# DJjjjhao/FIRA-ICSE

Measured on AMD Instinct MI355X. Metric: training commits/sec (FIRA default config), higher is better.
Workload: dtype f32; 1 GPU; BASELINE configs[1]: FIRA training step (fwd+bwd+Adam, dropout 0.1/0.2), batch 32 commits/GPU, fp32, 650-node graphs (mean nnz 1066/graph), vocab 24650; global_batch=32, parallelism=dp1

## Files before the change

### fira_icse_amd/_lib.py

```python
from __future__ import annotations

import ctypes as C
import os

HERE = os.path.dirname(os.path.abspath(__file__))
LIB_PATH = os.environ.get("FIRA_HIP_LIB") or os.path.join(HERE, "libfira_hip.so")


class FiraError(RuntimeError):
    pass


class Dims(C.Structure):
    _fields_ = [("sou_len", C.c_int32), ("sub_len", C.c_int32), ("ast_len", C.c_int32), ("tar_len", C.c_int32),
                ("d_model", C.c_int32), ("n_head", C.c_int32), ("n_layer", C.c_int32), ("vocab", C.c_int32),
                ("ast_vocab", C.c_int32), ("d_ff", C.c_int32)]


class Batch(C.Structure):
    _fields_ = [("B", C.c_int32), ("nnz", C.c_int32), ("sou", C.c_void_p), ("tar", C.c_void_p), ("mark", C.c_void_p),
                ("ast_change", C.c_void_p), ("tar_label", C.c_void_p), ("sub_token", C.c_void_p),
                ("n_nodes", C.c_int32), ("node_rows", C.c_void_p), ("rowptr", C.c_void_p), ("col", C.c_void_p),
                ("val", C.c_void_p), ("n_code", C.c_int32), ("code_rows", C.c_void_p), ("code_mark", C.c_void_p),
                ("n_mem", C.c_int32), ("mem_rows", C.c_void_p), ("mem_dst", C.c_void_p), ("head_rows", C.c_void_p),
                ("n_head_rows", C.c_int32), ("n_emb_items", C.c_int32), ("emb_item_tok", C.c_void_p),
                ("emb_item_ptr", C.c_void_p), ("emb_rows", C.c_void_p), ("n_ast_items", C.c_int32),
                ("ast_rows", C.c_void_p), ("ast_ids", C.c_void_p), ("dec_off", C.c_void_p), ("n_dec_rows", C.c_int32),
                ("dec_off_host", C.c_void_p)]


class TrainOpts(C.Structure):
    _fields_ = [("dropout", C.c_float), ("gcn_dropout", C.c_float), ("seed", C.c_uint64), ("compact_head", C.c_int32),
                ("dtype", C.c_int32), ("compact_dec", C.c_int32), ("zero_grads", C.c_int32)]


class LrSchedule(C.Structure):
    _fields_ = [("kind", C.c_int32), ("base_lr", C.c_float), ("warmup_steps", C.c_int32), ("decay_steps", C.c_int32),
                ("min_lr", C.c_float)]


class AdamOpts(C.Structure):
    _fields_ = [("lr", C.c_float), ("beta1", C.c_float), ("beta2", C.c_float), ("eps", C.c_float), ("step", C.c_int32),
                ("m", C.c_void_p), ("v", C.c_void_p), ("sched", C.POINTER(LrSchedule))]


def sched_ptr(sched):
    return None if sched is None else C.pointer(sched)


class ClipState(C.Structure):
    _fields_ = [("sq", C.c_float * 4), ("norm", C.c_float), ("coef", C.c_float), ("zero_flag", C.c_int32),
                ("n_clipped", C.c_int32), ("n_nonfinite", C.c_int32), ("reserved", C.c_int32 * 7)]


class RedEntry(C.Structure):
    _fields_ = [("dst", C.c_void_p), ("src", C.c_void_p), ("width", C.c_int32), ("n_part", C.c_int32),
                ("stride", C.c_int32)]


_P, _I, _F, _L, _Z = C.c_void_p, C.c_int, C.c_float, C.c_int64, C.c_size_t
_U64, _U32 = C.c_uint64, C.c_uint32
_DP, _BP, _OP = C.POINTER(Dims), C.POINTER(Batch), C.POINTER(TrainOpts)

SIGNATURES = {
    "fira_last_error": (C.c_char_p, []),
    "fira_abi_version": (_I, []),
    "fira_param_count": (_I, [_DP]),
    "fira_param_info": (_I, [_DP, _I, C.c_char_p, C.POINTER(_L), C.POINTER(_L), C.POINTER(C.c_int32), C.POINTER(_L)]),
    "fira_param_total": (_L, [_DP]),
    "fira_workspace_bytes": (_Z, [_DP, _I, _I]),
    "fira_decode_workspace_bytes": (_Z, [_DP, _I, _I]),
    "fira_decode_workspace_bytes_ex": (_Z, [_DP, _I, _I, _I]),
    "fira_gemm_f32": (_I, [_P, _I, _I, _I, _I, _I, _P, _I, _P, _I, _P, _I, _P, _I, _I]),
    "fira_gemm_bf16": (_I, [_P, _I, _I, _I, _I, _I, _P, _I, _P, _I, _P, _I, _P, _I, _I]),
    "fira_weight_shadow": (_I, [_P, _I, _I, _P, _P, _P]),
    "fira_gemm_bf16_wb": (_I, [_P, _I, _I, _I, _P, _I, _P, _I, _P, _I, _P, _I, _I]),
    "fira_csr_spmm_f32": (_I, [_P, _I, _P, _P, _P, _P, _I, _P, _I, _I, _I]),
    "fira_csr_spmm": (_I, [_P, _I, _L, _P, _P, _P, _P, _I, _P, _I, _I, _I, _I]),
    "fira_gcn_layer_fwd": (_I, [_P, _I, _P, _P, _P, _P, _P, _P, _P, _P, _P, _P, _P, _P, _P, _F, _U64, _U32, _I]),
    "fira_gcn_layer_bwd": (_I, [_P, _I, _P, _P, _P, _P, _P, _P, _P, _I]),
    "fira_gcn_weight_planes": (_I, [_P, _I, _P, _P]),
    "fira_linear_x3": (_I, [_P, _I, _I, _P, _I, _P, _P, _P, _I, _I]),
    "fira_linear_dgrad_x3": (_I, [_P, _I, _I, _P, _I, _P, _P, _I, _I, _I]),
    "fira_dgrad_x3_splitk_planes_bytes": (_Z, [_I]),
    "fira_dgrad_x3_splitk": (_I, [_P, _I, _I, _P, _I, _P, _P, _P, _I, _I]),
    "fira_head_logits_x3_scratch_bytes": (_Z, [_I]),
    "fira_head_logits_x3": (_I, [_P, _I, _I, _P, _I, _P, _P, _P, _I, _P]),
    "fira_combination_block_fwd": (_I, [_P, _I, _P, _P, _P, _P, _P, _P, _P, _I, _P, _P, _P, _P, _P, _P, _P, _P, _P, _F, _U64, _U32, _U32, _I]),
    "fira_combination_block_bwd": (_I, [_P, _I, _P, _P, _P, _P, _P, _P, _P, _P, _P, _I, _P, _P, _P, _P, _P, _P, _I, _P, _F, _U64, _U32, _U32, _I]),
    "fira_combination_block_bwd_part_floats": (_I, []),
    "fira_embed_gather_fwd": (_I, [_P, _I, _I, _P, _P, _P, _P, _I, _I]),
    "fira_embed_gather_bwd": (_I, [_P, _I, _I, _P, _P, _P, _I, _I, _I]),
    "fira_combination_fwd": (_I, [_P, _I, _P, _P, _P, _P, _F, _U64, _U32]),
    "fira_combination_bwd": (_I, [_P, _I, _P, _P, _P, _P, _P, _P, _F, _U64, _U32]),
    "fira_add_layernorm_fwd": (_I, [_P, _I, _P, _P, _P, _P, _P, _P, _F, _U64, _U32]),
    "fira_linear_presum_f32": (_I, [_P, _I, _I, _P, _I, _P, _P, _P, _P, _F, _U64, _U32]),
    "fira_ln_linear_f32": (_I, [_P, _I, _I, _P, _I, _P, _P, _P, _I, _I, _P, _P, _P, _P]),
    "fira_ln_bwd_linear_f32": (_I, [_P, _I, _I, _P, _P, _P, _P, _P, _P, _P, _P, _P, _P, _P, _P, _F, _U64, _U32]),
    "fira_linear_layernorm_bf16_fwd": (_I, [_P, _I, _P, _I, _P, _I, _P, _P, _P, _P, _P, _P, _P, _F, _U64, _U32]),
    "fira_add_layernorm_bwd": (_I, [_P, _I, _P, _P, _P, _P, _P, _P, _P, _P, _F, _U64, _U32]),
    "fira_dropout_mask": (_I, [_P, _U64, _U32, _L, _F, _P]),
    "fira_colsum_f32": (_I, [_P, _I, _I, _P, _I, _P]),
    "fira_attention_fwd": (_I, [_P, _I, _I, _I, _I, _P, _I, _P, _I, _P, _I, _P, _I, _I, _P, _I]),
    "fira_attention_bwd": (_I, [_P, _I, _I, _I, _I, _P, _I, _P, _I, _P, _I, _P, _I, _I, _P, _I, _P, _I,
                                _P, _I, _P, _I, _P, _I]),
    "fira_attention_fwd_ex": (_I, [_P, _I, _I, _I, _I, _P, _I, _P, _I, _P, _I, _P, _I, _I, _P, _I, _P, _I, _I, _P]),
    "fira_attention_bwd_ex": (_I, [_P, _I, _I, _I, _I, _P, _I, _P, _I, _P, _I, _P, _I, _I, _P, _I, _P, _I,
                                   _P, _I, _P, _I, _P, _I, _P, _I, _I, _P]),
    "fira_decode_attention": (_I, [_P, _I, _I, _I, _P, _I, _P, _I, _P, _I, _P, _P, _I, _I, _I, _I, _P, _P, _I, _P, _P, _P]),
    "fira_copy_score_fwd": (_I, [_P, _I, _I, _I, _P, _P, _P, _P, _P]),
    "fira_copy_score_bwd": (_I, [_P, _I, _I, _I, _P, _P, _P, _P, _P, _P, _P, _P]),
    "fira_head_loss": (_I, [_P, _I, _I, _I, _I, _P, _P, _I, _P, _P, _P, _P, _P, _P, _P, _I]),
    "fira_copy_score_fwd_ex": (_I, [_P, _I, _I, _I, _P, _P, _P, _P, _P, _I, _P, _P, _I, _P]),
    "fira_copy_score_bwd_ex": (_I, [_P, _I, _I, _I, _P, _P, _P, _P, _P, _P, _P, _P, _P, _P, _P]),
    "fira_copy_score_bwd_blocks": (_I, [_I, _I]),
    "fira_copy_part_stride": (_I, []),
    "fira_head_loss_ex": (_I, [_P, _I, _I, _I, _I, _P, _P, _I, _P, _P, _P, _P, _P, _P, _P, _I, _P]),
    "fira_deferred_reduce_max": (_I, []),
    "fira_deferred_reduce": (_I, [_P, _I, C.POINTER(RedEntry)]),
    "fira_rows_move": (_I, [_P, _I, _I, _I, _P, _I, _P, _I, _P, _P]),
    "fira_rank2_rows": (_I, [_P, _I, _P, _P, _P]),
    "fira_colsum_weighted": (_I, [_P, _I, _I, _P, _I, _P, _P]),
    "fira_embed_rows_fwd": (_I, [_P, _I, _I, _P, _P, _P, _P, _P]),
    "fira_embed_rows_bwd": (_I, [_P, _I, _P, _P, _P, _P, _I]),
    "fira_embed_grouped_bwd": (_I, [_P, _I, _P, _P, _P, _P, _P]),
    "fira_embed_list_bwd_small": (_I, [_P, _I, _P, _P, _P, _P, _I]),
    "fira_embed_gather_bwd_small": (_I, [_P, _I, _I, _P, _P, _P, _I, _I, _I, _I]),
    "fira_adam_step": (_I, [_P, _L, _P, _P, _P, _P, _F, _F, _F, _F, _I, _P]),
    "fira_adam_step_mb": (_I, [_P, _L, _P, _P, _P, _P, _P, _F, _F, _F, _F, _I, _P, _P]),
    "fira_inv_count": (_I, [_P, _P, _P]),
    "fira_adam_step_count": (_I, [_P, _L, _P, _P, _P, _P, _F, _F, _F, _F, _I, _P]),
    "fira_pack_stats": (_I, [_P, _P, _P, _P]),
    "fira_accum_stats": (_I, [_P, _P, _P, _P, _P, _I]),
    "fira_train_accum_micro": (_I, [_P, _DP, _BP, _P, _P, _P, _Z, _OP, _P, _P, C.POINTER(AdamOpts), _P]),
    "fira_train_accum_last": (_I, [_P, _DP, _BP, _P, _P, _P, _Z, _OP, _P, _P, C.POINTER(AdamOpts), _P, _P, _P, _F, _P, _P]),
    "fira_debug_chain": (_I, [_P, _I, _I, _P]),
    "fira_train_fwd_bwd": (_I, [_P, _DP, _BP, _P, _P, _P, _Z, _OP, _P, _P, _P]),
    "fira_train_step": (_I, [_P, _DP, _BP, _P, _P, _P, _Z, _OP, _P, _P, C.POINTER(AdamOpts)]),
    "fira_gemm_wgrad_panel": (_I, [_P, _I, _I, _I, _I, _P, _I, _P, _I, _P, _I, _P, _P, _Z]),
    "fira_ffn_fwd": (_I, [_P, _I, _I] + [_P] * 11 + [_F, _U64, _U32, _I]),
    "fira_ffn_bwd": (_I, [_P, _I, _I] + [_P] * 17 + [_F, _U64, _U32, _I]),
    "fira_head_topk": (_I, [_P, _I, _I, _I, _P, _P, _P, _P, _I, _P, _P, _I]),
    "fira_train_step_rows": (_I, [_P, _DP, _BP, _P, _P, _P, _Z, _OP, _P, _P, C.POINTER(AdamOpts), _P]),
    "fira_adam_rows_sync": (_I, [_P, _DP, _P, C.POINTER(AdamOpts), _P]),
    "fira_adam_rows_catchup": (_I, [_P, _DP, _P, C.POINTER(AdamOpts), _P, _I, _P, _I]),
    "fira_adam_rows_step": (_I, [_P, _DP, _P, _P, C.POINTER(AdamOpts), _P, _P, _P, _I]),
    "fira_train_step_begin_rows": (_I, [_P, _DP, _BP, _P, _P, _P, _Z, _OP, _P, _P, _P, C.POINTER(AdamOpts), _P]),
    "fira_train_step_end_rows": (_I, [_P, _P, C.POINTER(AdamOpts), _P, _P, _P]),
    "fira_ema_update": (_I, [_P, _L, _P, _P, _F]),
    "fira_ema_update_rows": (_I, [_P, _DP, _P, _P, C.POINTER(AdamOpts), _P, _F]),
    "fira_grad_sqsum_scratch_bytes": (_Z, []),
    "fira_grad_sqsum": (_I, [_P, _L, _P, _P, _I, _P]),
    "fira_clip_finish": (_I, [_P, _P, _I, _P, _P, _F]),
    "fira_adam_step_clip": (_I, [_P, _L, _P, _P, _P, _P, _F, _F, _F, _F, _I, _P, _P, _P]),
    "fira_adam_rows_step_clip": (_I, [_P, _DP, _P, _P, C.POINTER(AdamOpts), _P, _P, _P, _I, _P]),
    "fira_train_step_clip": (_I, [_P, _DP, _BP, _P, _P, _P, _Z, _OP, _P, _P, C.POINTER(AdamOpts), _P, _F, _P, _P]),
    "fira_lr_at": (_F, [C.POINTER(LrSchedule), _I]),
    "fira_lr_schedule_check": (_I, [C.POINTER(LrSchedule)]),
    "fira_train_step_begin": (_I, [_P, _DP, _BP, _P, _P, _P, _Z, _OP, _P, _P, _P]),
    "fira_train_step_end": (_I, [_P, _P, C.POINTER(AdamOpts), _P, _P]),
    "fira_f32_to_bf16": (_I, [_P, _L, _P, _P]),
    "fira_bf16_to_f32": (_I, [_P, _L, _P, _P]),
    "fira_prof_enable": (None, [_I]),
    "fira_prof_report": (_I, [_I, C.POINTER(C.c_double), C.POINTER(C.c_double), C.POINTER(C.c_double), C.POINTER(_L)]),
    "fira_param_groups": (_I, [_DP, C.POINTER(_L), C.POINTER(_L)]),
    "fira_host_node_lists": (_I, [_I, _I, _I, _I, _I] + [_P] * 7 + [_I] + [_P] * 14),
    "fira_host_collate_csr": (_I, [_I, _I, _P, _L, _P, _P, _P, _P, _P, _P, _P]),
    "fira_forward_dev": (_I, [_P, _DP, _BP, _P, _P, _Z, _P, _P, _P, _I]),
    "fira_dev_bleu_stats": (_I, [_P, _I, _I, _I, _I, _I, _P, _P, _P, _P, _P, _P]),
    "fira_mbr_bleu_stats": (_I, [_P, _I, _I, _I, _P, _P, _P]),
    "fira_dev_rouge_l_stats": (_I, [_P, _I, _I, _I, _I, _I, _P, _P, _P, _P, _P]),
    "fira_mbr_rouge_l_stats": (_I, [_P, _I, _I, _I, _P, _P, _P]),
    "fira_dev_meteor_stats": (_I, [_P, _I, _I, _I, _I, _I, _P, _P, _P, _P, _P, _P]),
    "fira_mbr_meteor_stats": (_I, [_P, _I, _I, _I, _P, _P, _I, _P, _P]),
    "fira_constrain_dist": (_I, [_P, _DP, _I, _I, _P, _P, _P, _P, _I, _I, _P, _I, _P, _P, _P]),
    "fira_merge_dist": (_I, [_P, _DP, _I, _I, _P, _P, _P, _P, _P]),
    "fira_force_dist": (_I, [_P, _DP, _I, _I, _P, _P, _P, _P, _P, _P, _P, _P, _P]),
    "fira_penalise_dist": (_I, [_P, _DP, _I, _I, _P, _P, _P, _P, _P, _P, _P, _P, _P, _P, _P]),
    "fira_ban_phrases_dist": (_I, [_P, _DP, _I, _I] + [_P] * 10),
    "fira_template_dist": (_I, [_P, _DP, _I, _I] + [_P] * 11),
    "fira_wordset_dist": (_I, [_P, _DP, _I, _I] + [_P] * 13),
    "fira_mix_dist": (_I, [_P, _I, _I, _I, C.POINTER(_P), C.POINTER(_F), _P, _P, _P]),
    "fira_pool_memory": (_I, [_P, _DP, _I, _P, _P, _P]),
    "fira_nn_search_scratch_bytes": (_Z, [_I, _I]),
    "fira_nn_search": (_I, [_P, _P, _I, _P, _I, _P, _P, _P, _P, _Z]),
    "fira_mix_neighbour": (_I, [_P, _DP, _I, _I, _P, _P, _P, _P, _P]),
    "fira_knn_search_scratch_bytes": (_Z, [_I, _I, _I]),
    "fira_knn_search": (_I, [_P, _P, _I, _P, _P, _P, _P, _I, _I, _P, _P, _P, _Z]),
    "fira_mix_knn": (_I, [_P, _DP, _I, _P, _P, _P, _I, _I, _P, _P, _P, _P]),
    "fira_decode_begin": (_I, [_P, _DP, _BP, _P, _P, _Z, _I]),
    "fira_decode_begin_ex": (_I, [_P, _DP, _BP, _P, _P, _Z, _I, _I]),
    "fira_decode_step_ex": (_I, [_P, _DP, _P, _P, _Z, _I, _I, _I, _P, _P, _P, _P, _P, _I]),
    "fira_beam_prepare": (_I, [_P, _I, _I, _I, _I, _P, _P, _P, _P, _P, _P]),
    "fira_beam_select": (_I, [_P, _DP, _I, _I, _P, _P, _P, _P, _P, _P, _P, _P, _P, _P, _P, _P, _P]),
    "fira_beam_select_scored": (_I, [_P, _DP, _I, _I, _P, _P, _P, _P, _P, _P, _P, _P, _P, _P, _P, _P, _P, _P, _I, _F, _P]),
    "fira_beam_select_gumbel": (_I, [_P, _DP, _I, _I, _I, _F] + [_P] * 18),
    "fira_beam_select_required": (_I, [_P, _DP, _I, _I] + [_P] * 16),
    "fira_beam_select_phrases": (_I, [_P, _DP, _I, _I] + [_P] * 17),
    "fira_contrastive_select": (_I, [_P, _DP, _I, _I, _I, _F] + [_P] * 19),
    "fira_greedy_advance": (_I, [_P, _DP, _I, _I, _P, _P, _P, _P, _P, _P, _P, _P, _P, _P]),
    "fira_decode_step": (_I, [_P, _DP, _P, _P, _Z, _I, _I, _I, _P, _P, _P, _P, _P]),
    "fira_decode_step_sample": (_I, [_P, _DP, _P, _P, _Z, _I, _I, _I, _P, _P, _P, _F, _I, _F, _P, _P, _P, _I]),
    "fira_decode_step_sample_cut": (_I, [_P, _DP, _P, _P, _Z, _I, _I, _I, _P, _P, _P, _F, _I, _F, _F, _F, _F, _F, _P, _P, _P,
                                        _I]),
    "fira_sample_dist": (_I, [_P, _DP, _I, _I, _I, _P, _P, _P, _F, _I, _F, _F, _F, _F, _F, _P, _P]),
    "fira_decode_step_score": (_I, [_P, _DP, _P, _P, _Z, _I, _I, _I] + [_P] * 15 + [_I]),
    "fira_sample_advance": (_I, [_P, _DP, _I, _I, _I, _P, _P, _P, _P, _P, _P, _P, _P, _P, _P, _P]),
    "fira_decoder_forward": (_I, [_P, _DP, _P, _P, _Z, _I, _P, _P, _P, _P]),
    "fira_decode_memory": (_P, [_DP, _P, _I, _I]),
    "fira_decode_mem_valid": (_P, [_DP, _P, _I, _I]),
    "fira_decode_hidden": (_I, [_P, _DP, _P, _Z, _I, _I, _I, _P]),
}


def _ensure_built():
    if os.path.exists(LIB_PATH):
        return
    import fcntl
    from . import build as _build
    with open(os.path.join(HERE, ".build.lock"), "w") as lock:
        fcntl.flock(lock, fcntl.LOCK_EX)
        try:
            if not os.path.exists(LIB_PATH):
                _build.build()
        finally:
            fcntl.flock(lock, fcntl.LOCK_UN)


def load():
    try:
        _ensure_built()
    except Exception as e:
        raise ImportError(
            "fira_icse_amd: %s is missing and could not be built (%s). Build it with `python -m fira_icse_amd.build` "
            "(needs hipcc, gfx950). There is no CPU fallback." % (LIB_PATH, e))
    lib = C.CDLL(LIB_PATH)
    if lib.fira_abi_version() != 11:
        raise ImportError("libfira_hip.so ABI version mismatch")
    for name, (res, args) in SIGNATURES.items():
        fn = getattr(lib, name)
        fn.restype = res
        fn.argtypes = args
    return lib


_lib = None


def lib():
    global _lib
    if _lib is None:
        _lib = load()
    return _lib


_host_warned = False
_host_failed = False


def host_lib():
    global _host_warned, _host_failed
    if _host_failed:
        return None
    try:
        return lib()
    except (ImportError, OSError, AttributeError) as e:
        _host_failed = True
        if not _host_warned:
            _host_warned = True
            import warnings
            warnings.warn("fira_icse_amd: libfira_hip.so unavailable (%s); host collate falls back to numpy" % (e,))
        return None


def check(rc: int, what: str = ""):
    if rc != 0:
        msg = lib().fira_last_error()
        raise FiraError("%s failed: %s" % (what or "libfira_hip call", msg.decode() if msg else "unknown error"))


def ptr(t):
    return None if t is None else C.c_void_p(t.data_ptr())


def cur_stream():
    import torch
    return C.c_void_p(torch.cuda.current_stream().cuda_stream)


def make_dims(cfg) -> Dims:
    return Dims(cfg.sou_len, cfg.sub_token_len, cfg.ast_change_len, cfg.tar_len, cfg.embedding_dim, cfg.num_head,
                cfg.num_layers, cfg.vocab_size, cfg.ast_change_vocab_size, 4 * cfg.embedding_dim)
```

### fira_icse_amd/csrc/engine.h

```cpp
#pragma once
#include "common.h"
#include <string>
#include <vector>

namespace fira {

int gemm_f32(hipStream_t s, int tA, int tB, int M, int N, int K, const float* A, int lda, const float* B, int ldb,
             float* C, int ldc, const float* bias, int flags, int splitk);
int gemm_f32_ex(hipStream_t s, int tA, int tB, int M, int N, int K, const float* A, int lda, const float* B, int ldb,
                float* C, int ldc, const float* bias, int flags, int splitk, float* colsum,
                const int32_t* c_rows = nullptr, const float* relu_mask = nullptr);
int gemm_bf16_ex(hipStream_t s, int tA, int tB, int M, int N, int K, const float* A, int lda, const float* B, int ldb,
                 float* C, int ldc, const float* bias, int flags, int splitk, float* colsum,
                 const int32_t* c_rows = nullptr, const float* relu_mask = nullptr);
struct ShadowEntry { int64_t offset; int rows, cols, pitch_t; int64_t offset_t; };
constexpr int SHADOW_MAX = 64;
struct ShadowTable {
    int n = 0;
    int64_t wbt_elems = 0;
    int tile_start[SHADOW_MAX + 1] = {0};
    ShadowEntry e[SHADOW_MAX];
};
int weight_shadows(hipStream_t s, const ShadowTable& tab, const float* P, uint16_t* Wb, uint16_t* WbT);
int gemm_bf16_wb_ex(hipStream_t s, int M, int N, int K, const float* A, int lda, const uint16_t* Bb, int ldb, float* C,
                    int ldc, const float* bias, int flags, int splitk, const int32_t* c_rows = nullptr,
                    const float* relu_mask = nullptr);
bool gemm_bf16_takes(int M, int N, int K);
struct GroupProblem {
    const float* A;
    const float* B;
    float* C;
    float* colsum;
    int M, N, K, lda, ldb, ldc, tiles_m, tiles_n, splitk, k_chunk;
};
constexpr int GROUP_MAX = 40;
struct GroupTable {
    int n = 0, chunk = 0;
    int wg_start[GROUP_MAX + 1] = {0};
    GroupProblem p[GROUP_MAX];
    void cost(double& flop, double& bytes) const {
        flop = bytes = 0;
        for (int i = 0; i < n; ++i) {
            const double M = p[i].M, N = p[i].N, K = p[i].K;
            flop += 2.0 * M * N * K;
            bytes += 4.0 * (M * K + N * K + M * N);
        }
    }
};
int gemm_group_plan(GroupProblem& q, int max_split);
int gemm_group_launch(hipStream_t s, const GroupTable& t);
int gemm_bf16_group_plan(GroupProblem& q, int max_split);
int gemm_bf16_group_launch(hipStream_t s, GroupTable& t);
struct PanelProblem {
    const float *A, *B;
    float *C, *colsum;
    float* part;
    int M, N, K, lda, ldb, ldc;
    int tiles_m, tiles_n, slabs, k_slab;
};
constexpr int PANEL_MAX = 48;
struct PanelTable {
    int n = 0;
    int wg_start[PANEL_MAX + 1] = {0};
    PanelProblem p[PANEL_MAX];
};
bool gemm_wgrad_panel_takes(int M, int N, int K, const float* A, int lda, const float* B, int ldb, int ldc);
int gemm_wgrad_panel_launch(hipStream_t s, int np, PanelTable& t, float* scratch, size_t scratch_floats);
struct WgradQueue {
    GroupTable tiled;
    PanelTable panels;
    float* scratch = nullptr;
    size_t scratch_floats = 0;
    int dtype = 0;
    void reset(int dtype_, float* scratch_, size_t floats) {
        tiled.n = 0; panels.n = 0;
        dtype = dtype_; scratch = scratch_; scratch_floats = scratch_ ? floats : 0;
    }
    bool full() const { return tiled.n == GROUP_MAX || panels.n == PANEL_MAX; }
    int panel_pending() const { return panels.n; }
    int add_tiled(int M, int N, int K, const float* A, int lda, const float* B, int ldb, float* C, int ldc, float* colsum,
                  int max_split = 0) {
        if (M <= 0 || N <= 0 || K <= 0) return 0;
        FIRA_REQUIRE(tiled.n < GROUP_MAX, "wgrad queue: tiled group full (fork and flush first)");
        GroupProblem& q = tiled.p[tiled.n];
        q.A = A; q.B = B; q.C = C; q.colsum = colsum;
        q.M = M; q.N = N; q.K = K; q.lda = lda; q.ldb = ldb; q.ldc = ldc;
        q.tiles_m = cdiv(M, 64); q.tiles_n = cdiv(N, 64);
        if (int rc = dtype == 1 ? gemm_bf16_group_plan(q, max_split) : gemm_group_plan(q, max_split)) return rc;
        tiled.wg_start[tiled.n + 1] = tiled.wg_start[tiled.n] + q.tiles_m * q.tiles_n * q.splitk;
        ++tiled.n;
        return 0;
    }
    int add_panel(int M, int N, int K, const float* A, int lda, const float* B, int ldb, float* C, int ldc, float* colsum) {
        FIRA_REQUIRE(panels.n < PANEL_MAX, "wgrad queue: panel table full (fork and flush first)");
        PanelProblem& q = panels.p[panels.n++];
        q.A = A; q.B = B; q.C = C; q.colsum = colsum;
        q.M = M; q.N = N; q.K = K; q.lda = lda; q.ldb = ldb; q.ldc = ldc;
        q.tiles_m = cdiv(M, 256); q.tiles_n = N / 256;
        q.slabs = 1; q.k_slab = K; q.part = nullptr;
        return 0;
    }
    int flush(hipStream_t s) {
        int rc = 0;
        if (tiled.n > 0) rc = dtype == 1 ? gemm_bf16_group_launch(s, tiled) : gemm_group_launch(s, tiled);
        tiled.n = 0;
        return rc ? rc : flush_panels(s);
    }
    int flush_panels(hipStream_t s) {
        const int rc = gemm_wgrad_panel_launch(s, dtype == 1 ? 1 : 3, panels, scratch, scratch_floats);
        panels.n = 0;
        return rc;
    }
};
constexpr int GEMM_SIDE_PAD = 1 << 8;
struct EpiRes;
bool gemm_tile32_takes(int tB, int M, int N, int K, const float* A, int lda, const float* B, int ldb);
bool gemm_tile32_try(hipStream_t s, int tB, int M, int N, int K, const float* A, int lda, const float* B, int ldb,
                     float* C, int ldc, const float* bias, int flags, int* rc, const int32_t* c_rows,
                     const float* relu_mask, const int32_t* a_rows, const EpiRes* er);
bool gemm_tile32_ln_try(hipStream_t s, int M, int N, const float* S, int lds, const float* W, const float* bias, float* Y,
                        int ldy, int flags, const float* gamma, const float* beta, float* x_out, float* stats_out, int* rc);
int gemm_tile32_lnb_blocks(int M);
bool gemm_tile32_lnb_try(hipStream_t s, int M, int N, const float* dy, const float* W, int ldw, float* dX, int lddx,
                         const float* relu_mask, const float* sum, const float* stats, const float* gamma, float* ds,
                         float* dx_drop, float* part, float dropout, uint64_t seed, uint32_t site, int* rc,
                         uint32_t idx0 = 0);
bool gemm_small_try(hipStream_t s, int tA, int tB, int M, int N, int K, const float* A, int lda, const float* B, int ldb,
                    float* C, int ldc, const float* bias, int flags, int* rc, const int32_t* c_rows = nullptr,
                    const float* relu_mask = nullptr);
int csr_spmm(hipStream_t s, int n_rows, const int32_t* rowptr, const int32_t* col, const float* val, const float* X,
             int ldx, float* Y, int ldy, int graph_rows, int variant);
int csr_spmm_ex(hipStream_t s, int n_rows, const int32_t* rowptr, const int32_t* col, const float* val, const float* X,
                int ldx, float* Y, int ldy, int graph_rows, int variant, int accum, float* rowsum);
int gcn_fused_fwd(hipStream_t s, int n_rows, const int32_t* rowptr, const int32_t* col, const float* val, const float* X,
                  const float* Wk, const float* bias, const float* r1_col, const float* gamma, const float* beta, float* sum,
                  float* y, float* stats, float* rowsum_out, const int32_t* slot2, float* y2, float dropout, uint64_t seed,
                  uint32_t site, int bf16, const uint16_t* Wx = nullptr);
int gcn_fused_bwd(hipStream_t s, int n_rows, const int32_t* rowptr, const int32_t* col, const float* val, const float* dY,
                  const float* Wk, float* u_out, float* acc_out, int bf16, const uint16_t* Wx = nullptr);
int gcn_split_planes(hipStream_t s, int n, const float* const* src, uint16_t* const* dst);
size_t head_logits_x3_scratch_elems(int R);
int head_logits_x3(hipStream_t s, int R, int V, const float* x, int ldx, const float* W, const float* bias, float* out, int ldo,
                   uint16_t* xplanes);
int transpose256(hipStream_t s, int nl, const float* W, float* Wt);
int linear_x3(hipStream_t s, int M, const float* X, int ldx, const uint16_t* Wx, int nb, const float* bias, float* out, int ldo,
              bool one_plane);
int split_planes_t(hipStream_t s, const float* W, int V, uint16_t* planes, bool one_plane);
int dgrad_x3_splitk(hipStream_t s, int M, int K, const float* A, int lda, const uint16_t* Wx, float* out, int ldo, bool one_plane);
int linear_x3_kacc(hipStream_t s, int M, const float* A, int lda, const uint16_t* Wx, int nkb, float* out, int ldo, bool accum,
                   bool one_plane);
int comb_fused_fwd(hipStream_t s, int n_rows, const float* Xc, const float* WqT, const float* WkT, const float* WoT,
                   const float* bqk, const float* bo, const float* vtab, int ldv, const int32_t* mark, float* qk, float* c,
                   const float* gamma, const float* beta, float* sum, float* y, const int32_t* y_rows, float* stats,
                   float dropout, uint64_t seed, uint32_t site_gate, uint32_t site_out, int bf16, const uint16_t* Wx = nullptr);
int comb_fused_bwd_parts();
int comb_fused_bwd(hipStream_t s, int n_rows, float* dG, const int32_t* rows, const float* sum, const float* stats,
                   const float* gamma, const float* Wo, const float* Wqk, const float* qk, const float* vtab, int ldv,
                   const int32_t* mark, float* dYc, float* dqk, float* part_ln, float* part_v, float dropout, uint64_t seed,
                   uint32_t site_gate, uint32_t site_out, int bf16, const uint16_t* WTx = nullptr);
struct TransposeTable { int n = 0; const float* src[24]; float* dst[24]; };
int transpose256_table(hipStream_t s, const TransposeTable& tab);
int embed_gather_fwd(hipStream_t s, int B, int L, const int32_t* idx, const float* table, const float* pos, float* out,
                     int out_bstride, int out_off);
int embed_grouped_bwd(hipStream_t s, int n_items, const int32_t* item_tok, const int32_t* item_ptr, const int32_t* rows,
                      float* dtable, const float* dnode);
int embed_list_bwd_small(hipStream_t s, int n, const int32_t* rows, const int32_t* ids, float* dtable, const float* dnode,
                         int table_rows);
int embed_gather_bwd(hipStream_t s, int B, int L, const int32_t* idx, float* dtable, const float* dout,
                     int out_bstride, int out_off, int padding_idx);
int embed_gather_bwd_small(hipStream_t s, int B, int L, const int32_t* idx, float* dtable, const float* dout,
                           int out_bstride, int out_off, int padding_idx, int table_rows);
int combination_fwd(hipStream_t s, int M, const float* qk, const float* vtab, int ldv, const int32_t* mark, float* out,
                    float dropout, uint64_t seed, uint32_t site);
int combination_bwd(hipStream_t s, int M, const float* qk, const float* vtab, int ldv, const int32_t* mark,
                    const float* dout, float* dqk, float* dvtab, int lddv, float dropout, uint64_t seed, uint32_t site,
                    float* part = nullptr);
int combination_bwd_blocks(int M);
struct RedEntry { float* dst; const float* src; int width, n_part, stride; };
constexpr int RED_MAX = 96;
struct RedTable {
    int n = 0;
    int wg_start[RED_MAX + 1] = {0};
    RedEntry e[RED_MAX];
};
int deferred_reduce(hipStream_t s, RedTable& tab);
int add_layernorm_fwd(hipStream_t s, int M, float* x, const float* res, const float* gamma, const float* beta,
                      float* y, float* stats, float dropout, uint64_t seed, uint32_t site, const int32_t* y_rows, const float* r1_row = nullptr,
                      const float* r1_col = nullptr,
                      const int32_t* slot2 = nullptr, float* y2 = nullptr,
                      uint32_t idx0 = 0);
bool gemm_bf16_k256_try(hipStream_t s, int M, int N, int K, const float* A, int lda, const uint16_t* Bb, int ldb, float* C,
                        int ldc, const float* bias, int flags, const int32_t* c_rows, const float* relu_mask, int* rc);
bool linear_ln_bf16_try(hipStream_t s, int M, int K, const float* X, int ldx, const uint16_t* Wb, int ldb, const float* bias,
                        const float* res, const float* gamma, const float* beta, float* sum, float* y, float* stats,
                        float dropout, uint64_t seed, uint32_t site, const int32_t* y_rows, const float* r1_row,
                        const float* r1_col, int* rc, bool force = false);
int add_layernorm_bwd(hipStream_t s, int M, const float* dy, const float* sum, const float* stats, const float* gamma,
                      float* ds, float* dx_drop, float* dgamma, float* dbeta, float dropout, uint64_t seed,
                      uint32_t site, const int32_t* rows = nullptr,
                      float* part = nullptr,
                      const float* row_w = nullptr, uint32_t idx0 = 0);
int add_layernorm_bwd_blocks(int M);
int gcn_bias_unfold(hipStream_t s, const float* W2, const float* b1, const float* dc, float* dW2, float* db1);
struct UnfoldEntry { const float *W2, *b1, *dc; float *dW2, *db1; };
struct UnfoldTable { int n = 0; UnfoldEntry e[16]; };
int gcn_bias_unfold_all(hipStream_t s, const UnfoldTable& tab);
int gcn_fold_weights(hipStream_t s, int n_layers, const float* const* W2, const float* const* W1, const float* const* b1,
                     float* W21, float* W21t, float* c21);
int gcn_unfold_products(hipStream_t s, int n_layers, const float* const* dW21, const float* const* W1, const float* const* W2,
                        float* const* dW1, float* const* dW2);
int colsum(hipStream_t s, int M, int N, const float* X, int ldx, float* out, const float* row_weight = nullptr);
int rank2_rows(hipStream_t s, int M, const float* g, const float* w, float* out);
int prep(hipStream_t s, int B, int L, int S, int T, const int32_t* sou, const int32_t* sub, const int32_t* tar,
         int32_t* mem_valid, int32_t* tar_valid, float* pos_code, float* pos_tar, int R, const int32_t* rows,
         int32_t* compact_row, int32_t* iota, float* loss_sum = nullptr, int32_t* n_tok = nullptr,
         int Nc = 0, const int32_t* code_rows = nullptr, int Cc = 0, int32_t* code_slot = nullptr,
         const int32_t* mem_rows = nullptr, int Mc = 0, int32_t* mem_slot = nullptr,
         const int32_t* dec_off = nullptr, int32_t* row_bt = nullptr, int32_t* rows_c = nullptr,
         const int32_t* mem_dst = nullptr, int32_t* mem_off = nullptr, int32_t* mem_valid_c = nullptr);
struct AdamRowsView;
int embed_rows_fwd(hipStream_t s, int R, int T, const int32_t* row_bt, const int32_t* idx, const float* table,
                   const float* pos, float* out, const AdamRowsView* vw = nullptr);
int embed_rows_bwd(hipStream_t s, int R, const int32_t* row_bt, const int32_t* idx, float* dtable, const float* dout,
                   int padding_idx);
int node_features(hipStream_t s, int Nc, const int32_t* node_rows, int N, int L, int S, const int32_t* sou,
                  const int32_t* sub, const int32_t* ast, const float* emb, const float* ast_emb, const float* pos_code,
                  float* X, const int32_t* slot2 = nullptr, float* X2 = nullptr,
                  const AdamRowsView* vw = nullptr);
int rows_move(hipStream_t s, int mode, int R, int W, float* out, const float* in, const int32_t* src, const int32_t* dst);
int rows_move_ld(hipStream_t s, int mode, int R, int W, float* out, int ld_out, const float* in, int ld_in,
                 const int32_t* src, const int32_t* dst);
int rows_gather_idx(hipStream_t s, int R, float* compact, const float* src, const int32_t* rows);
int rows_scatter_add_idx(hipStream_t s, int R, const float* compact, float* dst, const int32_t* rows);
int fill_pos_tables(hipStream_t s, int L, float* pos_code, int T, float* pos_tar);
int tar_mask(hipStream_t s, int n, const int32_t* tar, int32_t* valid);
int permute_cache(hipStream_t s, int nl, int BR, int T, int len, const int32_t* parent, const float* ksrc,
                  const float* vsrc, float* kdst, float* vdst, const int32_t* hist_src, int32_t* hist_dst);
int mark_history(hipStream_t s, int BR, int T, int step, const int32_t* tokens, int32_t* hist);
int decode_embed(hipStream_t s, int BR, int T, int step, const int32_t* tokens, const float* table, const float* pos_row,
                 float* x, int32_t* hist);

int attention_fwd(hipStream_t s, int B, int H, int Tq, int Tk, const float* Q, int ldq, const float* K, int ldk,
                  const float* V, int ldv, const int32_t* key_valid, int causal, int q_pos0, float* O, int ldo,
                  const int32_t* q_off = nullptr, int self_kv = 0,
                  int bf16 = 0,
                  const int32_t* k_off = nullptr);
int attention_fwd_ex(hipStream_t s, int B, int H, int Tq, int Tk, const float* Q, int ldq, const float* K, int ldk,
                     const float* V, int ldv, const int32_t* key_valid, int causal, int q_pos0, float* O, int ldo,
                     int kb, int kvb, int qpk, const int32_t* q_off = nullptr, int self_kv = 0, int bf16 = 0,
                     const int32_t* k_off = nullptr);
int decode_attention(hipStream_t s, int BR, int H, int Tk, const float* Q, int ldq, const float* K, int ldk,
                     const float* V, int ldv, const int32_t* key_valid, float* O, int ldo, int kb, int kvb, int qpk,
                     const float* Knew = nullptr, const float* Vnew = nullptr, int ldn = 0, float* Kc_out = nullptr,
                     float* Vc_out = nullptr, const int32_t* k_off = nullptr);
int decode_self_block(hipStream_t s, int BR, int Tk, int T, const float* qkv, float* Kc, float* Vc, const int32_t* hist,
                      const float* WoT, const float* bo, const float* xres, const float* gamma, const float* beta,
                      const float* WqT, const float* bq, float* xa, float* qc);
int decode_attention_kv16(hipStream_t s, int BR, int H, int Tk, const float* Q, int ldq, const uint16_t* K, int ldk,
                          const uint16_t* V, int ldv, const int32_t* key_valid, float* O, int ldo, int kb, int kvb, int qpk,
                          const int32_t* k_off = nullptr);
int rows_to_bf16(hipStream_t s, int64_t n, const float* in, uint16_t* out);
int rows_from_bf16(hipStream_t s, int64_t n, const uint16_t* in, float* out);
int attention_bwd(hipStream_t s, int B, int H, int Tq, int Tk, const float* Q, int ldq, const float* K, int ldk,
                  const float* V, int ldv, const int32_t* key_valid, int causal, int q_pos0, const float* O, int ldo,
                  const float* dO, int lddo, float* dQ, int lddq, float* dK, int lddk, float* dV, int lddv,
                  const int32_t* q_off = nullptr, int self_kv = 0, int bf16 = 0, const int32_t* k_off = nullptr);
int copy_score_fwd(hipStream_t s, int B, int T, int S, const float* src, const float* tgt, const float* w,
                   const float* bias, float* score);
int copy_score_fwd_ex(hipStream_t s, int B, int T, int S, const float* src, const float* tgt, const float* w,
                      const float* bias, float* score, int qpk, const int32_t* mem_valid,
                      const int32_t* tar_label = nullptr, int V = 0,
                      const int32_t* t_off = nullptr);
int copy_score_bwd_ex(hipStream_t s, int B, int T, int S, const float* src, const float* tgt, const float* w,
                      const float* dscore, float* dsrc, float* dtgt, float* dw, float* dbias, const int32_t* mem_valid,
                      float* part = nullptr, const int32_t* t_off = nullptr);
int copy_score_bwd_blocks(int B, int S);
constexpr int COPY_PART_STRIDE = 264;
int decode_dist(hipStream_t s, int R, int V, int S, const float* logits, int ldl, const float* score,
                const int32_t* mem_valid, int qpk, const float* gate_logits, float* dist, int32_t* best_id,
                float* best_p, const float* x = nullptr, const float* wp = nullptr, const float* bp = nullptr);
int inv_count(hipStream_t s, const int32_t* n_tok, float* out);
int accum_stats(hipStream_t s, const float* loss_sum, const int32_t* n_tok, float* stats, int32_t* n_tok_total, int first);
struct SampleCuts {
    float min_p = 0.f, epsilon = 0.f, eta = 0.f, typical_p = 1.f;
    bool on() const { return min_p > 0.f || epsilon > 0.f || eta > 0.f || typical_p < 1.f; }
};
int require_sampler_args(const char* who, int W, float temperature, int top_k, float top_p, const SampleCuts* cut);
int sample_dist(hipStream_t s, int R, int n_sample, int V, int S, const float* logits, int ldl, const float* score,
                const int32_t* mem_valid, const float* x, const float* wp, const float* bp, int T, int step,
                const int32_t* key, const uint64_t* seed_dev, float temperature, int top_k, float top_p, float* dist,
                int32_t* best_id, float* best_p, const SampleCuts* cut = nullptr);
int score_dist(hipStream_t s, int R, int n_cand, int V, int L, int S, const float* logits, int ldl, const float* score,
               const int32_t* mem_valid, const float* x, const float* wp, const float* bp, const int32_t* target,
               const int32_t* label, const int32_t* sou, const int32_t* sub, float* dist, float* p_word, float* p_entry,
               int32_t* entry, float* copy_share, float* p_label, int32_t* top_id, float* logp_word, float* logp_entry,
               float* logp_label);
int row_topk(hipStream_t s, int R, int V, int k, const float* logits, int ldl, int32_t* ids, float* vals);
int copy_score_bwd(hipStream_t s, int B, int T, int S, const float* src, const float* tgt, const float* w,
                   const float* dscore, float* dsrc, float* dtgt, float* dw, float* dbias);
int head_loss(hipStream_t s, int BT, int T, int V, int S, const int32_t* compact_row, float* logits, int ldl,
              float* score, const int32_t* mem_valid, float* gate_logits, const int32_t* tar_label, float* loss_sum,
              int32_t* n_tok, int32_t* argmax_out, int want_grad,
              const int32_t* row_bt = nullptr);
int adam_step(hipStream_t s, int64_t n, float* p, const float* g, float* m, float* v, float lr, float beta1,
              float beta2, float eps, int step, const float* scale_ptr, int scale_is_count = 0);
int adam_step_mb(hipStream_t s, int64_t n, float* p, const float* g0, const float* g1, float* m, float* v, float lr,
                 float beta1, float beta2, float eps, int step, const int32_t* n0, const int32_t* n1);
constexpr int ADAM_ROWS_K = 32;
struct AdamRowsHist { float bc1[ADAM_ROWS_K], bc2s[ADAM_ROWS_K], lr[ADAM_ROWS_K]; };
struct AdamLr {
    float lr = 0.f;
    bool scheduled = false;
    fira_lr_schedule sched{};
    float at(int step) const { return scheduled ? fira_lr_at(&sched, step) : lr; }
};
inline AdamLr adam_lr(const fira_adam_opts& ad) {
    AdamLr r;
    r.lr = ad.lr;
    if (ad.sched) { r.scheduled = true; r.sched = *ad.sched; }
    return r;
}
struct AdamRowsTables { float *p, *m, *v; int64_t off[2]; int rows[2]; int32_t* last; };
struct AdamRowsView {
    const float *m = nullptr, *v = nullptr;
    const int32_t* last = nullptr;
    int to = 0;
    float beta1 = 0.f, beta2 = 0.f, eps = 0.f, gz = 0.f;
    AdamRowsHist h;
};
AdamRowsView adam_rows_view(const AdamRowsTables& tb, int table, const AdamLr& lr, float beta1, float beta2, float eps, int to);
struct AdamRowsLists { int n_lists; int end[4]; int table[4]; const int32_t* ids[4]; };
int adam_rows_step(hipStream_t s, const AdamRowsTables& tb, const float* g, const AdamLr& lr, float beta1, float beta2, float eps,
                   int step, const int32_t* n0, const float* count, int tables = 3);
int adam_rows_catchup(hipStream_t s, const AdamRowsTables& tb, const AdamRowsLists* ls, const AdamLr& lr, float beta1, float beta2,
                      float eps, int to);
AdamRowsHist adam_rows_hist(const AdamLr& lr, float beta1, float beta2, int end);
struct ClipClose {
    const int32_t* n_tok;
    const float* count;
    float max_norm;
    int n_slots;
};
size_t grad_sqsum_scratch_bytes();
int grad_sqsum(hipStream_t s, int64_t n, const float* g, fira_clip_state* st, int slot, void* scratch, const ClipClose* fin);
int clip_finish(hipStream_t s, fira_clip_state* st, const ClipClose& fin);
int adam_step_clip(hipStream_t s, int64_t n, float* p, const float* g, float* m, float* v, float lr, float beta1, float beta2,
                   float eps, int step, const int32_t* n0, const float* count, const fira_clip_state* st);
int adam_rows_step_clip(hipStream_t s, const AdamRowsTables& tb, const float* g, const AdamLr& lr, float beta1, float beta2, float eps,
                        int step, const int32_t* n0, const float* count, int tables, const fira_clip_state* st);

struct ParamInfo {
    std::string name;
    int64_t offset = -1, numel = 0;
    int ndim = 0;
    int64_t shape[2] = {0, 0};
};

struct EncLayer {
    int64_t wqk, bqk, w2, b2, wo, bo, ln1g, ln1b, fc1w, fc1b, fc2w, fc2b, ln2g, ln2b;
};
struct DecLayer {
    int64_t wqkv, bqkv, wo_s, bo_s, lns_g, lns_b, wq_c, bq_c, wkv_c, bkv_c, wo_c, bo_c, lnc_g, lnc_b, w1, b1, w2, b2,
        lnf_g, lnf_b;
};
struct Layout {
    fira_dims d;
    std::vector<ParamInfo> infos;
    int64_t total = 0;
    int64_t split = 0, live = 0;
    int64_t emb, ast_emb, mark_emb, w2_all, b2_all, dec_emb, wkv_all, bkv_all, wout, bout, ws, wt, wres, bres, wp, bp;
    std::vector<EncLayer> enc;
    std::vector<DecLayer> dec;
};
const Layout* get_layout(const fira_dims* d);

}
```

### fira_icse_amd/csrc/gemm_small.hip

```cpp
#include "engine.h"
#include "epilogue.h"
#include <stdlib.h>

namespace fira {

typedef float f32x16 __attribute__((ext_vector_type(16)));
typedef float f32x4 __attribute__((ext_vector_type(4)));

template <bool B_KCONTIG>
__global__ __launch_bounds__(256) void gemm_small_kernel(int M, int N, int K, const float* __restrict__ A, int lda,
                                                         const float* __restrict__ B, int ldb, float* __restrict__ C,
                                                         int ldc, const float* __restrict__ bias, int flags,
                                                         const int32_t* __restrict__ c_rows,
                                                         const float* __restrict__ relu_mask) {
    __shared__ float red[4][1024];
    const int lane = threadIdx.x & 63, wave = threadIdx.x >> 6;
    const int l31 = lane & 31, kh = lane >> 5;
    const int m0 = blockIdx.y * 32, n0 = blockIdx.x * 32;
    const float* pa = A + (size_t)min(m0 + l31, M - 1) * lda + kh * 16;
    const float* pb = B_KCONTIG ? B + (size_t)min(n0 + l31, N - 1) * ldb + kh * 16
                                : B + (size_t)(kh * 16) * ldb + min(n0 + l31, N - 1);
    f32x16 acc;
#pragma unroll
    for (int r = 0; r < 16; ++r) acc[r] = 0.f;
    const int nchunk = K / 32;
    for (int c = wave; c < nchunk; c += 8) {
        float a[2][16], b[2][16];
#pragma unroll
        for (int u = 0; u < 2; ++u) {
            const int cc = c + 4 * u;
            if (cc < nchunk) {
                const float4* qa = reinterpret_cast<const float4*>(pa + cc * 32);
#pragma unroll
                for (int q = 0; q < 4; ++q) {
                    const float4 v = qa[q];
                    a[u][4 * q] = v.x; a[u][4 * q + 1] = v.y; a[u][4 * q + 2] = v.z; a[u][4 * q + 3] = v.w;
                }
                if (B_KCONTIG) {
                    const float4* qb = reinterpret_cast<const float4*>(pb + cc * 32);
#pragma unroll
                    for (int q = 0; q < 4; ++q) {
                        const float4 v = qb[q];
                        b[u][4 * q] = v.x; b[u][4 * q + 1] = v.y; b[u][4 * q + 2] = v.z; b[u][4 * q + 3] = v.w;
                    }
                } else {
                    const float* qb = pb + (size_t)cc * 32 * ldb;
#pragma unroll
                    for (int s = 0; s < 16; ++s) b[u][s] = qb[(size_t)s * ldb];
                }
            } else {
#pragma unroll
                for (int s = 0; s < 16; ++s) { a[u][s] = 0.f; b[u][s] = 0.f; }
            }
        }
#pragma unroll
        for (int u = 0; u < 2; ++u)
#pragma unroll
            for (int s = 0; s < 16; ++s) acc = __builtin_amdgcn_mfma_f32_32x32x2f32(a[u][s], b[u][s], acc, 0, 0, 0);
    }
#pragma unroll
    for (int r = 0; r < 16; ++r) red[wave][r * 64 + lane] = acc[r];
    __syncthreads();
    {
        const int ln = threadIdx.x & 63, rq = threadIdx.x >> 6;
        float vals[4];
        int rows[4];
#pragma unroll
        for (int i = 0; i < 4; ++i) {
            const int idx = threadIdx.x + 256 * i, r = rq + 4 * i;
            vals[i] = (red[0][idx] + red[1][idx]) + (red[2][idx] + red[3][idx]);
            rows[i] = m0 + (r & 3) + 8 * (r >> 2) + 4 * (ln >> 5);
        }
        epilogue_col<4>(vals, rows, n0 + (ln & 31), M, N, C, ldc, bias, flags & FIRA_GEMM_RELU, flags & FIRA_GEMM_ACCUM, false,
                        c_rows, relu_mask);
    }
}

__device__ __forceinline__ int swz8(int row) { return (row >> 1) & 7; }

struct ChunkRegs { f32x4 a0, a1, a2, a3, b0, b1, b2, b3; };

template <bool B_KCONTIG>
__device__ __forceinline__ void tile32_fetch(ChunkRegs& R, const float* pa0, const float* pa1, const float* pa2,
                                             const float* pa3, const float* pb0, const float* pb1, const float* pb2,
                                             const float* pb3, int kc, int ldb) {
    const size_t ob = B_KCONTIG ? (size_t)kc : (size_t)kc * ldb;
    R.a0 = *reinterpret_cast<const f32x4*>(pa0 + kc);
    R.a1 = *reinterpret_cast<const f32x4*>(pa1 + kc);
    R.a2 = *reinterpret_cast<const f32x4*>(pa2 + kc);
    R.a3 = *reinterpret_cast<const f32x4*>(pa3 + kc);
    R.b0 = *reinterpret_cast<const f32x4*>(pb0 + ob);
    R.b1 = *reinterpret_cast<const f32x4*>(pb1 + ob);
    R.b2 = *reinterpret_cast<const f32x4*>(pb2 + ob);
    R.b3 = *reinterpret_cast<const f32x4*>(pb3 + ob);
}

#define FIRA_MFMA4(va, vb)                                                    \
    acc = __builtin_amdgcn_mfma_f32_32x32x2f32(va.x, vb.x, acc, 0, 0, 0);     \
    acc = __builtin_amdgcn_mfma_f32_32x32x2f32(va.y, vb.y, acc, 0, 0, 0);     \
    acc = __builtin_amdgcn_mfma_f32_32x32x2f32(va.z, vb.z, acc, 0, 0, 0);     \
    acc = __builtin_amdgcn_mfma_f32_32x32x2f32(va.w, vb.w, acc, 0, 0, 0);

__device__ __forceinline__ void tile32_stage(const ChunkRegs& R, char* slot, int wr_off) {
    __builtin_amdgcn_wave_barrier();
    *reinterpret_cast<f32x4*>(slot + wr_off) = R.a0;
    *reinterpret_cast<f32x4*>(slot + wr_off + 1024) = R.a1;
    *reinterpret_cast<f32x4*>(slot + wr_off + 2048) = R.a2;
    *reinterpret_cast<f32x4*>(slot + wr_off + 3072) = R.a3;
    *reinterpret_cast<f32x4*>(slot + 4096 + wr_off) = R.b0;
    *reinterpret_cast<f32x4*>(slot + 4096 + wr_off + 1024) = R.b1;
    *reinterpret_cast<f32x4*>(slot + 4096 + wr_off + 2048) = R.b2;
    *reinterpret_cast<f32x4*>(slot + 4096 + wr_off + 3072) = R.b3;
    __builtin_amdgcn_fence(__ATOMIC_RELEASE, "wavefront");
    __builtin_amdgcn_wave_barrier();
    __builtin_amdgcn_fence(__ATOMIC_ACQUIRE, "wavefront");
}
template <bool B_KCONTIG>
__device__ __forceinline__ f32x16 tile32_compute(const char* slot, int fa0, int fa1, int fa2, int fa3, int fb, f32x16 acc) {
    const f32x4 va0 = *reinterpret_cast<const f32x4*>(slot + fa0);
    const f32x4 va1 = *reinterpret_cast<const f32x4*>(slot + fa1);
    const f32x4 va2 = *reinterpret_cast<const f32x4*>(slot + fa2);
    const f32x4 va3 = *reinterpret_cast<const f32x4*>(slot + fa3);
    if (B_KCONTIG) {
        const f32x4 vb0 = *reinterpret_cast<const f32x4*>(slot + 4096 + fa0);
        const f32x4 vb1 = *reinterpret_cast<const f32x4*>(slot + 4096 + fa1);
        const f32x4 vb2 = *reinterpret_cast<const f32x4*>(slot + 4096 + fa2);
        const f32x4 vb3 = *reinterpret_cast<const f32x4*>(slot + 4096 + fa3);
        FIRA_MFMA4(va0, vb0) FIRA_MFMA4(va1, vb1) FIRA_MFMA4(va2, vb2) FIRA_MFMA4(va3, vb3)
    } else {
        const char* pb = slot + 4096 + fb;
        f32x4 vb0, vb1, vb2, vb3;
        vb0.x = *reinterpret_cast<const float*>(pb);        vb0.y = *reinterpret_cast<const float*>(pb + 128);
        vb0.z = *reinterpret_cast<const float*>(pb + 256);  vb0.w = *reinterpret_cast<const float*>(pb + 384);
        vb1.x = *reinterpret_cast<const float*>(pb + 512);  vb1.y = *reinterpret_cast<const float*>(pb + 640);
        vb1.z = *reinterpret_cast<const float*>(pb + 768);  vb1.w = *reinterpret_cast<const float*>(pb + 896);
        vb2.x = *reinterpret_cast<const float*>(pb + 1024); vb2.y = *reinterpret_cast<const float*>(pb + 1152);
        vb2.z = *reinterpret_cast<const float*>(pb + 1280); vb2.w = *reinterpret_cast<const float*>(pb + 1408);
        vb3.x = *reinterpret_cast<const float*>(pb + 1536); vb3.y = *reinterpret_cast<const float*>(pb + 1664);
        vb3.z = *reinterpret_cast<const float*>(pb + 1792); vb3.w = *reinterpret_cast<const float*>(pb + 1920);
        FIRA_MFMA4(va0, vb0) FIRA_MFMA4(va1, vb1) FIRA_MFMA4(va2, vb2) FIRA_MFMA4(va3, vb3)
    }
    return acc;
}

struct LnA {
    const float* gamma = nullptr;
    const float* beta = nullptr;
    float* x_out = nullptr;
    float* stats_out = nullptr;
};

struct LnB {
    const float* sum = nullptr;
    const float* stats = nullptr;
    const float* gamma = nullptr;
    float* ds = nullptr;
    float* dx = nullptr;
    float* part = nullptr;
    float p = 0.f, inv_keep = 1.f;
    uint64_t seed = 0;
    uint32_t site = 0;
    uint32_t idx0 = 0;
};

template <bool B_KCONTIG, int NCH, bool LN_A = false, bool LN_B = false, int NW = 4>
__global__ __launch_bounds__(NW * 64) void gemm_tile32_kernel(int M, int N, const float* __restrict__ A, int lda,
                                                          const float* __restrict__ B, int ldb, float* __restrict__ C,
                                                          int ldc, const float* __restrict__ bias, int flags,
                                                          const int32_t* __restrict__ c_rows,
                                                          const float* __restrict__ relu_mask,
                                                          const int32_t* __restrict__ a_rows, int tiles_n, const EpiRes er,
                                                          const LnA ln, const LnB lb) {
    static_assert(NW == 4 || (!LN_A && !LN_B), "the LayerNorm prologues are written for four waves");
    extern __shared__ __attribute__((aligned(16))) char tile32_dyn[];
    __shared__ __attribute__((aligned(16))) char smem4[NW == 4 ? 4 * 8192 : 16];
    char* const smem = NW == 4 ? smem4 : tile32_dyn;
    __shared__ float ln_red[2][4][32];
    const int lane = threadIdx.x & 63;
    const int wave = __builtin_amdgcn_readfirstlane(threadIdx.x >> 6);
    int t;
    {
        const int b = blockIdx.x, nwg = gridDim.x, q = nwg >> 3, r = nwg & 7, x = b & 7;
        t = (x < r ? x * (q + 1) : r * (q + 1) + (x - r) * q) + (b >> 3);
    }
    const int m0 = (t / tiles_n) * 32, n0 = (t % tiles_n) * 32;
    char* slot = smem + wave * 8192;
    const int lr = lane >> 3, ls = lane & 7;
    const int sw_even = lr >> 1, sw_odd = 4 + (lr >> 1);
    int ra0 = min(m0 + lr, M - 1), ra1 = min(m0 + 8 + lr, M - 1), ra2 = min(m0 + 16 + lr, M - 1), ra3 = min(m0 + 24 + lr, M - 1);
    if (a_rows) { ra0 = a_rows[ra0]; ra1 = a_rows[ra1]; ra2 = a_rows[ra2]; ra3 = a_rows[ra3]; }
    const float* pa0 = A + (size_t)ra0 * lda + ((ls ^ sw_even) << 2);
    const float* pa1 = A + (size_t)ra1 * lda + ((ls ^ sw_odd) << 2);
    const float* pa2 = A + (size_t)ra2 * lda + ((ls ^ sw_even) << 2);
    const float* pa3 = A + (size_t)ra3 * lda + ((ls ^ sw_odd) << 2);
    const float *pb0, *pb1, *pb2, *pb3;
    if (B_KCONTIG) {
        pb0 = B + (size_t)min(n0 + lr, N - 1) * ldb + ((ls ^ sw_even) << 2);
        pb1 = B + (size_t)min(n0 + 8 + lr, N - 1) * ldb + ((ls ^ sw_odd) << 2);
        pb2 = B + (size_t)min(n0 + 16 + lr, N - 1) * ldb + ((ls ^ sw_even) << 2);
        pb3 = B + (size_t)min(n0 + 24 + lr, N - 1) * ldb + ((ls ^ sw_odd) << 2);
    } else {
        pb0 = B + (size_t)lr * ldb + n0 + (ls << 2);
        pb1 = pb0 + (size_t)8 * ldb;
        pb2 = pb0 + (size_t)16 * ldb;
        pb3 = pb0 + (size_t)24 * ldb;
    }
    const int i31 = lane & 31, kh = lane >> 5;
    const int wr_off = lr * 128 + ls * 16;
    const int sw_i = swz8(i31);
    const int fa0 = i31 * 128 + (((kh * 4 + 0) ^ sw_i) << 4), fa1 = i31 * 128 + (((kh * 4 + 1) ^ sw_i) << 4);
    const int fa2 = i31 * 128 + (((kh * 4 + 2) ^ sw_i) << 4), fa3 = i31 * 128 + (((kh * 4 + 3) ^ sw_i) << 4);
    const int fb = kh * 16 * 128 + i31 * 4;
    f32x16 acc;
#pragma unroll
    for (int r = 0; r < 16; ++r) acc[r] = 0.f;
    ChunkRegs R0, R1;
    tile32_fetch<B_KCONTIG>(R0, pa0, pa1, pa2, pa3, pb0, pb1, pb2, pb3, wave << 5, ldb);
    if (NCH > 1) tile32_fetch<B_KCONTIG>(R1, pa0, pa1, pa2, pa3, pb0, pb1, pb2, pb3, (wave + NW) << 5, ldb);
    if (LN_A) {
        static_assert(!LN_A || NCH == 2, "the LayerNorm prologue needs the whole row in the two chunks of the four waves");
        auto hsum = [](const f32x4 v) { return (v.x + v.y) + (v.z + v.w); };
        const int ce = (ls ^ sw_even) << 2, co = (ls ^ sw_odd) << 2;
        const int k0 = wave << 5, k1 = (wave + 4) << 5;
        const f32x4 g0e = *reinterpret_cast<const f32x4*>(ln.gamma + k0 + ce), g0o = *reinterpret_cast<const f32x4*>(ln.gamma + k0 + co);
        const f32x4 g1e = *reinterpret_cast<const f32x4*>(ln.gamma + k1 + ce), g1o = *reinterpret_cast<const f32x4*>(ln.gamma + k1 + co);
        const f32x4 b0e = *reinterpret_cast<const f32x4*>(ln.beta + k0 + ce), b0o = *reinterpret_cast<const f32x4*>(ln.beta + k0 + co);
        const f32x4 b1e = *reinterpret_cast<const f32x4*>(ln.beta + k1 + ce), b1o = *reinterpret_cast<const f32x4*>(ln.beta + k1 + co);
        asm volatile("" ::: "memory");
        float mean[4], rstd[4];
        {
            const float p0 = sum8(hsum(R0.a0) + hsum(R1.a0)), p1 = sum8(hsum(R0.a1) + hsum(R1.a1));
            const float p2 = sum8(hsum(R0.a2) + hsum(R1.a2)), p3 = sum8(hsum(R0.a3) + hsum(R1.a3));
            if (ls == 0) { ln_red[0][wave][lr] = p0; ln_red[0][wave][8 + lr] = p1; ln_red[0][wave][16 + lr] = p2; ln_red[0][wave][24 + lr] = p3; }
            __syncthreads();
#pragma unroll
            for (int j = 0; j < 4; ++j)
                mean[j] = ((ln_red[0][0][8 * j + lr] + ln_red[0][1][8 * j + lr]) + (ln_red[0][2][8 * j + lr] + ln_red[0][3][8 * j + lr])) *
                          (1.0f / FIRA_D);
        }
        {
            auto sq = [](const f32x4 v, float m) { const f32x4 d = v - m; return (d.x * d.x + d.y * d.y) + (d.z * d.z + d.w * d.w); };
            const float p0 = sum8(sq(R0.a0, mean[0]) + sq(R1.a0, mean[0])), p1 = sum8(sq(R0.a1, mean[1]) + sq(R1.a1, mean[1]));
            const float p2 = sum8(sq(R0.a2, mean[2]) + sq(R1.a2, mean[2])), p3 = sum8(sq(R0.a3, mean[3]) + sq(R1.a3, mean[3]));
            if (ls == 0) { ln_red[1][wave][lr] = p0; ln_red[1][wave][8 + lr] = p1; ln_red[1][wave][16 + lr] = p2; ln_red[1][wave][24 + lr] = p3; }
            __syncthreads();
#pragma unroll
            for (int j = 0; j < 4; ++j) {
                const float var = ((ln_red[1][0][8 * j + lr] + ln_red[1][1][8 * j + lr]) + (ln_red[1][2][8 * j + lr] + ln_red[1][3][8 * j + lr])) *
                                  (1.0f / FIRA_D);
                rstd[j] = 1.0f / sqrtf(var + 1e-5f);
            }
        }
        R0.a0 = (R0.a0 - mean[0]) * rstd[0] * g0e + b0e; R1.a0 = (R1.a0 - mean[0]) * rstd[0] * g1e + b1e;
        R0.a1 = (R0.a1 - mean[1]) * rstd[1] * g0o + b0o; R1.a1 = (R1.a1 - mean[1]) * rstd[1] * g1o + b1o;
        R0.a2 = (R0.a2 - mean[2]) * rstd[2] * g0e + b0e; R1.a2 = (R1.a2 - mean[2]) * rstd[2] * g1e + b1e;
        R0.a3 = (R0.a3 - mean[3]) * rstd[3] * g0o + b0o; R1.a3 = (R1.a3 - mean[3]) * rstd[3] * g1o + b1o;
        if (n0 == 0) {
            const int r0 = m0 + lr, r1 = m0 + 8 + lr, r2 = m0 + 16 + lr, r3 = m0 + 24 + lr;
            float* xo = ln.x_out;
            if (r0 < M) { *reinterpret_cast<f32x4*>(xo + (size_t)r0 * FIRA_D + k0 + ce) = R0.a0; *reinterpret_cast<f32x4*>(xo + (size_t)r0 * FIRA_D + k1 + ce) = R1.a0; }
            if (r1 < M) { *reinterpret_cast<f32x4*>(xo + (size_t)r1 * FIRA_D + k0 + co) = R0.a1; *reinterpret_cast<f32x4*>(xo + (size_t)r1 * FIRA_D + k1 + co) = R1.a1; }
            if (r2 < M) { *reinterpret_cast<f32x4*>(xo + (size_t)r2 * FIRA_D + k0 + ce) = R0.a2; *reinterpret_cast<f32x4*>(xo + (size_t)r2 * FIRA_D + k1 + ce) = R1.a2; }
            if (r3 < M) { *reinterpret_cast<f32x4*>(xo + (size_t)r3 * FIRA_D + k0 + co) = R0.a3; *reinterpret_cast<f32x4*>(xo + (size_t)r3 * FIRA_D + k1 + co) = R1.a3; }
            if (ln.stats_out && wave == 0 && ls == 0) {
                if (r0 < M) { ln.stats_out[2 * r0] = mean[0]; ln.stats_out[2 * r0 + 1] = rstd[0]; }
                if (r1 < M) { ln.stats_out[2 * r1] = mean[1]; ln.stats_out[2 * r1 + 1] = rstd[1]; }
                if (r2 < M) { ln.stats_out[2 * r2] = mean[2]; ln.stats_out[2 * r2 + 1] = rstd[2]; }
                if (r3 < M) { ln.stats_out[2 * r3] = mean[3]; ln.stats_out[2 * r3 + 1] = rstd[3]; }
            }
        }
    }
    if constexpr (LN_B) {
        static_assert(!LN_B || (NCH == 2 && !LN_A), "the LayerNorm-backward prologue needs the whole row in the two chunks of the four waves");
        auto hsum = [](const f32x4 v) { return (v.x + v.y) + (v.z + v.w); };
        const int ce = (ls ^ sw_even) << 2, co = (ls ^ sw_odd) << 2;
        const int k0 = wave << 5, k1 = (wave + 4) << 5;
        const float* ps0 = lb.sum + (size_t)ra0 * FIRA_D; const float* ps1 = lb.sum + (size_t)ra1 * FIRA_D;
        const float* ps2 = lb.sum + (size_t)ra2 * FIRA_D; const float* ps3 = lb.sum + (size_t)ra3 * FIRA_D;
        f32x4 s00 = *reinterpret_cast<const f32x4*>(ps0 + k0 + ce), s10 = *reinterpret_cast<const f32x4*>(ps0 + k1 + ce);
        f32x4 s01 = *reinterpret_cast<const f32x4*>(ps1 + k0 + co), s11 = *reinterpret_cast<const f32x4*>(ps1 + k1 + co);
        f32x4 s02 = *reinterpret_cast<const f32x4*>(ps2 + k0 + ce), s12 = *reinterpret_cast<const f32x4*>(ps2 + k1 + ce);
        f32x4 s03 = *reinterpret_cast<const f32x4*>(ps3 + k0 + co), s13 = *reinterpret_cast<const f32x4*>(ps3 + k1 + co);
        const float mean0 = lb.stats[2 * ra0], rstd0 = lb.stats[2 * ra0 + 1], mean1 = lb.stats[2 * ra1], rstd1 = lb.stats[2 * ra1 + 1];
        const float mean2 = lb.stats[2 * ra2], rstd2 = lb.stats[2 * ra2 + 1], mean3 = lb.stats[2 * ra3], rstd3 = lb.stats[2 * ra3 + 1];
        const f32x4 g0e = *reinterpret_cast<const f32x4*>(lb.gamma + k0 + ce), g0o = *reinterpret_cast<const f32x4*>(lb.gamma + k0 + co);
        const f32x4 g1e = *reinterpret_cast<const f32x4*>(lb.gamma + k1 + ce), g1o = *reinterpret_cast<const f32x4*>(lb.gamma + k1 + co);
        s00 = (s00 - mean0) * rstd0; s10 = (s10 - mean0) * rstd0; s01 = (s01 - mean1) * rstd1; s11 = (s11 - mean1) * rstd1;
        s02 = (s02 - mean2) * rstd2; s12 = (s12 - mean2) * rstd2; s03 = (s03 - mean3) * rstd3; s13 = (s13 - mean3) * rstd3;
        const f32x4 h00 = R0.a0 * g0e, h10 = R1.a0 * g1e, h01 = R0.a1 * g0o, h11 = R1.a1 * g1o;
        const f32x4 h02 = R0.a2 * g0e, h12 = R1.a2 * g1e, h03 = R0.a3 * g0o, h13 = R1.a3 * g1o;
        {
            const float p0 = sum8(hsum(h00) + hsum(h10)), p1 = sum8(hsum(h01) + hsum(h11));
            const float p2 = sum8(hsum(h02) + hsum(h12)), p3 = sum8(hsum(h03) + hsum(h13));
            const float q0 = sum8(hsum(h00 * s00) + hsum(h10 * s10)), q1 = sum8(hsum(h01 * s01) + hsum(h11 * s11));
            const float q2 = sum8(hsum(h02 * s02) + hsum(h12 * s12)), q3 = sum8(hsum(h03 * s03) + hsum(h13 * s13));
            if (ls == 0) {
                ln_red[0][wave][lr] = p0; ln_red[0][wave][8 + lr] = p1; ln_red[0][wave][16 + lr] = p2; ln_red[0][wave][24 + lr] = p3;
                ln_red[1][wave][lr] = q0; ln_red[1][wave][8 + lr] = q1; ln_red[1][wave][16 + lr] = q2; ln_red[1][wave][24 + lr] = q3;
            }
        }
        if (lb.part && n0 == 0) {
            const bool v0 = m0 + lr < M, v1 = m0 + 8 + lr < M, v2 = m0 + 16 + lr < M, v3 = m0 + 24 + lr < M;
            const f32x4 z = {0.f, 0.f, 0.f, 0.f};
            const f32x4 d00 = v0 ? R0.a0 : z, d10 = v0 ? R1.a0 : z, d01 = v1 ? R0.a1 : z, d11 = v1 ? R1.a1 : z;
            const f32x4 d02 = v2 ? R0.a2 : z, d12 = v2 ? R1.a2 : z, d03 = v3 ? R0.a3 : z, d13 = v3 ? R1.a3 : z;
            float* sc = reinterpret_cast<float*>(slot);
            float colsum[2];
#pragma unroll
            for (int pass = 0; pass < 2; ++pass) {
                __builtin_amdgcn_wave_barrier();
                *reinterpret_cast<f32x4*>(sc + (lr) * 64 + ce) = pass ? d00 : d00 * s00;
                *reinterpret_cast<f32x4*>(sc + (lr) * 64 + 32 + ce) = pass ? d10 : d10 * s10;
                *reinterpret_cast<f32x4*>(sc + (8 + lr) * 64 + co) = pass ? d01 : d01 * s01;
                *reinterpret_cast<f32x4*>(sc + (8 + lr) * 64 + 32 + co) = pass ? d11 : d11 * s11;
                *reinterpret_cast<f32x4*>(sc + (16 + lr) * 64 + ce) = pass ? d02 : d02 * s02;
                *reinterpret_cast<f32x4*>(sc + (16 + lr) * 64 + 32 + ce) = pass ? d12 : d12 * s12;
                *reinterpret_cast<f32x4*>(sc + (24 + lr) * 64 + co) = pass ? d03 : d03 * s03;
                *reinterpret_cast<f32x4*>(sc + (24 + lr) * 64 + 32 + co) = pass ? d13 : d13 * s13;
                __builtin_amdgcn_fence(__ATOMIC_RELEASE, "wavefront");
                __builtin_amdgcn_wave_barrier();
                __builtin_amdgcn_fence(__ATOMIC_ACQUIRE, "wavefront");
                float a0 = 0.f, a1 = 0.f;
#pragma unroll
                for (int r = 0; r < 32; r += 2) { a0 += sc[r * 64 + lane]; a1 += sc[(r + 1) * 64 + lane]; }
                colsum[pass] = a0 + a1;
            }
            const int col = ((wave + 4 * (lane >> 5)) << 5) + (lane & 31);
            float* pp = lb.part + (size_t)(m0 >> 5) * (2 * FIRA_D);
            pp[col] = colsum[0];
            pp[FIRA_D + col] = colsum[1];
        }
        __syncthreads();
        float m1[4], m2[4];
#pragma unroll
        for (int j = 0; j < 4; ++j) {
            m1[j] = ((ln_red[0][0][8 * j + lr] + ln_red[0][1][8 * j + lr]) + (ln_red[0][2][8 * j + lr] + ln_red[0][3][8 * j + lr])) * (1.0f / FIRA_D);
            m2[j] = ((ln_red[1][0][8 * j + lr] + ln_red[1][1][8 * j + lr]) + (ln_red[1][2][8 * j + lr] + ln_red[1][3][8 * j + lr])) * (1.0f / FIRA_D);
        }
        const f32x4 e00 = (h00 - m1[0] - s00 * m2[0]) * rstd0, e10 = (h10 - m1[0] - s10 * m2[0]) * rstd0;
        const f32x4 e01 = (h01 - m1[1] - s01 * m2[1]) * rstd1, e11 = (h11 - m1[1] - s11 * m2[1]) * rstd1;
        const f32x4 e02 = (h02 - m1[2] - s02 * m2[2]) * rstd2, e12 = (h12 - m1[2] - s12 * m2[2]) * rstd2;
        const f32x4 e03 = (h03 - m1[3] - s03 * m2[3]) * rstd3, e13 = (h13 - m1[3] - s13 * m2[3]) * rstd3;
        auto drop = [&](const f32x4 v, int row, int col) {
            if (lb.p <= 0.f) return v;
            const uint32_t e0 = lb.idx0 + (uint32_t)row * FIRA_D + (uint32_t)col;
            return f32x4{v.x * dropout_scale(lb.seed, lb.site, e0, lb.p, lb.inv_keep), v.y * dropout_scale(lb.seed, lb.site, e0 + 1, lb.p, lb.inv_keep),
                         v.z * dropout_scale(lb.seed, lb.site, e0 + 2, lb.p, lb.inv_keep), v.w * dropout_scale(lb.seed, lb.site, e0 + 3, lb.p, lb.inv_keep)};
        };
        const int r0 = m0 + lr, r1 = m0 + 8 + lr, r2 = m0 + 16 + lr, r3 = m0 + 24 + lr;
        R0.a0 = drop(e00, r0, k0 + ce); R1.a0 = drop(e10, r0, k1 + ce); R0.a1 = drop(e01, r1, k0 + co); R1.a1 = drop(e11, r1, k1 + co);
        R0.a2 = drop(e02, r2, k0 + ce); R1.a2 = drop(e12, r2, k1 + ce); R0.a3 = drop(e03, r3, k0 + co); R1.a3 = drop(e13, r3, k1 + co);
        if (n0 == 0) {
            float* o1 = lb.ds;
            float* o2 = lb.dx;
            if (r0 < M) { *reinterpret_cast<f32x4*>(o1 + (size_t)r0 * FIRA_D + k0 + ce) = e00; *reinterpret_cast<f32x4*>(o1 + (size_t)r0 * FIRA_D + k1 + ce) = e10;
                          *reinterpret_cast<f32x4*>(o2 + (size_t)r0 * FIRA_D + k0 + ce) = R0.a0; *reinterpret_cast<f32x4*>(o2 + (size_t)r0 * FIRA_D + k1 + ce) = R1.a0; }
            if (r1 < M) { *reinterpret_cast<f32x4*>(o1 + (size_t)r1 * FIRA_D + k0 + co) = e01; *reinterpret_cast<f32x4*>(o1 + (size_t)r1 * FIRA_D + k1 + co) = e11;
                          *reinterpret_cast<f32x4*>(o2 + (size_t)r1 * FIRA_D + k0 + co) = R0.a1; *reinterpret_cast<f32x4*>(o2 + (size_t)r1 * FIRA_D + k1 + co) = R1.a1; }
            if (r2 < M) { *reinterpret_cast<f32x4*>(o1 + (size_t)r2 * FIRA_D + k0 + ce) = e02; *reinterpret_cast<f32x4*>(o1 + (size_t)r2 * FIRA_D + k1 + ce) = e12;
                          *reinterpret_cast<f32x4*>(o2 + (size_t)r2 * FIRA_D + k0 + ce) = R0.a2; *reinterpret_cast<f32x4*>(o2 + (size_t)r2 * FIRA_D + k1 + ce) = R1.a2; }
            if (r3 < M) { *reinterpret_cast<f32x4*>(o1 + (size_t)r3 * FIRA_D + k0 + co) = e03; *reinterpret_cast<f32x4*>(o1 + (size_t)r3 * FIRA_D + k1 + co) = e13;
                          *reinterpret_cast<f32x4*>(o2 + (size_t)r3 * FIRA_D + k0 + co) = R0.a3; *reinterpret_cast<f32x4*>(o2 + (size_t)r3 * FIRA_D + k1 + co) = R1.a3; }
        }
    }
#pragma unroll
    for (int ci = 0; ci < NCH; ++ci) {
        if ((ci & 1) == 0) {
            tile32_stage(R0, slot, wr_off);
            if (ci + 2 < NCH) tile32_fetch<B_KCONTIG>(R0, pa0, pa1, pa2, pa3, pb0, pb1, pb2, pb3, (wave + NW * (ci + 2)) << 5, ldb);
        } else {
            tile32_stage(R1, slot, wr_off);
            if (ci + 2 < NCH) tile32_fetch<B_KCONTIG>(R1, pa0, pa1, pa2, pa3, pb0, pb1, pb2, pb3, (wave + NW * (ci + 2)) << 5, ldb);
        }
        acc = tile32_compute<B_KCONTIG>(slot, fa0, fa1, fa2, fa3, fb, acc);
    }
    __builtin_amdgcn_wave_barrier();
    float* red = reinterpret_cast<float*>(slot);
#pragma unroll
    for (int r = 0; r < 16; ++r) red[r * 64 + lane] = acc[r];
    __syncthreads();
    {
        constexpr int NV = (16 + NW - 1) / NW;
        const int lnn = threadIdx.x & 63;
        float vals[NV];
        int rows[NV];
        const float* p0 = reinterpret_cast<const float*>(smem);
#pragma unroll
        for (int i = 0; i < NV; ++i) {
            const int idx = threadIdx.x + NW * 64 * i, r = idx >> 6;
            const bool in = (16 % NW == 0) || idx < 1024;
            const int ix = in ? idx : threadIdx.x;
            if constexpr (NW == 4) {
                vals[i] = (p0[ix] + p0[2048 + ix]) + (p0[4096 + ix] + p0[6144 + ix]);
            } else {
                float v = 0.f;
#pragma unroll
                for (int w = 0; w < NW; w += 4)
                    v += (p0[w * 2048 + ix] + p0[(w + 1) * 2048 + ix]) + (p0[(w + 2) * 2048 + ix] + p0[(w + 3) * 2048 + ix]);
                vals[i] = v;
            }
            rows[i] = in ? m0 + (r & 3) + 8 * (r >> 2) + 4 * (lnn >> 5) : M;
        }
        epilogue_col<NV>(vals, rows, n0 + (lnn & 31), M, N, C, ldc, bias, flags & FIRA_GEMM_RELU, flags & FIRA_GEMM_ACCUM, false,
                         c_rows, relu_mask, er);
    }
}

template <bool B_KCONTIG, int NCH>
static void tile32_launch(hipStream_t s, dim3 grid, int M, int N, const float* A, int lda, const float* B, int ldb, float* C,
                          int ldc, const float* bias, int flags, const int32_t* c_rows, const float* relu_mask,
                          const int32_t* a_rows, int tiles_n, const EpiRes& er) {
    hipLaunchKernelGGL((gemm_tile32_kernel<B_KCONTIG, NCH, false, false>), grid, dim3(256), 0, s, M, N, A, lda, B, ldb, C, ldc, bias,
                       flags, c_rows, relu_mask, a_rows, tiles_n, er, LnA(), LnB());
}

static int tile32_waves(int K, int n_wg) {
    const int chunks = K / 32;
    if (chunks == 32 && n_wg <= 256) return 16;
    if (chunks == 24 && n_wg <= 256) return 12;
    if ((chunks == 16 || chunks == 32) && n_wg <= 512) return 8;
    return 4;
}
template <bool B_KCONTIG, int NCH, int NW>
static int tile32_launch_wide_t(hipStream_t s, dim3 grid, int M, int N, const float* A, int lda, const float* B, int ldb, float* C,
                                int ldc, const float* bias, int flags, const int32_t* c_rows, const float* relu_mask,
                                const int32_t* a_rows, int tiles_n, const EpiRes& er) {
    constexpr auto kern = gemm_tile32_kernel<B_KCONTIG, NCH, false, false, NW>;
    if (int rc = raise_dynamic_lds<kern>(NW * 8192, "gemm_tile32")) return rc;
    hipLaunchKernelGGL(kern, grid, dim3(NW * 64), NW * 8192, s, M, N, A, lda, B, ldb, C, ldc, bias, flags, c_rows, relu_mask, a_rows,
                       tiles_n, er, LnA(), LnB());
    hipError_t e = hipGetLastError();
    return e != hipSuccess ? set_err("gemm_tile32 (%d waves): %s", NW, hipGetErrorString(e)) : 0;
}
static int tile32_launch_wide(hipStream_t s, int nw, int K, int tB, dim3 grid, int M, int N, const float* A, int lda, const float* B,
                              int ldb, float* C, int ldc, const float* bias, int flags, const int32_t* c_rows,
                              const float* relu_mask, const int32_t* a_rows, int tiles_n, const EpiRes& er) {
#define FIRA_T32W(NCH, NW)                                                                                             \
    return tB ? tile32_launch_wide_t<true, NCH, NW>(s, grid, M, N, A, lda, B, ldb, C, ldc, bias, flags, c_rows, relu_mask, a_rows, tiles_n, er) \
              : tile32_launch_wide_t<false, NCH, NW>(s, grid, M, N, A, lda, B, ldb, C, ldc, bias, flags, c_rows, relu_mask, a_rows, tiles_n, er);
    const int per_wave = K / 32 / nw;
    if (nw == 16 && per_wave == 2) { FIRA_T32W(2, 16) }
    if (nw == 12 && per_wave == 2) { FIRA_T32W(2, 12) }
    if (nw == 8 && per_wave == 2) { FIRA_T32W(2, 8) }
    if (nw == 8 && per_wave == 4) { FIRA_T32W(4, 8) }
    return set_err("gemm_tile32: unsupported shape K = %d on %d waves", K, nw);
#undef FIRA_T32W
}

bool gemm_tile32_takes(int tB, int M, int N, int K, const float* A, int lda, const float* B, int ldb) {
    if (M <= 0 || N <= 0) return false;
    if (K % 128 != 0 || lda % 4 != 0 || ((uintptr_t)A % 16) != 0 || ldb % 4 != 0 || ((uintptr_t)B % 16) != 0) return false;
    const int nch = K / 128;
    if (nch != 1 && nch != 2 && nch != 3 && nch != 4 && nch != 6 && nch != 8) return false;
    if (!tB && N % 32 != 0) return false;
    return true;
}

bool gemm_tile32_try(hipStream_t s, int tB, int M, int N, int K, const float* A, int lda, const float* B, int ldb,
                     float* C, int ldc, const float* bias, int flags, int* rc, const int32_t* c_rows,
                     const float* relu_mask, const int32_t* a_rows, const EpiRes* er_in) {
    if (!gemm_tile32_takes(tB, M, N, K, A, lda, B, ldb)) return false;
    const EpiRes er = er_in ? *er_in : EpiRes();
    const int nch = K / 128;
    const int tiles_n = cdiv(N, 32);
    const dim3 grid(cdiv(M, 32) * tiles_n);
    {
        const int nw = tile32_waves(K, (int)grid.x);
        if (nw > 4) {
            *rc = tile32_launch_wide(s, nw, K, tB, grid, M, N, A, lda, B, ldb, C, ldc, bias, flags, c_rows, relu_mask, a_rows, tiles_n, er);
            return true;
        }
    }
#define FIRA_T32(NCH)                                                                                                  \
    case NCH:                                                                                                          \
        if (tB) tile32_launch<true, NCH>(s, grid, M, N, A, lda, B, ldb, C, ldc, bias, flags, c_rows, relu_mask, a_rows, tiles_n, er); \
        else tile32_launch<false, NCH>(s, grid, M, N, A, lda, B, ldb, C, ldc, bias, flags, c_rows, relu_mask, a_rows, tiles_n, er); \
        break;
    switch (nch) { FIRA_T32(1) FIRA_T32(2) FIRA_T32(3) FIRA_T32(4) FIRA_T32(6) FIRA_T32(8) }
#undef FIRA_T32
    hipError_t e = hipGetLastError();
    *rc = e != hipSuccess ? set_err("gemm_tile32: %s", hipGetErrorString(e)) : 0;
    return true;
}

bool gemm_tile32_ln_try(hipStream_t s, int M, int N, const float* S, int lds, const float* W, const float* bias, float* Y,
                        int ldy, int flags, const float* gamma, const float* beta, float* x_out, float* stats_out, int* rc) {
    if (!gemm_tile32_takes(1, M, N, FIRA_D, S, lds, W, FIRA_D)) return false;
    if (((uintptr_t)gamma % 16) || ((uintptr_t)beta % 16) || ((uintptr_t)x_out % 16)) return false;
    ProfScope prof(s, PROF_GEMM, 2.0 * M * N * (double)FIRA_D, 4.0 * ((double)M * FIRA_D + (double)N * FIRA_D + (double)M * N));
    const int tiles_n = cdiv(N, 32);
    LnA ln;
    ln.gamma = gamma; ln.beta = beta; ln.x_out = x_out; ln.stats_out = stats_out;
    hipLaunchKernelGGL((gemm_tile32_kernel<true, 2, true, false>), dim3(cdiv(M, 32) * tiles_n), dim3(256), 0, s, M, N, S, lds, W, FIRA_D,
                       Y, ldy, bias, flags & 3, (const int32_t*)nullptr, (const float*)nullptr, (const int32_t*)nullptr, tiles_n,
                       EpiRes(), ln, LnB());
    hipError_t e = hipGetLastError();
    *rc = e != hipSuccess ? set_err("gemm_tile32_ln: %s", hipGetErrorString(e)) : 0;
    return true;
}

int gemm_tile32_lnb_blocks(int M) { return cdiv(M, 32); }
bool gemm_tile32_lnb_try(hipStream_t s, int M, int N, const float* dy, const float* W, int ldw, float* dX, int lddx,
                         const float* relu_mask, const float* sum, const float* stats, const float* gamma, float* ds,
                         float* dx_drop, float* part, float dropout, uint64_t seed, uint32_t site, int* rc, uint32_t idx0) {
    if (!gemm_tile32_takes(0, M, N, FIRA_D, dy, FIRA_D, W, ldw)) return false;
    if (((uintptr_t)sum % 16) || ((uintptr_t)gamma % 16) || ((uintptr_t)ds % 16) || ((uintptr_t)dx_drop % 16) || ds == dy) return false;
    ProfScope prof(s, PROF_GEMM, 2.0 * M * N * (double)FIRA_D, 4.0 * ((double)M * FIRA_D + (double)N * FIRA_D + (double)M * N));
    const int tiles_n = cdiv(N, 32);
    LnB lb;
    lb.sum = sum; lb.stats = stats; lb.gamma = gamma; lb.ds = ds; lb.dx = dx_drop; lb.part = part;
    lb.p = dropout; lb.inv_keep = dropout > 0.f ? 1.0f / (1.0f - dropout) : 1.0f; lb.seed = seed; lb.site = site; lb.idx0 = idx0;
    hipLaunchKernelGGL((gemm_tile32_kernel<false, 2, false, true>), dim3(cdiv(M, 32) * tiles_n), dim3(256), 0, s, M, N, dy, FIRA_D, W, ldw,
                       dX, lddx, (const float*)nullptr, 0, (const int32_t*)nullptr, relu_mask, (const int32_t*)nullptr, tiles_n,
                       EpiRes(), LnA(), lb);
    hipError_t e = hipGetLastError();
    *rc = e != hipSuccess ? set_err("gemm_tile32_lnb: %s", hipGetErrorString(e)) : 0;
    return true;
}

struct UnfoldGemm { const float *A, *B; float* C; int a_rs, a_ks, b_rs, b_ks, mode; };
struct UnfoldGemmTable { int n = 0; UnfoldGemm e[32]; };
__global__ __launch_bounds__(256) void unfold_gemm_kernel(const UnfoldGemmTable tab) {
    __shared__ float red[4][1024];
    const UnfoldGemm& q = tab.e[blockIdx.y];
    const int lane = threadIdx.x & 63, wave = threadIdx.x >> 6;
    const int l31 = lane & 31, kh = lane >> 5;
    if (q.mode == 2) {
        if (blockIdx.x >= 8) return;
        const f32x4 x = *reinterpret_cast<const f32x4*>(q.B + lane * 4);
        f32x4 a[8];
#pragma unroll
        for (int r = 0; r < 8; ++r)
            a[r] = *reinterpret_cast<const f32x4*>(q.A + (size_t)(blockIdx.x * 32 + wave * 8 + r) * q.a_rs + lane * 4);
#pragma unroll
        for (int r = 0; r < 8; ++r) {
            const float d = wave_sum((a[r].x * x.x + a[r].y * x.y) + (a[r].z * x.z + a[r].w * x.w));
            if (lane == 0) q.C[blockIdx.x * 32 + wave * 8 + r] = d;
        }
        return;
    }
    const int m0 = (blockIdx.x >> 3) * 32, n0 = (blockIdx.x & 7) * 32;
    const float* pa = q.A + (size_t)(m0 + l31) * q.a_rs;
    const float* pb = q.B + (size_t)(n0 + l31) * q.b_rs;
    f32x16 acc;
#pragma unroll
    for (int r = 0; r < 16; ++r) acc[r] = 0.f;
    float a[2][16], b[2][16];
#pragma unroll
    for (int u = 0; u < 2; ++u) {
        const int k0 = (wave + 4 * u) * 32 + kh * 16;
        if (q.a_ks == 1) {
#pragma unroll
            for (int v = 0; v < 4; ++v) {
                const f32x4 x = *reinterpret_cast<const f32x4*>(pa + k0 + 4 * v);
                a[u][4 * v] = x.x; a[u][4 * v + 1] = x.y; a[u][4 * v + 2] = x.z; a[u][4 * v + 3] = x.w;
            }
        } else {
#pragma unroll
            for (int t = 0; t < 16; ++t) a[u][t] = pa[(size_t)(k0 + t) * q.a_ks];
        }
        if (q.b_ks == 1) {
#pragma unroll
            for (int v = 0; v < 4; ++v) {
                const f32x4 x = *reinterpret_cast<const f32x4*>(pb + k0 + 4 * v);
                b[u][4 * v] = x.x; b[u][4 * v + 1] = x.y; b[u][4 * v + 2] = x.z; b[u][4 * v + 3] = x.w;
            }
        } else {
#pragma unroll
            for (int t = 0; t < 16; ++t) b[u][t] = pb[(size_t)(k0 + t) * q.b_ks];
        }
    }
#pragma unroll
    for (int u = 0; u < 2; ++u)
#pragma unroll
        for (int t = 0; t < 16; ++t) acc = __builtin_amdgcn_mfma_f32_32x32x2f32(a[u][t], b[u][t], acc, 0, 0, 0);
#pragma unroll
    for (int r = 0; r < 16; ++r) red[wave][r * 64 + lane] = acc[r];
    __syncthreads();
#pragma unroll
    for (int i = 0; i < 4; ++i) {
        const int idx = threadIdx.x + 256 * i;
        const int r = idx >> 6, ln = idx & 63;
        const int row = m0 + (r & 3) + 8 * (r >> 2) + 4 * (ln >> 5), col = n0 + (ln & 31);
        float* pc = q.C + (size_t)row * FIRA_D + col;
        const float v = (red[0][idx] + red[1][idx]) + (red[2][idx] + red[3][idx]);
        if (q.mode == 0) *pc += v;
        else *pc = v;
    }
}
int gcn_unfold_products(hipStream_t s, int n_layers, const float* const* dW21, const float* const* W1, const float* const* W2,
                        float* const* dW1, float* const* dW2) {
    if (n_layers <= 0) return 0;
    if (n_layers > 16) return set_err("gcn_unfold_products: %d layers", n_layers);
    UnfoldGemmTable tab;
    for (int l = 0; l < n_layers; ++l) {
        tab.e[tab.n++] = UnfoldGemm{dW21[l], W1[l], dW2[l], FIRA_D, 1, FIRA_D, 1, 0};
        tab.e[tab.n++] = UnfoldGemm{W2[l], dW21[l], dW1[l], 1, FIRA_D, 1, FIRA_D, 0};
    }
    ProfScope prof(s, PROF_GEMM, 2.0 * tab.n * FIRA_D * (double)FIRA_D * FIRA_D, 4.0 * tab.n * 3.0 * FIRA_D * FIRA_D);
    hipLaunchKernelGGL(unfold_gemm_kernel, dim3(64, tab.n), dim3(256), 0, s, tab);
    hipError_t e = hipGetLastError();
    return e != hipSuccess ? set_err("gcn_unfold_products: %s", hipGetErrorString(e)) : 0;
}

int gcn_fold_weights(hipStream_t s, int n_layers, const float* const* W2, const float* const* W1, const float* const* b1,
                     float* W21, float* W21t, float* c21) {
    if (n_layers <= 0) return 0;
    if (n_layers > 10) return set_err("gcn_fold_weights: %d layers", n_layers);
    UnfoldGemmTable tab;
    for (int l = 0; l < n_layers; ++l) {
        float* w = W21 + (size_t)l * FIRA_D * FIRA_D;
        tab.e[tab.n++] = UnfoldGemm{W2[l], W1[l], w, FIRA_D, 1, 1, FIRA_D, 1};
        if (W21t)
            tab.e[tab.n++] = UnfoldGemm{W1[l], W2[l], W21t + (size_t)l * FIRA_D * FIRA_D, 1, FIRA_D, FIRA_D, 1, 1};
        tab.e[tab.n++] = UnfoldGemm{W2[l], b1[l], c21 + (size_t)l * FIRA_D, FIRA_D, 1, 0, 0, 2};
    }
    ProfScope prof(s, PROF_GEMM, 2.0 * n_layers * (W21t ? 2 : 1) * FIRA_D * (double)FIRA_D * FIRA_D, 4.0 * tab.n * 3.0 * FIRA_D * FIRA_D);
    hipLaunchKernelGGL(unfold_gemm_kernel, dim3(64, tab.n), dim3(256), 0, s, tab);
    hipError_t e = hipGetLastError();
    return e != hipSuccess ? set_err("gcn_fold_weights: %s", hipGetErrorString(e)) : 0;
}

bool gemm_small_try(hipStream_t s, int tA, int tB, int M, int N, int K, const float* A, int lda, const float* B, int ldb,
                    float* C, int ldc, const float* bias, int flags, int* rc, const int32_t* c_rows,
                    const float* relu_mask) {
    *rc = 0;
    constexpr long max_tiles = 1024;
    const long tiles = (long)cdiv(M, 32) * cdiv(N, 32);
    if (tA || (M > 64 && tiles > max_tiles) || K % 32 != 0 || K < 64 || lda % 4 != 0 || ((uintptr_t)A % 16) != 0) return false;
    if (tB && (ldb % 4 != 0 || ((uintptr_t)B % 16) != 0)) return false;
    if (gemm_tile32_try(s, tB, M, N, K, A, lda, B, ldb, C, ldc, bias, flags, rc, c_rows, relu_mask, nullptr, nullptr))
        return true;
    dim3 grid(cdiv(N, 32), cdiv(M, 32));
    if (tB) hipLaunchKernelGGL(gemm_small_kernel<true>, grid, dim3(256), 0, s, M, N, K, A, lda, B, ldb, C, ldc, bias, flags, c_rows, relu_mask);
    else hipLaunchKernelGGL(gemm_small_kernel<false>, grid, dim3(256), 0, s, M, N, K, A, lda, B, ldb, C, ldc, bias, flags, c_rows, relu_mask);
    hipError_t e = hipGetLastError();
    if (e != hipSuccess) *rc = set_err("gemm_small: %s", hipGetErrorString(e));
    return true;
}

}

extern "C" {
int fira_linear_presum_f32(void* stream, int M, int K, const float* X, int ldx, const float* W, const float* bias,
                           const float* res, float* sum, float dropout, uint64_t seed, uint32_t stream_id) {
    FIRA_REQUIRE(X && W && res && sum && M > 0, "fira_linear_presum_f32: bad argument");
    FIRA_REQUIRE(dropout >= 0.f && dropout < 1.f, "fira_linear_presum_f32: dropout must be in [0,1)");
    fira::EpiRes er;
    er.res = res; er.ldr = FIRA_D; er.p = dropout; er.inv_keep = dropout > 0.f ? 1.0f / (1.0f - dropout) : 1.0f;
    er.seed = seed; er.site = stream_id;
    int rc = 0;
    if (!fira::gemm_tile32_try((hipStream_t)stream, 1, M, FIRA_D, K, X, ldx, W, K, sum, FIRA_D, bias, 0, &rc, nullptr, nullptr,
                               nullptr, &er))
        return fira::set_err("fira_linear_presum_f32: shape %d x 256 x %d / alignment not taken by the tile kernel", M, K);
    return rc;
}
int fira_ln_bwd_linear_f32(void* stream, int M, int N, const float* dy, const float* Wt, float* dX, const float* relu_mask,
                           const float* sum, const float* stats, const float* gamma, float* ds, float* dx_drop, float* dgamma,
                           float* dbeta, float* part, float dropout, uint64_t seed, uint32_t site) {
    FIRA_REQUIRE(dy && Wt && dX && sum && stats && gamma && ds && dx_drop && dgamma && dbeta && part && M > 0 && N > 0,
                 "fira_ln_bwd_linear_f32: bad argument");
    FIRA_REQUIRE(ds != dy, "fira_ln_bwd_linear_f32: ds must not alias dy");
    FIRA_REQUIRE(dropout >= 0.f && dropout < 1.f, "fira_ln_bwd_linear_f32: dropout must be in [0,1)");
    int rc = 0;
    if (!fira::gemm_tile32_lnb_try((hipStream_t)stream, M, N, dy, Wt, N, dX, N, relu_mask, sum, stats, gamma, ds, dx_drop, part,
                                   dropout, seed, site, &rc))
        return fira::set_err("fira_ln_bwd_linear_f32: shape %d x %d / alignment not taken by the tile kernel", M, N);
    if (rc) return rc;
    fira::RedTable tab;
    const int nb = fira::gemm_tile32_lnb_blocks(M);
    tab.e[0] = fira::RedEntry{dgamma, part, FIRA_D, nb, 2 * FIRA_D};
    tab.e[1] = fira::RedEntry{dbeta, part + FIRA_D, FIRA_D, nb, 2 * FIRA_D};
    tab.n = 2;
    return fira::deferred_reduce((hipStream_t)stream, tab);
}
int fira_ln_linear_f32(void* stream, int M, int N, const float* S, int lds, const float* W, const float* bias, float* Y,
                       int ldy, int relu, const float* gamma, const float* beta, float* x_out, float* stats_out) {
    FIRA_REQUIRE(S && W && Y && gamma && beta && x_out && M > 0 && N > 0, "fira_ln_linear_f32: bad argument");
    int rc = 0;
    if (!fira::gemm_tile32_ln_try((hipStream_t)stream, M, N, S, lds, W, bias, Y, ldy, relu ? FIRA_GEMM_RELU : 0, gamma, beta, x_out,
                                  stats_out, &rc))
        return fira::set_err("fira_ln_linear_f32: shape %d x %d / alignment not taken by the tile kernel", M, N);
    return rc;
}
}
```

### fira_icse_amd/ops.py

```python
from __future__ import annotations

import dataclasses

import torch

from . import _lib
from ._lib import check, cur_stream, ptr


def _f32(t):
    assert t.is_cuda and t.dtype == torch.float32 and t.is_contiguous(), "expected a contiguous fp32 CUDA tensor"
    return t


def _i32(t):
    assert t.is_cuda and t.dtype == torch.int32 and t.is_contiguous(), "expected a contiguous int32 CUDA tensor"
    return t


def gemm(A, B, *, transA=False, transB=True, bias=None, relu=False, out=None, accumulate=False, splitk=1,
         tile=0, dtype="f32"):
    for t in (A, B):
        assert t.is_cuda and t.dtype == torch.float32 and t.dim() == 2 and t.stride(1) == 1
    M, K = (A.shape[1], A.shape[0]) if transA else A.shape
    N = B.shape[0] if transB else B.shape[1]
    assert (B.shape[1] if transB else B.shape[0]) == K
    if out is None:
        out = torch.zeros((M, N), dtype=torch.float32, device=A.device) if accumulate else \
            torch.empty((M, N), dtype=torch.float32, device=A.device)
    flags = (1 if relu else 0) | (2 if accumulate else 0) | (tile << 4)
    fn = _lib.lib().fira_gemm_bf16 if dtype == "bf16" else _lib.lib().fira_gemm_f32
    check(fn(cur_stream(), int(transA), int(transB), M, N, K, ptr(A), A.stride(0), ptr(B), B.stride(0), ptr(out),
             out.stride(0), ptr(bias), flags, splitk), "fira_gemm_%s" % dtype)
    return out


def weight_shadow(W):
    rows, cols = W.shape
    wb = torch.empty((rows, cols), dtype=torch.int16, device=W.device)
    wbt = torch.empty((cols, rows), dtype=torch.int16, device=W.device)
    check(_lib.lib().fira_weight_shadow(cur_stream(), rows, cols, ptr(_f32(W)), ptr(wb), ptr(wbt)), "fira_weight_shadow")
    return wb, wbt


def gemm_wb(A, Bb, *, bias=None, relu=False, out=None, accumulate=False, splitk=1):
    M, K = A.shape
    N = Bb.shape[0]
    assert Bb.shape[1] == K and Bb.dtype == torch.int16 and Bb.stride(1) == 1
    if out is None:
        out = (torch.zeros if accumulate else torch.empty)((M, N), dtype=torch.float32, device=A.device)
    flags = (1 if relu else 0) | (2 if accumulate else 0)
    check(_lib.lib().fira_gemm_bf16_wb(cur_stream(), M, N, K, ptr(A), A.stride(0), ptr(Bb), Bb.stride(0), ptr(out),
                                       out.stride(0), ptr(bias), flags, splitk), "fira_gemm_bf16_wb")
    return out


def csr_spmm(rowptr, col, val, X, graph_rows=0, variant=0, out=None, dtype=0, auto=False):
    for t in (X,) + ((out,) if out is not None else ()):
        assert t.is_cuda and t.dtype == torch.float32 and t.dim() == 2 and t.stride(1) == 1
    Y = torch.empty_like(X, memory_format=torch.contiguous_format) if out is None else out
    assert Y.shape == X.shape
    if auto or variant >= 3:
        check(_lib.lib().fira_csr_spmm(cur_stream(), X.shape[0], int(col.numel()), ptr(_i32(rowptr)), ptr(_i32(col)),
                                       ptr(_f32(val)), ptr(X), X.stride(0), ptr(Y), Y.stride(0), graph_rows, variant, dtype),
              "fira_csr_spmm")
        return Y
    check(_lib.lib().fira_csr_spmm_f32(cur_stream(), X.shape[0], ptr(_i32(rowptr)), ptr(_i32(col)), ptr(_f32(val)),
                                       ptr(X), X.stride(0), ptr(Y), Y.stride(0), graph_rows, variant),
          "fira_csr_spmm_f32")
    return Y


def embed_gather(idx, table, pos=None, out=None, out_bstride=None, out_off=0):
    B, L = idx.shape
    if out is None:
        out = torch.empty((B, L, 256), dtype=torch.float32, device=table.device)
        out_bstride = L
    check(_lib.lib().fira_embed_gather_fwd(cur_stream(), B, L, ptr(_i32(idx)), ptr(_f32(table)), ptr(pos), ptr(out),
                                           out_bstride, out_off), "fira_embed_gather_fwd")
    return out


def embed_scatter_add(idx, dtable, dout, out_bstride, out_off, padding_idx):
    B, L = idx.shape
    check(_lib.lib().fira_embed_gather_bwd(cur_stream(), B, L, ptr(_i32(idx)), ptr(_f32(dtable)), ptr(_f32(dout)),
                                           out_bstride, out_off, padding_idx), "fira_embed_gather_bwd")
    return dtable


def combination_fwd(qk, vtab, mark, dropout=0.0, seed=0, site=0):
    M = qk.shape[0]
    out = torch.empty((M, 256), dtype=torch.float32, device=qk.device)
    check(_lib.lib().fira_combination_fwd(cur_stream(), M, ptr(_f32(qk)), ptr(_f32(vtab)), ptr(_i32(mark)), ptr(out),
                                          dropout, seed, site), "fira_combination_fwd")
    return out


def combination_bwd(qk, vtab, mark, dout, dropout=0.0, seed=0, site=0):
    M = qk.shape[0]
    dqk = torch.empty_like(qk)
    dvtab = torch.zeros_like(vtab)
    check(_lib.lib().fira_combination_bwd(cur_stream(), M, ptr(_f32(qk)), ptr(_f32(vtab)), ptr(_i32(mark)),
                                          ptr(_f32(dout)), ptr(dqk), ptr(dvtab), dropout, seed, site),
          "fira_combination_bwd")
    return dqk, dvtab


def add_layernorm_fwd(x, res, gamma, beta, dropout=0.0, seed=0, site=0):
    M = x.shape[0]
    y = torch.empty_like(x)
    stats = torch.empty((M, 2), dtype=torch.float32, device=x.device)
    check(_lib.lib().fira_add_layernorm_fwd(cur_stream(), M, ptr(_f32(x)), ptr(res), ptr(_f32(gamma)), ptr(_f32(beta)),
                                            ptr(y), ptr(stats), dropout, seed, site), "fira_add_layernorm_fwd")
    return y, x, stats


def linear_presum(x, w, bias, res, dropout=0.0, seed=0, site=0):
    M, K = x.shape
    assert w.shape == (256, K) and x.stride(1) == 1
    s = torch.empty((M, 256), dtype=torch.float32, device=x.device)
    check(_lib.lib().fira_linear_presum_f32(cur_stream(), M, K, ptr(x), x.stride(0), ptr(_f32(w)), ptr(bias), ptr(_f32(res)),
                                            ptr(s), dropout, seed, site), "fira_linear_presum_f32")
    return s


def ln_linear(s, w, bias, gamma, beta, relu=False):
    M = s.shape[0]
    N = w.shape[0]
    assert w.shape[1] == 256 and s.shape[1] == 256 and s.stride(1) == 1
    y = torch.empty((M, N), dtype=torch.float32, device=s.device)
    x = torch.empty((M, 256), dtype=torch.float32, device=s.device)
    stats = torch.empty((M, 2), dtype=torch.float32, device=s.device)
    check(_lib.lib().fira_ln_linear_f32(cur_stream(), M, N, ptr(s), s.stride(0), ptr(_f32(w)), ptr(bias), ptr(y), N, int(relu),
                                        ptr(_f32(gamma)), ptr(_f32(beta)), ptr(x), ptr(stats)), "fira_ln_linear_f32")
    return y, x, stats


def linear_layernorm_bf16_fwd(x, wb, bias, res, gamma, beta, dropout=0.0, seed=0, site=0):
    M, K = x.shape
    assert K == 256 and wb.shape == (256, 256) and wb.dtype == torch.int16 and x.stride(1) == 1
    y = torch.empty((M, 256), dtype=torch.float32, device=x.device)
    s = torch.empty_like(y)
    stats = torch.empty((M, 2), dtype=torch.float32, device=x.device)
    check(_lib.lib().fira_linear_layernorm_bf16_fwd(cur_stream(), M, ptr(x), x.stride(0), ptr(wb), wb.stride(0), ptr(bias),
                                                    ptr(res), ptr(_f32(gamma)), ptr(_f32(beta)), ptr(s), ptr(y), ptr(stats),
                                                    dropout, seed, site), "fira_linear_layernorm_bf16_fwd")
    return y, s, stats


def add_layernorm_bwd(dy, s, stats, gamma, dropout=0.0, seed=0, site=0, want_dx_drop=False):
    M = dy.shape[0]
    ds = torch.empty_like(dy)
    dxd = torch.empty_like(dy) if want_dx_drop else None
    dg = torch.zeros(256, dtype=torch.float32, device=dy.device)
    db = torch.zeros(256, dtype=torch.float32, device=dy.device)
    check(_lib.lib().fira_add_layernorm_bwd(cur_stream(), M, ptr(_f32(dy)), ptr(_f32(s)), ptr(_f32(stats)),
                                            ptr(_f32(gamma)), ptr(ds), ptr(dxd), ptr(dg), ptr(db), dropout, seed, site),
          "fira_add_layernorm_bwd")
    return ds, dxd, dg, db


def ln_bwd_linear(dy, Wt, summ, stats, gamma, relu_mask=None, dropout=0.0, seed=0, site=0):
    M, N = dy.shape[0], Wt.shape[1]
    dX = torch.empty((M, N), dtype=torch.float32, device=dy.device)
    ds, dxd = torch.empty_like(dy), torch.empty_like(dy)
    dg = torch.zeros(256, dtype=torch.float32, device=dy.device)
    db = torch.zeros(256, dtype=torch.float32, device=dy.device)
    part = torch.empty(((M + 31) // 32) * 512, dtype=torch.float32, device=dy.device)
    check(_lib.lib().fira_ln_bwd_linear_f32(cur_stream(), M, N, ptr(_f32(dy)), ptr(_f32(Wt)), ptr(dX),
                                            ptr(None if relu_mask is None else _f32(relu_mask)), ptr(_f32(summ)),
                                            ptr(_f32(stats)), ptr(_f32(gamma)), ptr(ds), ptr(dxd), ptr(dg), ptr(db), ptr(part),
                                            dropout, seed, site), "fira_ln_bwd_linear_f32")
    return dX, ds, dxd, dg, db


def dropout_mask(seed, site, n, p, device="cuda"):
    out = torch.empty(n, dtype=torch.float32, device=device)
    check(_lib.lib().fira_dropout_mask(cur_stream(), seed, site, n, p, ptr(out)), "fira_dropout_mask")
    return out


def colsum(X):
    out = torch.zeros(X.shape[1], dtype=torch.float32, device=X.device)
    check(_lib.lib().fira_colsum_f32(cur_stream(), X.shape[0], X.shape[1], ptr(_f32(X)), X.stride(0), ptr(out)),
          "fira_colsum_f32")
    return out


def gcn_weight_planes(B):
    B = _f32(B).contiguous()
    n = B.numel() // (256 * 256)
    planes = torch.empty(n * 3 * 256 * 256, dtype=torch.int16, device=B.device)
    check(_lib.lib().fira_gcn_weight_planes(cur_stream(), n, ptr(B), ptr(planes)), "fira_gcn_weight_planes")
    return planes


def linear_x3(x, W, bias=None, dtype=2, ldo=None):
    x = _f32(x)
    M, N = x.shape[0], W.shape[0]
    planes = gcn_weight_planes(W)
    ldo = N if ldo is None else ldo
    out = torch.zeros((M, ldo), dtype=torch.float32, device=x.device)
    check(_lib.lib().fira_linear_x3(cur_stream(), M, N, ptr(x), x.stride(0), ptr(planes), ptr(None if bias is None else _f32(bias)),
                                    ptr(out), ldo, dtype), "fira_linear_x3")
    return out[:, :N]


def linear_dgrad_x3(dy, W, dx=None, dtype=2):
    assert dy.is_cuda and dy.dtype == torch.float32 and dy.stride(1) == 1
    M, K = dy.shape
    Wt = _f32(W).view(K // 256, 256, 256).transpose(1, 2).contiguous()
    planes = gcn_weight_planes(Wt)
    acc = dx is not None
    if dx is None:
        dx = torch.empty((M, 256), dtype=torch.float32, device=dy.device)
    check(_lib.lib().fira_linear_dgrad_x3(cur_stream(), M, K, ptr(dy), dy.stride(0), ptr(planes), ptr(dx), dx.stride(0), 1 if acc else 0,
                                          dtype), "fira_linear_dgrad_x3")
    return dx


def dgrad_x3_splitk(dy, W, dx, dtype=2):
    assert dy.is_cuda and dy.dtype == torch.float32 and dy.stride(1) == 1
    M, K = dy.shape
    ws = torch.empty(_lib.lib().fira_dgrad_x3_splitk_planes_bytes(K), dtype=torch.uint8, device=dy.device)
    check(_lib.lib().fira_dgrad_x3_splitk(cur_stream(), M, K, ptr(dy), dy.stride(0), ptr(_f32(W)), ptr(ws), ptr(dx), dx.stride(0),
                                          dtype), "fira_dgrad_x3_splitk")
    return dx


def gcn_layer_fwd(rowptr, col, val, X, W21t, bias, c21, gamma, beta, dropout=0.0, seed=0, site=0, dtype=0, want_rowsum=True):
    n = X.shape[0]
    if dtype >= 2:
        W21t = gcn_weight_planes(_f32(W21t).t().contiguous())
    else:
        W21t = _f32(W21t)
    summ, y = torch.empty_like(X), torch.empty_like(X)
    stats = torch.empty((n, 2), dtype=torch.float32, device=X.device)
    rs = torch.empty(n, dtype=torch.float32, device=X.device) if want_rowsum else None
    check(_lib.lib().fira_gcn_layer_fwd(cur_stream(), n, ptr(_i32(rowptr)), ptr(_i32(col)), ptr(_f32(val)), ptr(_f32(X)),
                                        ptr(W21t), ptr(_f32(bias)), ptr(_f32(c21)), ptr(_f32(gamma)), ptr(_f32(beta)),
                                        ptr(summ), ptr(y), ptr(stats), ptr(rs), dropout, seed, site, dtype),
          "fira_gcn_layer_fwd")
    return summ, y, stats, rs


def combination_block_fwd(Xc, Wqk, bqk, Wo, bo, vtab, mark, gamma, beta, dropout=0.0, seed=0, site_gate=0, site_out=0, y=None,
                          y_rows=None, dtype=0):
    n = Xc.shape[0]
    dev = Xc.device
    assert vtab.is_cuda and vtab.dtype == torch.float32 and vtab.stride(1) == 1 and vtab.shape[0] == 4, "vtab: fp32 rows"
    if dtype >= 2:
        WqT = WkT = WoT = gcn_weight_planes(torch.cat([_f32(Wqk), _f32(Wo)], 0))
    else:
        WqT, WkT, WoT = (_f32(Wqk[:256]).t().contiguous(), _f32(Wqk[256:]).t().contiguous(), _f32(Wo).t().contiguous())
    qk = torch.empty((n, 512), dtype=torch.float32, device=dev)
    c, summ = torch.empty_like(Xc), torch.empty_like(Xc)
    if y is None:
        y = torch.empty_like(Xc)
    stats = torch.empty((n, 2), dtype=torch.float32, device=dev)
    yr = None if y_rows is None else _i32(y_rows)
    check(_lib.lib().fira_combination_block_fwd(cur_stream(), n, ptr(_f32(Xc)), ptr(WqT), ptr(WkT), ptr(WoT), ptr(_f32(bqk)),
                                                ptr(_f32(bo)), ptr(vtab), vtab.stride(0), ptr(_i32(mark)), ptr(qk), ptr(c),
                                                ptr(_f32(gamma)), ptr(_f32(beta)), ptr(summ), ptr(y), ptr(yr), ptr(stats),
                                                dropout, seed, site_gate, site_out, dtype), "fira_combination_block_fwd")
    return qk, c, summ, y, stats


def combination_block_bwd(dG, rows, summ, stats, gamma, Wo, Wqk, qk, vtab, mark, dropout=0.0, seed=0, site_gate=0, site_out=0,
                          dtype=0):
    n = summ.shape[0]
    dev = summ.device
    assert vtab.is_cuda and vtab.dtype == torch.float32 and vtab.stride(1) == 1 and vtab.shape[0] == 4, "vtab: fp32 rows"
    dYc = torch.empty((n, 256), dtype=torch.float32, device=dev)
    dqk = torch.empty((n, 512), dtype=torch.float32, device=dev)
    dgamma, dbeta = torch.zeros(256, device=dev), torch.zeros(256, device=dev)
    dvtab = torch.zeros((4, 256), device=dev)
    part = torch.empty(_lib.lib().fira_combination_block_bwd_part_floats(), dtype=torch.float32, device=dev)
    if dtype >= 2:
        Wo = gcn_weight_planes(torch.stack([_f32(Wqk[:256]).t(), _f32(Wqk[256:]).t(), _f32(Wo).t()]).contiguous())
    else:
        Wo = _f32(Wo)
    check(_lib.lib().fira_combination_block_bwd(cur_stream(), n, ptr(_f32(dG)), ptr(_i32(rows)), ptr(_f32(summ)), ptr(_f32(stats)),
                                                ptr(_f32(gamma)), ptr(Wo), ptr(_f32(Wqk)), ptr(_f32(qk)), ptr(vtab),
                                                vtab.stride(0), ptr(_i32(mark)), ptr(dYc), ptr(dqk), ptr(dgamma), ptr(dbeta),
                                                ptr(dvtab), 256, ptr(part), dropout, seed, site_gate, site_out, dtype),
          "fira_combination_block_bwd")
    return dYc, dqk, dgamma, dbeta, dvtab


def gcn_layer_bwd(rowptr, col, val, dY, W21, dX, dtype=0):
    V = torch.empty_like(dY)
    W = gcn_weight_planes(_f32(W21).t().contiguous()) if dtype >= 2 else _f32(W21)
    check(_lib.lib().fira_gcn_layer_bwd(cur_stream(), dY.shape[0], ptr(_i32(rowptr)), ptr(_i32(col)), ptr(_f32(val)),
                                        ptr(_f32(dY)), ptr(W), ptr(V), ptr(_f32(dX)), dtype), "fira_gcn_layer_bwd")
    return V


def attention_ragged_fwd(q, k, v, key_valid, q_off, Tq, Tk, causal=False, self_kv=False, dtype=0, heads=8, k_off=None):
    B = q_off.numel() - 1
    o = torch.zeros_like(q)
    ko = None if k_off is None else _i32(k_off)
    check(_lib.lib().fira_attention_fwd_ex(cur_stream(), B, heads, Tq, Tk, ptr(q), q.stride(0), ptr(k), k.stride(0), ptr(v),
                                           v.stride(0), ptr(_i32(key_valid)), int(causal), 0, ptr(o), 256, ptr(_i32(q_off)),
                                           int(self_kv), dtype, ptr(ko)), "fira_attention_fwd_ex")
    return o


def attention_ragged_bwd(q, k, v, key_valid, o, do, q_off, Tq, Tk, causal=False, self_kv=False, dtype=0, heads=8, k_off=None,
                         fill=0.0):
    B = q_off.numel() - 1
    dq, dk, dv = torch.full_like(q, fill), torch.full_like(k, fill), torch.full_like(v, fill)
    ko = None if k_off is None else _i32(k_off)
    check(_lib.lib().fira_attention_bwd_ex(cur_stream(), B, heads, Tq, Tk, ptr(q), q.stride(0), ptr(k), k.stride(0), ptr(v),
                                           v.stride(0), ptr(_i32(key_valid)), int(causal), 0, ptr(_f32(o)), 256,
                                           ptr(_f32(do)), 256, ptr(dq), dq.stride(0), ptr(dk), dk.stride(0), ptr(dv),
                                           dv.stride(0), ptr(_i32(q_off)), int(self_kv), dtype, ptr(ko)),
          "fira_attention_bwd_ex")
    return dq, dk, dv


def attention_fwd(q, k, v, key_valid, causal=False, q_pos0=0, heads=8):
    B, Tq, _ = q.shape
    Tk = k.shape[1]
    o = torch.empty((B, Tq, 256), dtype=torch.float32, device=q.device)
    check(_lib.lib().fira_attention_fwd(cur_stream(), B, heads, Tq, Tk, ptr(q), q.stride(1), ptr(k), k.stride(1),
                                        ptr(v), v.stride(1), ptr(_i32(key_valid)), int(causal), q_pos0, ptr(o), 256),
          "fira_attention_fwd")
    return o


def decode_attention(q, k, v, key_valid, tk=None, qpk=1, heads=8, knew=None, vnew=None, k_off=None):
    BR = q.shape[0]
    if k_off is not None:
        kb = kvb = tk
        ldk, ldv = k.stride(0), v.stride(0)
    else:
        kb, kvb = k.shape[1], key_valid.shape[1]
        ldk, ldv = k.stride(1), v.stride(1)
    tk = kb if tk is None else tk
    o = torch.empty((BR, 256), dtype=torch.float32, device=q.device)
    ko = None if k_off is None else _i32(k_off)
    check(_lib.lib().fira_decode_attention(cur_stream(), BR, heads, tk, ptr(q), q.stride(0), ptr(k), ldk, ptr(v),
                                           ldv, ptr(_i32(key_valid)), ptr(o), 256, kb, kvb, qpk, ptr(knew),
                                           ptr(vnew), knew.stride(0) if knew is not None else 0,
                                           ptr(k) if knew is not None else None, ptr(v) if knew is not None else None,
                                           ptr(ko)),
          "fira_decode_attention")
    return o


def attention_bwd(q, k, v, key_valid, o, do, causal=False, q_pos0=0, heads=8):
    B, Tq, _ = q.shape
    Tk = k.shape[1]
    dq = torch.empty((B, Tq, 256), dtype=torch.float32, device=q.device)
    dk = torch.empty((B, Tk, 256), dtype=torch.float32, device=q.device)
    dv = torch.empty((B, Tk, 256), dtype=torch.float32, device=q.device)
    check(_lib.lib().fira_attention_bwd(cur_stream(), B, heads, Tq, Tk, ptr(q), q.stride(1), ptr(k), k.stride(1),
                                        ptr(v), v.stride(1), ptr(_i32(key_valid)), int(causal), q_pos0, ptr(_f32(o)),
                                        256, ptr(_f32(do)), 256, ptr(dq), 256, ptr(dk), 256, ptr(dv), 256),
          "fira_attention_bwd")
    return dq, dk, dv


def copy_score_fwd(src, tgt, w, bias):
    B, S, _ = src.shape
    T = tgt.shape[1]
    score = torch.empty((B, T, S), dtype=torch.float32, device=src.device)
    check(_lib.lib().fira_copy_score_fwd(cur_stream(), B, T, S, ptr(_f32(src)), ptr(_f32(tgt)), ptr(_f32(w)),
                                         ptr(_f32(bias)), ptr(score)), "fira_copy_score_fwd")
    return score


def copy_score_bwd(src, tgt, w, dscore):
    B, S, _ = src.shape
    T = tgt.shape[1]
    dsrc = torch.empty_like(src)
    dtgt = torch.zeros_like(tgt)
    dw = torch.zeros(256, dtype=torch.float32, device=src.device)
    db = torch.zeros(1, dtype=torch.float32, device=src.device)
    check(_lib.lib().fira_copy_score_bwd(cur_stream(), B, T, S, ptr(_f32(src)), ptr(_f32(tgt)), ptr(_f32(w)),
                                         ptr(_f32(dscore)), ptr(dsrc), ptr(dtgt), ptr(dw), ptr(db)),
          "fira_copy_score_bwd")
    return dsrc, dtgt, dw, db


def head_loss(logits, score, mem_valid, gate_logits, tar_label, V, compact_row=None, want_grad=True, argmax=False):
    B, T = tar_label.shape
    S = score.shape[-1]
    loss = torch.zeros(1, dtype=torch.float32, device=logits.device)
    ntok = torch.zeros(1, dtype=torch.int32, device=logits.device)
    ids = torch.empty((B, T), dtype=torch.int32, device=logits.device) if argmax else None
    check(_lib.lib().fira_head_loss(cur_stream(), B * T, T, V, S, ptr(compact_row), ptr(_f32(logits)),
                                    logits.stride(0), ptr(_f32(score)), ptr(_i32(mem_valid)), ptr(_f32(gate_logits)),
                                    ptr(_i32(tar_label)), ptr(loss), ptr(ntok), ptr(ids), int(want_grad)),
          "fira_head_loss")
    return loss, ntok, ids


def copy_score_fwd_ex(src, tgt, w, bias, score, T, qpk=1, mem_valid=None, tar_label=None, V=0, t_off=None):
    S = src.shape[1]
    B = src.shape[0] * qpk
    opt = lambda t: None if t is None else _i32(t)
    check(_lib.lib().fira_copy_score_fwd_ex(cur_stream(), B, T, S, ptr(_f32(src)), ptr(_f32(tgt)), ptr(_f32(w)),
                                            ptr(_f32(bias)), ptr(_f32(score)), qpk, ptr(opt(mem_valid)), ptr(opt(tar_label)),
                                            V, ptr(opt(t_off))), "fira_copy_score_fwd_ex")
    return score


def copy_score_bwd_blocks(B, S):
    n = _lib.lib().fira_copy_score_bwd_blocks(B, S)
    if n < 0:
        check(n, "fira_copy_score_bwd_blocks")
    return n


def copy_part_stride():
    return _lib.lib().fira_copy_part_stride()


def copy_score_bwd_ex(src, tgt, w, dscore, dsrc, dtgt, dw, dbias, T, mem_valid=None, part=None, t_off=None):
    B, S = src.shape[0], src.shape[1]
    opt = lambda t: None if t is None else _i32(t)
    optf = lambda t: None if t is None else _f32(t)
    check(_lib.lib().fira_copy_score_bwd_ex(cur_stream(), B, T, S, ptr(_f32(src)), ptr(_f32(tgt)), ptr(_f32(w)),
                                            ptr(_f32(dscore)), ptr(_f32(dsrc)), ptr(_f32(dtgt)), ptr(optf(dw)),
                                            ptr(optf(dbias)), ptr(opt(mem_valid)), ptr(optf(part)), ptr(opt(t_off))),
          "fira_copy_score_bwd_ex")


def head_loss_ex(logits, score, mem_valid, gate_logits, tar_label, V, compact_row=None, row_bt=None, want_grad=True,
                 argmax=False):
    B, T = tar_label.shape
    R, S = score.shape
    loss = torch.zeros(1, dtype=torch.float32, device=logits.device)
    ntok = torch.zeros(1, dtype=torch.int32, device=logits.device)
    ids = torch.empty(R, dtype=torch.int32, device=logits.device) if argmax else None
    opt = lambda t: None if t is None else _i32(t)
    check(_lib.lib().fira_head_loss_ex(cur_stream(), R, T, V, S, ptr(opt(compact_row)), ptr(_f32(logits)), logits.stride(0),
                                       ptr(_f32(score)), ptr(_i32(mem_valid)), ptr(_f32(gate_logits)), ptr(_i32(tar_label)),
                                       ptr(loss), ptr(ntok), ptr(ids), int(want_grad), ptr(opt(row_bt))),
          "fira_head_loss_ex")
    return loss, ntok, ids


def deferred_reduce_max():
    return _lib.lib().fira_deferred_reduce_max()


def deferred_reduce(entries):
    arr = (_lib.RedEntry * max(len(entries), 1))()
    for i, (dst, src, width, n_part, stride) in enumerate(entries):
        assert dst.is_cuda and src.is_cuda and dst.dtype == src.dtype == torch.float32
        arr[i] = _lib.RedEntry(dst.data_ptr(), src.data_ptr(), width, n_part, stride)
    check(_lib.lib().fira_deferred_reduce(cur_stream(), len(entries), arr), "fira_deferred_reduce")


def rows_move(mode, R, W, out, ld_out, inp, ld_in, src=None, dst=None):
    opt = lambda t: None if t is None else _i32(t)
    assert out.is_cuda and inp.is_cuda and out.dtype == inp.dtype == torch.float32
    check(_lib.lib().fira_rows_move(cur_stream(), mode, R, W, ptr(out), ld_out, ptr(inp), ld_in, ptr(opt(src)),
                                    ptr(opt(dst))), "fira_rows_move")


def rank2_rows(g, w):
    out = torch.empty((g.shape[0], 256), dtype=torch.float32, device=g.device)
    check(_lib.lib().fira_rank2_rows(cur_stream(), g.shape[0], ptr(_f32(g)), ptr(_f32(w)), ptr(out)), "fira_rank2_rows")
    return out


def colsum_weighted(X, N, out, row_weight=None):
    check(_lib.lib().fira_colsum_weighted(cur_stream(), X.shape[0], N, ptr(_f32(X)), X.stride(0), ptr(_f32(out)),
                                          ptr(None if row_weight is None else _f32(row_weight))), "fira_colsum_weighted")
    return out


def embed_rows_fwd(row_bt, idx, table, pos):
    R, T = row_bt.numel(), idx.shape[1]
    out = torch.empty((R, 256), dtype=torch.float32, device=table.device)
    check(_lib.lib().fira_embed_rows_fwd(cur_stream(), R, T, ptr(_i32(row_bt)), ptr(_i32(idx)), ptr(_f32(table)),
                                         ptr(_f32(pos)), ptr(out)), "fira_embed_rows_fwd")
    return out


def embed_rows_bwd(row_bt, idx, dtable, dout, padding_idx=0):
    check(_lib.lib().fira_embed_rows_bwd(cur_stream(), row_bt.numel(), ptr(_i32(row_bt)), ptr(_i32(idx)), ptr(_f32(dtable)),
                                         ptr(_f32(dout)), padding_idx), "fira_embed_rows_bwd")
    return dtable


def embed_grouped_bwd(item_tok, item_ptr, rows, dtable, dnode):
    check(_lib.lib().fira_embed_grouped_bwd(cur_stream(), item_tok.numel(), ptr(_i32(item_tok)), ptr(_i32(item_ptr)),
                                            ptr(_i32(rows)), ptr(_f32(dtable)), ptr(_f32(dnode))), "fira_embed_grouped_bwd")
    return dtable


def embed_list_bwd_small(rows, ids, dtable, dnode):
    check(_lib.lib().fira_embed_list_bwd_small(cur_stream(), rows.numel(), ptr(_i32(rows)), ptr(_i32(ids)), ptr(_f32(dtable)),
                                               ptr(_f32(dnode)), dtable.shape[0]), "fira_embed_list_bwd_small")
    return dtable


def embed_scatter_add_small(idx, dtable, dout, out_bstride, out_off, padding_idx):
    B, L = idx.shape
    check(_lib.lib().fira_embed_gather_bwd_small(cur_stream(), B, L, ptr(_i32(idx)), ptr(_f32(dtable)), ptr(_f32(dout)),
                                                 out_bstride, out_off, padding_idx, dtable.shape[0]),
          "fira_embed_gather_bwd_small")
    return dtable


def adam_step(p, g, m, v, lr, step, beta1=0.9, beta2=0.999, eps=1e-8, inv_scale=None):
    check(_lib.lib().fira_adam_step(cur_stream(), p.numel(), ptr(_f32(p)), ptr(_f32(g)), ptr(_f32(m)), ptr(_f32(v)),
                                    lr, beta1, beta2, eps, step, ptr(inv_scale)), "fira_adam_step")


def adam_step_count(p, g, m, v, lr, step, count, beta1=0.9, beta2=0.999, eps=1e-8):
    check(_lib.lib().fira_adam_step_count(cur_stream(), p.numel(), ptr(_f32(p)), ptr(_f32(g)), ptr(_f32(m)), ptr(_f32(v)),
                                          lr, beta1, beta2, eps, step, ptr(_f32(count))), "fira_adam_step_count")


def pack_stats(loss_sum, n_tok, out2):
    check(_lib.lib().fira_pack_stats(cur_stream(), ptr(_f32(loss_sum)), ptr(_i32(n_tok)), ptr(_f32(out2))), "fira_pack_stats")
    return out2


ACCUM_MAX = 64


def accum_check(k):
    if k is None:
        return 1
    if isinstance(k, bool) or not isinstance(k, int) or not 1 <= k <= ACCUM_MAX:
        raise ValueError("accum steps %r: must be an integer in [1, %d]" % (k, ACCUM_MAX))
    return int(k)


def accum_split(lo: int, hi: int, k: int):
    k = accum_check(k)
    n = max(hi - lo, 0)
    size = -(-n // k)
    return [(min(lo + i * size, hi), min(lo + (i + 1) * size, hi)) for i in range(k)]


def accum_stats(loss_sum, n_tok, stats, n_tok_total, first: bool):
    check(_lib.lib().fira_accum_stats(cur_stream(), ptr(_f32(loss_sum)), ptr(_i32(n_tok)), ptr(_f32(stats)),
                                      ptr(_i32(n_tok_total)), 1 if first else 0), "fira_accum_stats")
    return stats


def adam_step_mb(p, g0, g1, m, v, lr, step, n_tok0, n_tok1=None, beta1=0.9, beta2=0.999, eps=1e-8):
    check(_lib.lib().fira_adam_step_mb(cur_stream(), p.numel(), ptr(_f32(p)), ptr(_f32(g0)), ptr(g1), ptr(_f32(m)),
                                       ptr(_f32(v)), lr, beta1, beta2, eps, step, ptr(_i32(n_tok0)), ptr(n_tok1)),
          "fira_adam_step_mb")


def ema_check(decay, every):
    try:
        ok = 0.0 < float(decay) < 1.0
    except (TypeError, ValueError):
        ok = False
    if not ok:
        raise ValueError("ema decay %r: must be a number in (0, 1)" % (decay,))
    if isinstance(every, bool) or not isinstance(every, int) or every < 1:
        raise ValueError("ema cadence %r: must be an integer >= 1" % (every,))
    return float(decay), int(every)


def ema_weight(decay: float, every: int = 1) -> float:
    import numpy as np
    decay, every = ema_check(decay, every)
    return float(np.float32(1.0 - decay ** every))


def ema_update(ema, p, w: float):
    assert ema.numel() == p.numel(), "ema and p differ in length"
    check(_lib.lib().fira_ema_update(cur_stream(), ema.numel(), ptr(_f32(ema)), ptr(_f32(p)), float(w)), "fira_ema_update")
    return ema


LR_KINDS = ("constant", "inv_sqrt", "cosine", "linear")


@dataclasses.dataclass(frozen=True)
class LrSchedule:
    kind: str = "constant"
    base_lr: float = 1e-4
    warmup_steps: int = 0
    decay_steps: int = 0
    min_lr: float = 0.0

    @staticmethod
    def make(obj) -> "LrSchedule":
        if isinstance(obj, LrSchedule):
            s = obj
        else:
            d = dict(obj)
            unknown = set(d) - {f.name for f in dataclasses.fields(LrSchedule)}
            if unknown:
                raise ValueError("lr_schedule: unknown field(s) %s" % sorted(unknown))
            s = LrSchedule(**d)
        kind = s.kind
        if isinstance(kind, int) and not isinstance(kind, bool) and 0 <= kind < len(LR_KINDS):
            kind = LR_KINDS[kind]
        kind = str(kind).replace("-", "_")
        if kind not in LR_KINDS:
            raise ValueError("lr_schedule: kind %r is not one of %s" % (s.kind, ", ".join(LR_KINDS)))
        s = LrSchedule(kind, float(s.base_lr), int(s.warmup_steps), int(s.decay_steps), float(s.min_lr))
        lr_schedule_check(s)
        return s

    def struct(self) -> "_lib.LrSchedule":
        return _lib.LrSchedule(LR_KINDS.index(self.kind), self.base_lr, self.warmup_steps, self.decay_steps, self.min_lr)

    def as_dict(self) -> dict:
        return dataclasses.asdict(self)


def _sched_struct(sched):
    return sched if isinstance(sched, _lib.LrSchedule) else sched.struct()


def lr_at(sched, step: int) -> float:
    import ctypes as C
    return float(_lib.lib().fira_lr_at(C.byref(_sched_struct(sched)), int(step)))


def lr_schedule_check(sched):
    import ctypes as C
    lib = _lib.lib()
    if lib.fira_lr_schedule_check(C.byref(_sched_struct(sched))) != 0:
        raise ValueError(lib.fira_last_error().decode())


def clip_state(device="cuda"):
    state = torch.zeros(16, dtype=torch.int32, device=device)
    scratch = torch.zeros(_lib.lib().fira_grad_sqsum_scratch_bytes() // 8, dtype=torch.float64, device=device)
    return state, scratch


def read_clip_state(state):
    st = _lib.ClipState.from_buffer_copy(state.cpu().numpy().tobytes())
    return {"sq": list(st.sq), "norm": st.norm, "coef": st.coef, "zero_flag": st.zero_flag, "n_clipped": st.n_clipped,
            "n_nonfinite": st.n_nonfinite}


def grad_sqsum_depth(n: int) -> int:
    n4 = n // 4
    slice4 = -(-(-(-n4 // 1024)) // 1024) * 1024
    return slice4 // 1024 + 12


def grad_sqsum(g, state, slot, scratch):
    assert g.dtype == torch.float32 and g.is_contiguous()
    check(_lib.lib().fira_grad_sqsum(cur_stream(), g.numel(), ptr(g), ptr(state), slot, ptr(scratch)), "fira_grad_sqsum")


def clip_finish(state, n_slots, max_norm, n_tok=None, count=None):
    check(_lib.lib().fira_clip_finish(cur_stream(), ptr(state), n_slots, ptr(n_tok), ptr(count), max_norm), "fira_clip_finish")


def adam_step_clip(p, g, m, v, lr, step, state, n_tok=None, count=None, beta1=0.9, beta2=0.999, eps=1e-8):
    check(_lib.lib().fira_adam_step_clip(cur_stream(), p.numel(), ptr(_f32(p)), ptr(_f32(g)), ptr(_f32(m)), ptr(_f32(v)), lr,
                                         beta1, beta2, eps, step, ptr(n_tok), ptr(count), ptr(state)), "fira_adam_step_clip")


def inv_count(n_tok, out):
    check(_lib.lib().fira_inv_count(cur_stream(), ptr(_i32(n_tok)), ptr(_f32(out))), "fira_inv_count")
    return out


def f32_to_bf16(src, dst):
    n = src.numel()
    assert dst.numel() == n and dst.dtype == torch.bfloat16 and src.dtype == torch.float32 and n % 4 == 0
    check(_lib.lib().fira_f32_to_bf16(cur_stream(), n, ptr(src), ptr(dst)), "fira_f32_to_bf16")
    return dst


def bf16_to_f32(src, dst):
    n = src.numel()
    assert dst.numel() == n and src.dtype == torch.bfloat16 and dst.dtype == torch.float32 and n % 4 == 0
    check(_lib.lib().fira_bf16_to_f32(cur_stream(), n, ptr(src), ptr(dst)), "fira_bf16_to_f32")
    return dst


def ffn_fwd(x, w1, b1, w2, b2, gamma, beta, dropout=0.0, seed=0, site=0, dtype=0):
    M, F = x.shape[0], w1.shape[0]
    h = torch.empty((M, F), dtype=torch.float32, device=x.device)
    summ, y = torch.empty_like(x), torch.empty_like(x)
    stats = torch.empty((M, 2), dtype=torch.float32, device=x.device)
    check(_lib.lib().fira_ffn_fwd(cur_stream(), M, F, ptr(_f32(x)), ptr(_f32(w1)), ptr(_f32(b1)), ptr(_f32(w2)), ptr(_f32(b2)),
                                  ptr(_f32(gamma)), ptr(_f32(beta)), ptr(h), ptr(summ), ptr(y), ptr(stats), dropout, seed, site,
                                  dtype), "fira_ffn_fwd")
    return h, summ, y, stats


def ffn_bwd(dy, x, h, summ, stats, w1, w2, gamma, dropout=0.0, seed=0, site=0, dtype=0):
    M, F = x.shape[0], w1.shape[0]
    dev = x.device
    z = lambda *s: torch.zeros(s, dtype=torch.float32, device=dev)
    dx, dyf, dh = torch.empty_like(x), torch.empty_like(x), torch.empty((M, F), dtype=torch.float32, device=dev)
    dw1, db1, dw2, db2, dg, db = z(F, 256), z(F), z(256, F), z(256), z(256), z(256)
    check(_lib.lib().fira_ffn_bwd(cur_stream(), M, F, ptr(_f32(dy)), ptr(_f32(x)), ptr(_f32(h)), ptr(_f32(summ)), ptr(_f32(stats)),
                                  ptr(_f32(w1)), ptr(_f32(w2)), ptr(_f32(gamma)), ptr(dx), ptr(dyf), ptr(dh), ptr(dw1), ptr(db1),
                                  ptr(dw2), ptr(db2), ptr(dg), ptr(db), dropout, seed, site, dtype), "fira_ffn_bwd")
    return dx, dw1, db1, dw2, db2, dg, db


def head_topk(x, wout, bout, k, dtype=0):
    R, V = x.shape[0], wout.shape[0]
    ldl = (V + 63) // 64 * 64
    logits = torch.empty((R, ldl), dtype=torch.float32, device=x.device)
    ids = torch.empty((R, k), dtype=torch.int32, device=x.device)
    vals = torch.empty((R, k), dtype=torch.float32, device=x.device)
    check(_lib.lib().fira_head_topk(cur_stream(), R, V, k, ptr(_f32(x)), ptr(_f32(wout)), ptr(_f32(bout)), ptr(logits), ldl,
                                    ptr(ids), ptr(vals), dtype), "fira_head_topk")
    return ids, vals, logits[:, :V]


def head_logits_x3(x, wout, bout):
    R, V = x.shape[0], wout.shape[0]
    ldl = (V + 63) // 64 * 64
    logits = torch.empty((R, ldl), dtype=torch.float32, device=x.device)
    scratch = torch.empty(_lib.lib().fira_head_logits_x3_scratch_bytes(R), dtype=torch.uint8, device=x.device)
    x = _f32(x)
    check(_lib.lib().fira_head_logits_x3(cur_stream(), R, V, ptr(x), x.stride(0), ptr(_f32(wout)), ptr(_f32(bout)), ptr(logits), ldl,
                                         ptr(scratch)), "fira_head_logits_x3")
    return logits[:, :V]


_panel_scratch = {}


def gemm_wgrad_panel(A, B, out, colsum=None, dtype=0, split=True):
    K, M, N = A.shape[0], out.shape[0], out.shape[1]
    assert B.shape[0] == K and B.shape[1] == N and A.stride(1) == 1 and B.stride(1) == 1 and out.stride(1) == 1
    scratch = None
    if split:
        scratch = _panel_scratch.get(A.device)
        if scratch is None:
            scratch = _panel_scratch[A.device] = torch.empty(256 * 65536, dtype=torch.float32, device=A.device)
    check(_lib.lib().fira_gemm_wgrad_panel(cur_stream(), dtype, M, N, K, ptr(A), A.stride(0), ptr(B), B.stride(0), ptr(out),
                                           out.stride(0), ptr(colsum), ptr(scratch), scratch.numel() if split else 0),
          "fira_gemm_wgrad_panel")
    return out


def dev_bleu_stats(ids, sou, sub_token, tar, V, hyp=None, stats=None):
    B, T = ids.shape
    L, S = sou.shape[1], sub_token.shape[1]
    assert sou.shape[0] == B and sub_token.shape[0] == B and tuple(tar.shape) == (B, T)
    if hyp is None:
        hyp = torch.empty((B, T), dtype=torch.int32, device=ids.device)
    if stats is None:
        stats = torch.empty((B, 12), dtype=torch.int32, device=ids.device)
    assert tuple(hyp.shape) == (B, T) and tuple(stats.shape) == (B, 12)
    check(_lib.lib().fira_dev_bleu_stats(cur_stream(), B, T, int(V), L, S, ptr(_i32(ids)), ptr(_i32(sou)), ptr(_i32(sub_token)),
                                         ptr(_i32(tar)), ptr(_i32(hyp)), ptr(_i32(stats))), "fira_dev_bleu_stats")
    return hyp, stats


def mbr_bleu_stats(tokens, length, stats=None):
    B, n, T = tokens.shape
    assert tuple(length.shape) == (B, n)
    if stats is None:
        stats = torch.empty((B, n, n, 12), dtype=torch.int32, device=tokens.device)
    assert tuple(stats.shape) == (B, n, n, 12)
    check(_lib.lib().fira_mbr_bleu_stats(cur_stream(), B, n, T, ptr(_i32(tokens)), ptr(_i32(length)), ptr(_i32(stats))),
          "fira_mbr_bleu_stats")
    return stats


def dev_rouge_l_stats(ids, sou, sub_token, tar, V, stats=None):
    B, T = ids.shape
    L, S = sou.shape[1], sub_token.shape[1]
    assert sou.shape[0] == B and sub_token.shape[0] == B and tuple(tar.shape) == (B, T)
    if stats is None:
        stats = torch.empty((B, 4), dtype=torch.int32, device=ids.device)
    assert tuple(stats.shape) == (B, 4)
    check(_lib.lib().fira_dev_rouge_l_stats(cur_stream(), B, T, int(V), L, S, ptr(_i32(ids)), ptr(_i32(sou)), ptr(_i32(sub_token)),
                                            ptr(_i32(tar)), ptr(_i32(stats))), "fira_dev_rouge_l_stats")
    return stats


def mbr_rouge_l_stats(tokens, length, stats=None):
    B, n, T = tokens.shape
    assert tuple(length.shape) == (B, n)
    if stats is None:
        stats = torch.empty((B, n, n, 4), dtype=torch.int32, device=tokens.device)
    assert tuple(stats.shape) == (B, n, n, 4)
    check(_lib.lib().fira_mbr_rouge_l_stats(cur_stream(), B, n, T, ptr(_i32(tokens)), ptr(_i32(length)), ptr(_i32(stats))),
          "fira_mbr_rouge_l_stats")
    return stats


def dev_meteor_stats(ids, sou, sub_token, tar, V, classes=None, stats=None):
    B, T = ids.shape
    L, S = sou.shape[1], sub_token.shape[1]
    assert sou.shape[0] == B and sub_token.shape[0] == B and tuple(tar.shape) == (B, T)
    assert classes is None or tuple(classes.shape) == (int(V),)
    if stats is None:
        stats = torch.empty((B, 4), dtype=torch.int32, device=ids.device)
    assert tuple(stats.shape) == (B, 4)
    check(_lib.lib().fira_dev_meteor_stats(cur_stream(), B, T, int(V), L, S, ptr(_i32(ids)), ptr(_i32(sou)), ptr(_i32(sub_token)),
                                           ptr(_i32(tar)), None if classes is None else ptr(_i32(classes)), ptr(_i32(stats))),
          "fira_dev_meteor_stats")
    return stats


def mbr_meteor_stats(tokens, length, classes=None, stats=None):
    B, n, T = tokens.shape
    assert tuple(length.shape) == (B, n)
    assert classes is None or classes.dim() == 1
    if stats is None:
        stats = torch.empty((B, n, n, 4), dtype=torch.int32, device=tokens.device)
    assert tuple(stats.shape) == (B, n, n, 4)
    check(_lib.lib().fira_mbr_meteor_stats(cur_stream(), B, n, T, ptr(_i32(tokens)), ptr(_i32(length)),
                                           0 if classes is None else classes.shape[0],
                                           None if classes is None else ptr(_i32(classes)), ptr(_i32(stats))),
          "fira_mbr_meteor_stats")
    return stats


def pool_memory(dims, mem, mem_valid, out=None):
    B = mem.shape[0]
    assert mem.dim() == 3 and tuple(mem_valid.shape) == tuple(mem.shape[:2]) and mem.shape[2] == 256
    assert mem.shape[1] == dims.sou_len + dims.sub_len
    if out is None:
        out = torch.empty((B, 256), dtype=torch.float32, device=mem.device)
    assert tuple(out.shape) == (B, 256)
    import ctypes as C
    check(_lib.lib().fira_pool_memory(cur_stream(), C.byref(dims), B, ptr(_f32(mem)), ptr(_i32(mem_valid)), ptr(_f32(out))),
          "fira_pool_memory")
    return out


def nn_search(Q, store, exclude=None, scratch=None):
    B, N = Q.shape[0], store.shape[0]
    assert Q.dim() == 2 and store.dim() == 2 and Q.shape[1] == 256 and store.shape[1] == 256
    assert exclude is None or tuple(exclude.shape) == (B,)
    lib = _lib.lib()
    need = lib.fira_nn_search_scratch_bytes(B, N)
    if scratch is None:
        scratch = torch.empty(max(need, 8), dtype=torch.uint8, device=Q.device)
    idx = torch.empty(B, dtype=torch.int32, device=Q.device)
    sim = torch.empty(B, dtype=torch.float32, device=Q.device)
    check(lib.fira_nn_search(cur_stream(), ptr(_f32(Q)), B, ptr(_f32(store)), N, None if exclude is None else ptr(_i32(exclude)),
                             ptr(idx), ptr(sim), ptr(scratch), scratch.numel()), "fira_nn_search")
    return idx, sim


def mix_neighbour(dims, rows_per_commit, coef, q, dist, best=False):
    R = dist.shape[0]
    assert tuple(q.shape) == tuple(dist.shape) and coef.numel() == 2 * (R // max(rows_per_commit, 1))
    import ctypes as C
    bid = torch.empty(R, dtype=torch.int32, device=dist.device) if best else None
    bp = torch.empty(R, dtype=torch.float32, device=dist.device) if best else None
    check(_lib.lib().fira_mix_neighbour(cur_stream(), C.byref(dims), R, rows_per_commit, ptr(_f32(coef)), ptr(q), ptr(dist),
                                        ptr(bid), ptr(bp)), "fira_mix_neighbour")
    return (bid, bp) if best else dist
```

### include/fira_hip.h

```cpp
#ifndef FIRA_HIP_H
#define FIRA_HIP_H

#include <stddef.h>
#include <stdint.h>

#ifdef __cplusplus
extern "C" {
#endif

#define FIRA_ABI_VERSION 11

typedef struct fira_dims {
    int32_t sou_len;
    int32_t sub_len;
    int32_t ast_len;
    int32_t tar_len;
    int32_t d_model;
    int32_t n_head;
    int32_t n_layer;
    int32_t vocab;
    int32_t ast_vocab;
    int32_t d_ff;
} fira_dims;

typedef struct fira_batch {
    int32_t B;
    int32_t nnz;
    const int32_t* sou;
    const int32_t* tar;
    const int32_t* mark;
    const int32_t* ast_change;
    const int32_t* tar_label;
    const int32_t* sub_token;
    int32_t n_nodes;
    const int32_t* node_rows;
    const int32_t* rowptr;
    const int32_t* col;
    const float*   val;
    int32_t n_code;
    const int32_t* code_rows;
    const int32_t* code_mark;
    int32_t n_mem;
    const int32_t* mem_rows;
    const int32_t* mem_dst;
    const int32_t* head_rows;
    int32_t n_head_rows;
    int32_t n_emb_items;
    const int32_t* emb_item_tok;
    const int32_t* emb_item_ptr;
    const int32_t* emb_rows;
    int32_t n_ast_items;
    const int32_t* ast_rows;
    const int32_t* ast_ids;
    const int32_t* dec_off;
    int32_t n_dec_rows;
    const int32_t* dec_off_host;
} fira_batch;

typedef struct fira_train_opts {
    float    dropout;
    float    gcn_dropout;
    uint64_t seed;
    int32_t  compact_head;
    int32_t  dtype;
    int32_t  compact_dec;
    int32_t  zero_grads;
} fira_train_opts;
#define FIRA_F32 0
#define FIRA_BF16 1
#define FIRA_F32X3 2
#define FIRA_BF16X1 3

const char* fira_last_error(void);
int         fira_abi_version(void);

int    fira_param_count(const fira_dims* d);
int    fira_param_info(const fira_dims* d, int index, char* name_buf, int64_t* offset, int64_t* numel,
                       int32_t* ndim, int64_t shape[2]);
int64_t fira_param_total(const fira_dims* d);
int    fira_param_groups(const fira_dims* d, int64_t* split, int64_t* live);

size_t fira_workspace_bytes(const fira_dims* d, int B, int mode);
size_t fira_decode_workspace_bytes(const fira_dims* d, int B, int n_beam);
size_t fira_decode_workspace_bytes_ex(const fira_dims* d, int B, int n_beam, int flags);

#define FIRA_PROF_NCLASS 7
void fira_prof_enable(int on);
int  fira_prof_report(int n_class, double* ms, double* work, double* bytes, int64_t* count);


#define FIRA_GEMM_RELU 1
#define FIRA_GEMM_ACCUM 2
#define FIRA_GEMM_TILE_SHIFT 4
int fira_gemm_f32(void* stream, int transA, int transB, int M, int N, int K,
                  const float* A, int lda, const float* B, int ldb, float* C, int ldc,
                  const float* bias, int flags, int splitk);
int fira_gemm_bf16(void* stream, int transA, int transB, int M, int N, int K,
                   const float* A, int lda, const float* B, int ldb, float* C, int ldc,
                   const float* bias, int flags, int splitk);

int fira_weight_shadow(void* stream, int rows, int cols, const float* W, uint16_t* Wb, uint16_t* WbT);
int fira_gemm_bf16_wb(void* stream, int M, int N, int K, const float* A, int lda, const uint16_t* Bb, int ldb,
                      float* C, int ldc, const float* bias, int flags, int splitk);

int fira_csr_spmm_f32(void* stream, int n_rows, const int32_t* rowptr, const int32_t* col, const float* val,
                      const float* X, int ldx, float* Y, int ldy, int graph_rows, int variant);
int fira_csr_spmm(void* stream, int n_rows, int64_t nnz, const int32_t* rowptr, const int32_t* col, const float* val,
                  const float* X, int ldx, float* Y, int ldy, int graph_rows, int variant, int dtype);

int fira_gcn_layer_fwd(void* stream, int n_rows, const int32_t* rowptr, const int32_t* col, const float* val,
                       const float* X, const float* W21t, const float* bias, const float* c21, const float* gamma,
                       const float* beta, float* sum, float* y, float* stats, float* rowsum_out, float dropout,
                       uint64_t seed, uint32_t site, int dtype);
int fira_gcn_layer_bwd(void* stream, int n_rows, const int32_t* rowptr, const int32_t* col, const float* val,
                       const float* dY, const float* W21, float* V, float* dX, int dtype);
int fira_gcn_weight_planes(void* stream, int n_mats, const float* B, uint16_t* planes);
int fira_linear_x3(void* stream, int M, int N, const float* x, int ldx, const uint16_t* w_planes, const float* bias, float* out,
                   int ldo, int dtype);
int fira_linear_dgrad_x3(void* stream, int M, int K, const float* dy, int lddy, const uint16_t* wt_planes, float* dx, int lddx,
                         int accumulate, int dtype);
size_t fira_dgrad_x3_splitk_planes_bytes(int K);
int fira_dgrad_x3_splitk(void* stream, int M, int K, const float* dy, int lddy, const float* W, uint16_t* planes_ws, float* dx,
                         int lddx, int dtype);

int fira_combination_block_fwd(void* stream, int n_rows, const float* Xc, const float* WqT, const float* WkT,
                               const float* WoT, const float* bqk, const float* bo, const float* vtab, int ldv,
                               const int32_t* mark, float* qk, float* c, const float* gamma, const float* beta, float* sum,
                               float* y, const int32_t* y_rows, float* stats, float dropout, uint64_t seed,
                               uint32_t site_gate, uint32_t site_out, int dtype);

int fira_combination_block_bwd(void* stream, int n_rows, float* dG, const int32_t* rows, const float* sum, const float* stats,
                               const float* gamma, const float* Wo, const float* Wqk, const float* qk, const float* vtab,
                               int ldv, const int32_t* mark, float* dYc, float* dqk, float* dgamma, float* dbeta,
                               float* dvtab, int lddv, float* part, float dropout, uint64_t seed, uint32_t site_gate,
                               uint32_t site_out, int dtype);
int fira_combination_block_bwd_part_floats(void);

int fira_embed_gather_fwd(void* stream, int B, int L, const int32_t* idx, const float* table,
                          const float* pos, float* out, int out_bstride, int out_off);
int fira_embed_gather_bwd(void* stream, int B, int L, const int32_t* idx, float* dtable,
                          const float* dout, int out_bstride, int out_off, int padding_idx);

int fira_combination_fwd(void* stream, int M, const float* qk, const float* vtab, const int32_t* mark,
                         float* out, float dropout, uint64_t seed, uint32_t stream_id);
int fira_combination_bwd(void* stream, int M, const float* qk, const float* vtab, const int32_t* mark,
                         const float* dout, float* dqk, float* dvtab ,
                         float dropout, uint64_t seed, uint32_t stream_id);

int fira_add_layernorm_fwd(void* stream, int M, float* x, const float* res, const float* gamma,
                           const float* beta, float* y, float* stats, float dropout, uint64_t seed,
                           uint32_t stream_id);
int fira_linear_presum_f32(void* stream, int M, int K, const float* X, int ldx, const float* W, const float* bias,
                           const float* res, float* sum, float dropout, uint64_t seed, uint32_t stream_id);
int fira_ln_linear_f32(void* stream, int M, int N, const float* S, int lds, const float* W, const float* bias, float* Y,
                       int ldy, int relu, const float* gamma, const float* beta, float* x_out, float* stats_out);
int fira_ln_bwd_linear_f32(void* stream, int M, int N, const float* dy, const float* Wt, float* dX, const float* relu_mask,
                           const float* sum, const float* stats, const float* gamma, float* ds, float* dx_drop,
                           float* dgamma, float* dbeta, float* part, float dropout, uint64_t seed, uint32_t site);
int fira_linear_layernorm_bf16_fwd(void* stream, int M, const float* X, int ldx, const uint16_t* Wb, int ldb,
                                   const float* bias, const float* res, const float* gamma, const float* beta,
                                   float* sum, float* y, float* stats, float dropout, uint64_t seed,
                                   uint32_t stream_id);
int fira_add_layernorm_bwd(void* stream, int M, const float* dy, const float* sum, const float* stats,
                           const float* gamma, float* ds, float* dx_drop, float* dgamma, float* dbeta,
                           float dropout, uint64_t seed, uint32_t stream_id);

#define FIRA_SITE_GATE 0
#define FIRA_SITE_COMB_OUT 1
#define FIRA_SITE_GCN 2
#define FIRA_SITE_SELF 3
#define FIRA_SITE_CROSS 4
#define FIRA_SITE_FFN 5
#define FIRA_SITE(layer, kind) ((uint32_t)((layer) * 8 + (kind) + 1))
int fira_dropout_mask(void* stream, uint64_t seed, uint32_t site, int64_t n, float p, float* out);

int fira_colsum_f32(void* stream, int M, int N, const float* X, int ldx, float* out);

int fira_attention_fwd(void* stream, int B, int H, int Tq, int Tk, const float* Q, int ldq,
                       const float* K, int ldk, const float* V, int ldv, const int32_t* key_valid,
                       int causal, int q_pos0, float* O, int ldo);
int fira_attention_bwd(void* stream, int B, int H, int Tq, int Tk, const float* Q, int ldq,
                       const float* K, int ldk, const float* V, int ldv, const int32_t* key_valid,
                       int causal, int q_pos0, const float* O, int ldo, const float* dO, int lddo,
                       float* dQ, int lddq, float* dK, int lddk, float* dV, int lddv);
int fira_attention_fwd_ex(void* stream, int B, int H, int Tq, int Tk, const float* Q, int ldq,
                          const float* K, int ldk, const float* V, int ldv, const int32_t* key_valid,
                          int causal, int q_pos0, float* O, int ldo, const int32_t* q_off, int self_kv, int dtype,
                          const int32_t* k_off);
int fira_attention_bwd_ex(void* stream, int B, int H, int Tq, int Tk, const float* Q, int ldq,
                          const float* K, int ldk, const float* V, int ldv, const int32_t* key_valid,
                          int causal, int q_pos0, const float* O, int ldo, const float* dO, int lddo,
                          float* dQ, int lddq, float* dK, int lddk, float* dV, int lddv,
                          const int32_t* q_off, int self_kv, int dtype, const int32_t* k_off);

int fira_decode_attention(void* stream, int BR, int H, int Tk, const float* Q, int ldq, const float* K, int ldk,
                          const float* V, int ldv, const int32_t* key_valid, float* O, int ldo, int kb, int kvb, int qpk,
                          const float* Knew, const float* Vnew, int ldn, float* Kc_out, float* Vc_out,
                          const int32_t* k_off);

int fira_copy_score_fwd(void* stream, int B, int T, int S, const float* src, const float* tgt,
                        const float* w, const float* bias, float* score);
int fira_copy_score_bwd(void* stream, int B, int T, int S, const float* src, const float* tgt,
                        const float* w, const float* dscore, float* dsrc , float* dtgt ,
                        float* dw , float* dbias );

int fira_head_loss(void* stream, int BT, int T, int V, int S, const int32_t* compact_row,
                   float* logits, int ldl, float* score , const int32_t* mem_valid ,
                   float* gate_logits , const int32_t* tar_label ,
                   float* loss_sum, int32_t* n_tok, int32_t* argmax_out, int want_grad);

int fira_copy_score_fwd_ex(void* stream, int B, int T, int S, const float* src, const float* tgt, const float* w,
                           const float* bias, float* score, int qpk, const int32_t* mem_valid, const int32_t* tar_label,
                           int V, const int32_t* t_off);
int fira_copy_score_bwd_ex(void* stream, int B, int T, int S, const float* src, const float* tgt, const float* w,
                           const float* dscore, float* dsrc , float* dtgt , float* dw ,
                           float* dbias , const int32_t* mem_valid, float* part, const int32_t* t_off);
int fira_copy_score_bwd_blocks(int B, int S);
int fira_copy_part_stride(void);
int fira_head_loss_ex(void* stream, int BT, int T, int V, int S, const int32_t* compact_row, float* logits, int ldl,
                      float* score, const int32_t* mem_valid, float* gate_logits, const int32_t* tar_label,
                      float* loss_sum, int32_t* n_tok, int32_t* argmax_out, int want_grad, const int32_t* row_bt);

typedef struct fira_red_entry {
    float*       dst;
    const float* src;
    int32_t      width, n_part, stride;
} fira_red_entry;
int fira_deferred_reduce_max(void);
int fira_deferred_reduce(void* stream, int n, const fira_red_entry* entries );
int fira_rows_move(void* stream, int mode, int R, int W, float* out, int ld_out, const float* in, int ld_in,
                   const int32_t* src, const int32_t* dst);
int fira_rank2_rows(void* stream, int M, const float* g, const float* w, float* out);
int fira_colsum_weighted(void* stream, int M, int N, const float* X, int ldx, float* out, const float* row_weight);
int fira_embed_rows_fwd(void* stream, int R, int T, const int32_t* row_bt, const int32_t* idx, const float* table,
                        const float* pos, float* out);
int fira_embed_rows_bwd(void* stream, int R, const int32_t* row_bt, const int32_t* idx, float* dtable, const float* dout,
                        int padding_idx);
int fira_embed_grouped_bwd(void* stream, int n_items, const int32_t* item_tok, const int32_t* item_ptr, const int32_t* rows,
                           float* dtable, const float* dnode);
int fira_embed_list_bwd_small(void* stream, int n, const int32_t* rows, const int32_t* ids, float* dtable, const float* dnode,
                              int table_rows);
int fira_embed_gather_bwd_small(void* stream, int B, int L, const int32_t* idx, float* dtable, const float* dout,
                                int out_bstride, int out_off, int padding_idx, int table_rows);

int fira_adam_step(void* stream, int64_t n, float* p, const float* g, float* m, float* v,
                   float lr, float beta1, float beta2, float eps, int step, const float* inv_scale_ntok);
int fira_adam_step_mb(void* stream, int64_t n, float* p, const float* g0, const float* g1, float* m, float* v,
                      float lr, float beta1, float beta2, float eps, int step, const int32_t* n_tok0,
                      const int32_t* n_tok1);
int fira_adam_step_count(void* stream, int64_t n, float* p, const float* g, float* m, float* v,
                         float lr, float beta1, float beta2, float eps, int step, const float* count);
int fira_pack_stats(void* stream, const float* loss_sum, const int32_t* n_tok, float* out2);
int fira_inv_count(void* stream, const int32_t* n_tok, float* out);

int fira_debug_chain(void* stream, int n, int mode, float* scratch);


int fira_train_fwd_bwd(void* stream, const fira_dims* d, const fira_batch* batch, const float* params,
                       float* grads, void* workspace, size_t workspace_bytes, const fira_train_opts* opts,
                       float* loss_sum, int32_t* n_tok, void* mid_event);

int fira_gemm_wgrad_panel(void* stream, int dtype, int M, int N, int K, const float* A, int lda, const float* B, int ldb,
                          float* C, int ldc, float* colsum, float* scratch, size_t scratch_floats);

int fira_ffn_fwd(void* stream, int M, int F, const float* x, const float* w1, const float* b1, const float* w2, const float* b2,
                 const float* gamma, const float* beta, float* h, float* sum, float* y, float* stats, float dropout,
                 uint64_t seed, uint32_t site, int dtype);
int fira_ffn_bwd(void* stream, int M, int F, const float* dy, const float* x, const float* h, const float* sum,
                 const float* stats, const float* w1, const float* w2, const float* gamma, float* dx, float* dyf_ws,
                 float* dh_ws, float* dw1, float* db1, float* dw2, float* db2, float* dgamma, float* dbeta, float dropout,
                 uint64_t seed, uint32_t site, int dtype);
int fira_head_topk(void* stream, int R, int V, int k, const float* x, const float* wout, const float* bout, float* logits_ws,
                   int ldl, int32_t* ids, float* vals, int dtype);

size_t fira_head_logits_x3_scratch_bytes(int R);
int fira_head_logits_x3(void* stream, int R, int V, const float* x, int ldx, const float* W, const float* bias, float* logits,
                        int ldl, void* scratch);


typedef struct fira_lr_schedule {
    int32_t kind;
    float   base_lr;
    int32_t warmup_steps;
    int32_t decay_steps;
    float   min_lr;
} fira_lr_schedule;
float fira_lr_at(const fira_lr_schedule* s, int step);
int   fira_lr_schedule_check(const fira_lr_schedule* s);

typedef struct fira_adam_opts {
    float   lr, beta1, beta2, eps;
    int32_t step;
    float*  m;
    float*  v;
    const fira_lr_schedule* sched;
} fira_adam_opts;
int fira_train_step(void* stream, const fira_dims* d, const fira_batch* batch, float* params, float* grads,
                    void* workspace, size_t workspace_bytes, const fira_train_opts* opts, float* loss_sum,
                    int32_t* n_tok, const fira_adam_opts* adam);

int fira_train_step_begin(void* stream, const fira_dims* d, const fira_batch* batch, const float* params, float* grads,
                          void* workspace, size_t workspace_bytes, const fira_train_opts* opts, float* loss_sum,
                          int32_t* n_tok, void* mid_event );
int fira_train_step_end(void* stream, float* params, const fira_adam_opts* adam, void* early_event ,
                        const float* count);

int fira_train_step_rows(void* stream, const fira_dims* d, const fira_batch* batch, float* params, float* grads,
                         void* workspace, size_t workspace_bytes, const fira_train_opts* opts, float* loss_sum,
                         int32_t* n_tok, const fira_adam_opts* adam, int32_t* row_step);
int fira_adam_rows_sync(void* stream, const fira_dims* d, float* params, const fira_adam_opts* adam, int32_t* row_step);
int fira_adam_rows_catchup(void* stream, const fira_dims* d, float* params, const fira_adam_opts* adam, int32_t* row_step,
                           int table, const int32_t* ids, int n_ids);
int fira_adam_rows_step(void* stream, const fira_dims* d, float* params, const float* grads, const fira_adam_opts* adam,
                        int32_t* row_step, const int32_t* n_tok, const float* count , int tables );
int fira_train_step_begin_rows(void* stream, const fira_dims* d, const fira_batch* batch, const float* params, float* grads,
                               void* workspace, size_t workspace_bytes, const fira_train_opts* opts, float* loss_sum,
                               int32_t* n_tok, void* mid_event, const fira_adam_opts* adam, int32_t* row_step);
int fira_train_step_end_rows(void* stream, float* params, const fira_adam_opts* adam, void* early_event, const float* count,
                             int32_t* row_step);

int fira_ema_update(void* stream, int64_t n, float* ema, const float* p, float w);
int fira_ema_update_rows(void* stream, const fira_dims* d, float* ema, const float* params, const fira_adam_opts* adam,
                         const int32_t* row_step, float w);

typedef struct fira_clip_state {
    float   sq[4];
    float   norm;
    float   coef;
    int32_t zero_flag;
    int32_t n_clipped;
    int32_t n_nonfinite;
    int32_t reserved[7];
} fira_clip_state;
size_t fira_grad_sqsum_scratch_bytes(void);
int fira_grad_sqsum(void* stream, int64_t n, const float* g, fira_clip_state* state, int slot, void* scratch);
int fira_clip_finish(void* stream, fira_clip_state* state, int n_slots, const int32_t* n_tok, const float* count,
                     float max_norm);
int fira_adam_step_clip(void* stream, int64_t n, float* p, const float* g, float* m, float* v, float lr, float beta1,
                        float beta2, float eps, int step, const int32_t* n_tok, const float* count,
                        const fira_clip_state* state);
int fira_adam_rows_step_clip(void* stream, const fira_dims* d, float* params, const float* grads, const fira_adam_opts* adam,
                             int32_t* row_step, const int32_t* n_tok, const float* count, int tables,
                             const fira_clip_state* state);
int fira_train_step_clip(void* stream, const fira_dims* d, const fira_batch* batch, float* params, float* grads,
                         void* workspace, size_t workspace_bytes, const fira_train_opts* opts, float* loss_sum,
                         int32_t* n_tok, const fira_adam_opts* adam, int32_t* row_step , float max_norm,
                         fira_clip_state* state, void* scratch);

int fira_accum_stats(void* stream, const float* loss_sum, const int32_t* n_tok, float* stats ,
                     int32_t* n_tok_total, int first);
int fira_train_accum_micro(void* stream, const fira_dims* d, const fira_batch* batch, const float* params, float* grads,
                           void* workspace, size_t workspace_bytes, const fira_train_opts* opts, float* loss_sum,
                           int32_t* n_tok, const fira_adam_opts* adam , int32_t* row_step );
int fira_train_accum_last(void* stream, const fira_dims* d, const fira_batch* batch, float* params, float* grads,
                          void* workspace, size_t workspace_bytes, const fira_train_opts* opts, float* loss_sum,
                          int32_t* n_tok, const fira_adam_opts* adam, int32_t* row_step ,
                          float* stats , int32_t* n_tok_total, float max_norm ,
                          fira_clip_state* clip_state , void* clip_scratch);

int fira_f32_to_bf16(void* stream, int64_t n, const float* in, uint16_t* out);
int fira_bf16_to_f32(void* stream, int64_t n, const uint16_t* in, float* out);

int fira_forward_dev(void* stream, const fira_dims* d, const fira_batch* batch, const float* params,
                     void* workspace, size_t workspace_bytes, int32_t* ids_out, float* loss_sum, int32_t* n_tok,
                     int dtype );

int fira_dev_bleu_stats(void* stream, int B, int T, int V, int L, int S,
                        const int32_t* ids,
                        const int32_t* sou,    const int32_t* sub_token,
                        const int32_t* tar,
                        int32_t* hyp,
                        int32_t* stats);

int fira_mbr_bleu_stats(void* stream, int B, int n, int T,
                        const int32_t* tokens,   const int32_t* length,
                        int32_t* stats);

int fira_mbr_rouge_l_stats(void* stream, int B, int n, int T,
                           const int32_t* tokens,   const int32_t* length,
                           int32_t* stats);
int fira_dev_rouge_l_stats(void* stream, int B, int T, int V, int L, int S,
                           const int32_t* ids,
                           const int32_t* sou,    const int32_t* sub_token,
                           const int32_t* tar,
                           int32_t* stats);

int fira_dev_meteor_stats(void* stream, int B, int T, int V, int L, int S,
                          const int32_t* ids,
                          const int32_t* sou,    const int32_t* sub_token,
                          const int32_t* tar,
                          const int32_t* classes,
                          int32_t* stats);
int fira_mbr_meteor_stats(void* stream, int B, int n, int T,
                          const int32_t* tokens,   const int32_t* length,
                          int V, const int32_t* classes,
                          int32_t* stats);

int fira_decode_begin(void* stream, const fira_dims* d, const fira_batch* batch, const float* params,
                      void* workspace, size_t workspace_bytes, int n_beam);
int fira_decode_step(void* stream, const fira_dims* d, const float* params, void* workspace,
                     size_t workspace_bytes, int B, int n_beam, int step, const int32_t* tokens,
                     const int32_t* parent, float* dist, int32_t* best_id, float* best_p);
#define FIRA_DECODE_KV_BF16 1
int fira_decode_begin_ex(void* stream, const fira_dims* d, const fira_batch* batch, const float* params,
                         void* workspace, size_t workspace_bytes, int n_beam, int flags);
int fira_decode_step_ex(void* stream, const fira_dims* d, const float* params, void* workspace,
                        size_t workspace_bytes, int B, int n_beam, int step, const int32_t* tokens,
                        const int32_t* parent, float* dist, int32_t* best_id, float* best_p, int flags);

int fira_beam_prepare(void* stream, int B, int n_beam, int tar_len, int step, const int32_t* gen, const int32_t* length,
                      int32_t* tokens, int32_t* finished, int32_t* active, int32_t* done);
int fira_beam_select(void* stream, const fira_dims* d, int B, int n_beam, const float* dist, const int32_t* finished,
                     const int32_t* active, const int32_t* done, const int32_t* sou, const int32_t* sub_token,
                     const int32_t* gen_in, const int32_t* len_in, const float* prob_in, int32_t* gen_out,
                     int32_t* len_out, float* prob_out, int32_t* parent);

int fira_beam_select_scored(void* stream, const fira_dims* d, int B, int n_beam, const float* dist, const int32_t* finished,
                            const int32_t* active, const int32_t* done, const int32_t* sou, const int32_t* sub_token,
                            const int32_t* gen_in, const int32_t* len_in, const float* prob_in, int32_t* gen_out,
                            int32_t* len_out, float* prob_out, int32_t* parent,
                            const float* inv_lp , int n_groups, float diversity,
                            float* key_out );

int fira_beam_select_gumbel(void* stream, const fira_dims* d, int B, int n_beam, int step, float temperature,
                            const float* dist, const int32_t* finished, const int32_t* done, const int32_t* sou,
                            const int32_t* sub_token, const int32_t* key , const uint64_t* seed_dev,
                            const int32_t* gen_in, const int32_t* len_in, const float* phi_in, const float* G_in,
                            const float* logp_in, int32_t* gen_out, int32_t* len_out, float* phi_out, float* G_out,
                            float* logp_out, int32_t* parent);

int fira_beam_select_required(void* stream, const fira_dims* d, int B, int n_beam, const float* dist, const int32_t* finished,
                              const int32_t* active, const int32_t* done, const int32_t* sou, const int32_t* sub_token,
                              const int32_t* gen_in, const int32_t* len_in, const float* prob_in, int32_t* gen_out,
                              int32_t* len_out, float* prob_out, int32_t* parent,
                              const int32_t* required , const int32_t* n_required ,
                              int32_t* met_out );

int fira_beam_select_phrases(void* stream, const fira_dims* d, int B, int n_beam, const float* dist, const int32_t* finished,
                             const int32_t* active, const int32_t* done, const int32_t* sou, const int32_t* sub_token,
                             const int32_t* gen_in, const int32_t* len_in, const float* prob_in, int32_t* gen_out,
                             int32_t* len_out, float* prob_out, int32_t* parent,
                             const int32_t* words ,
                             const int32_t* item_len , const int32_t* n_items ,
                             int32_t* met_out );

int fira_contrastive_select(void* stream, const fira_dims* d, int B, int k, int step, float alpha, const float* dist,
                            const float* hidden , const int32_t* finished, const int32_t* sou,
                            const int32_t* sub_token, const int32_t* gen_in, const int32_t* len_in, const float* p_in ,
                            const float* prob_in , float* hist ,
                            int32_t* ended , int32_t* gen_out, int32_t* len_out, float* p_out, float* prob_out,
                            int32_t* parent, int32_t* pick_out , float* sim_out ,
                            float* score_out );

int fira_greedy_advance(void* stream, const fira_dims* d, int B, int step, const int32_t* best_id, const float* best_p,
                        const int32_t* sou, const int32_t* sub_token, int32_t* out, int32_t* length, float* prob,
                        int32_t* alive, int32_t* tokens, int32_t* n_alive);

int fira_constrain_dist(void* stream, const fira_dims* d, int R, int rows_per_commit, const int32_t* gen ,
                        const int32_t* length , const int32_t* sou ,
                        const int32_t* sub_token , int no_repeat_ngram, int min_length,
                        const int32_t* banned , int n_banned,
                        float* dist ,
                        int32_t* best_id, float* best_p );

int fira_merge_dist(void* stream, const fira_dims* d, int R, int rows_per_commit,
                    const int32_t* sou ,
                    const int32_t* sub_token ,
                    float* dist ,
                    int32_t* best_id, float* best_p );

int fira_force_dist(void* stream, const fira_dims* d, int R, int rows_per_commit, const int32_t* gen ,
                    const int32_t* length , const int32_t* sou ,
                    const int32_t* sub_token ,
                    const int32_t* prefix ,
                    const int32_t* prefix_len ,
                    float* dist ,
                    int32_t* best_id, float* best_p );

int fira_penalise_dist(void* stream, const fira_dims* d, int R, int rows_per_commit, const int32_t* gen ,
                       const int32_t* length , const int32_t* sou ,
                       const int32_t* sub_token ,
                       const float* count_factor ,
                       const int32_t* bias_id ,
                       const float* bias_factor ,
                       const int32_t* n_bias ,
                       float* dist ,
                       int32_t* best_id, float* best_p );

int fira_ban_phrases_dist(void* stream, const fira_dims* d, int R, int rows_per_commit, const int32_t* gen ,
                          const int32_t* length , const int32_t* sou ,
                          const int32_t* sub_token ,
                          const int32_t* phrase ,
                          const int32_t* phrase_len ,
                          const int32_t* n_phrases ,
                          float* dist ,
                          int32_t* best_id, float* best_p );

int fira_template_dist(void* stream, const fira_dims* d, int R, int rows_per_commit, const int32_t* gen ,
                       const int32_t* length , const int32_t* sou ,
                       const int32_t* sub_token ,
                       const uint8_t* word_class , const int8_t* next ,
                       const int32_t* need , const int32_t* start ,
                       float* dist ,
                       int32_t* best_id, float* best_p );

int fira_wordset_dist(void* stream, const fira_dims* d, int R, int rows_per_commit, const int32_t* gen ,
                      const int32_t* length , const int32_t* sou ,
                      const int32_t* sub_token ,
                      const uint32_t* allow, const uint32_t* deny, const uint32_t* boost,
                      const uint32_t* ground ,
                      const uint32_t* slot_valid ,
                      const float* boost_factor ,
                      float* dist ,
                      int32_t* best_id, float* best_p );

int fira_mix_dist(void* stream, int R, int W, int n_members,
                  const float* const* dists ,
                  const float* weights ,
                  float* out ,
                  int32_t* best_id, float* best_p );

int fira_pool_memory(void* stream, const fira_dims* d, int B, const float* mem, const int32_t* mem_valid,
                     float* out );
size_t fira_nn_search_scratch_bytes(int B, int N);
int fira_nn_search(void* stream, const float* Q , int B, const float* store , int N,
                   const int32_t* exclude , int32_t* best_idx , float* best_sim ,
                   void* scratch, size_t scratch_bytes);
int fira_mix_neighbour(void* stream, const fira_dims* d, int R, int rows_per_commit,
                       const float* coef ,
                       const float* q ,
                       float* dist ,
                       int32_t* best_id, float* best_p );

size_t fira_knn_search_scratch_bytes(int R, int N, int K);
int fira_knn_search(void* stream, const float* Q , int R, const float* keys ,
                    const float* key_sq , const int32_t* owner ,
                    const int32_t* exclude , int N, int K, int32_t* idx_out ,
                    float* d2_out , void* scratch, size_t scratch_bytes);
int fira_mix_knn(void* stream, const fira_dims* d, int R, const int32_t* idx , const float* d2 ,
                 const int32_t* values , int N, int K, const float* coef ,
                 float* dist , int32_t* best_id, float* best_p );

int fira_decode_step_sample(void* stream, const fira_dims* d, const float* params, void* workspace,
                            size_t workspace_bytes, int B, int n_sample, int step, const int32_t* tokens,
                            const int32_t* key, const uint64_t* seed_dev, float temperature, int top_k, float top_p,
                            float* dist, int32_t* best_id, float* best_p, int flags);
int fira_decode_step_sample_cut(void* stream, const fira_dims* d, const float* params, void* workspace,
                                size_t workspace_bytes, int B, int n_sample, int step, const int32_t* tokens,
                                const int32_t* key, const uint64_t* seed_dev, float temperature, int top_k, float top_p,
                                float min_p, float epsilon, float eta, float typical_p, float* dist, int32_t* best_id,
                                float* best_p, int flags);
int fira_sample_advance(void* stream, const fira_dims* d, int B, int n_sample, int step, const int32_t* best_id,
                        const float* best_p, const int32_t* sou, const int32_t* sub_token, int32_t* out, int32_t* length,
                        float* prob, float* logp, int32_t* alive, int32_t* tokens, int32_t* n_alive);

int fira_sample_dist(void* stream, const fira_dims* d, int R, int rows_per_commit, int step,
                     const float* dist ,
                     const int32_t* key , const uint64_t* seed_dev,
                     float temperature, int top_k, float top_p, float min_p, float epsilon, float eta, float typical_p,
                     int32_t* best_id , float* best_p );

int fira_decode_step_score(void* stream, const fira_dims* d, const float* params, void* workspace,
                           size_t workspace_bytes, int B, int n_cand, int step, const int32_t* tokens,
                           const int32_t* target, const int32_t* label, const int32_t* sou, const int32_t* sub_token,
                           float* dist, float* p_word, float* p_entry, int32_t* entry, float* copy_share, float* p_label,
                           int32_t* top_id, float* logp_word, float* logp_entry, float* logp_label, int flags);

int fira_decoder_forward(void* stream, const fira_dims* d, const float* params, void* workspace,
                         size_t workspace_bytes, int B, const int32_t* tar, const float* memory,
                         const int32_t* mem_valid, float* out);

const float*   fira_decode_memory(const fira_dims* d, void* workspace, int B, int n_beam);
const int32_t* fira_decode_mem_valid(const fira_dims* d, void* workspace, int B, int n_beam);

int fira_decode_hidden(void* stream, const fira_dims* d, void* workspace, size_t workspace_bytes, int B, int n_beam, int flags,
                       float* out );

int fira_host_node_lists(int B, int N, int L, int S, int skip_padding, const int64_t* sou, const int64_t* sub_token,
                         const int64_t* ast_change, const int64_t* mark, const int32_t* rowptr, const int32_t* col,
                         const float* val, int chunk, int32_t* node_rows, int32_t* rowptr_c, int32_t* col_c,
                         float* val_c, int32_t* code_rows, int32_t* code_mark, int32_t* mem_rows, int32_t* mem_dst,
                         int32_t* item_tok, int32_t* item_ptr, int32_t* emb_rows, int32_t* ast_rows, int32_t* ast_ids,
                         int32_t* counts);

int fira_host_collate_csr(int B, int N, const int64_t* idx, int64_t n_commits, const int32_t* store_rowptr,
                          const int64_t* store_offset, const int32_t* store_col, const float* store_val,
                          int32_t* rowptr, int32_t* col, float* val);

#ifdef __cplusplus
}
#endif
#endif
```

Before: 13840 commits/s.

## Process several column tiles per workgroup in LayerNorm-prologue tile32 GEMMs

```diff
diff --git a/fira_icse_amd/_lib.py b/fira_icse_amd/_lib.py
--- a/fira_icse_amd/_lib.py
+++ b/fira_icse_amd/_lib.py
@@ -97,6 +97,8 @@
     "fira_linear_presum_f32": (_I, [_P, _I, _I, _P, _I, _P, _P, _P, _P, _F, _U64, _U32]),
     "fira_ln_linear_f32": (_I, [_P, _I, _I, _P, _I, _P, _P, _P, _I, _I, _P, _P, _P, _P]),
     "fira_ln_bwd_linear_f32": (_I, [_P, _I, _I, _P, _P, _P, _P, _P, _P, _P, _P, _P, _P, _P, _P, _F, _U64, _U32]),
+    "fira_ln_linear_tn_f32": (_I, [_P, _I, _I, _P, _I, _P, _P, _P, _I, _I, _P, _P, _P, _P, _I]),
+    "fira_ln_bwd_linear_tn_f32": (_I, [_P, _I, _I, _P, _P, _P, _P, _P, _P, _P, _P, _P, _P, _P, _P, _F, _U64, _U32, _U32, _I]),
     "fira_linear_layernorm_bf16_fwd": (_I, [_P, _I, _P, _I, _P, _I, _P, _P, _P, _P, _P, _P, _P, _F, _U64, _U32]),
     "fira_add_layernorm_bwd": (_I, [_P, _I, _P, _P, _P, _P, _P, _P, _P, _P, _F, _U64, _U32]),
     "fira_dropout_mask": (_I, [_P, _U64, _U32, _L, _F, _P]),
diff --git a/fira_icse_amd/csrc/engine.h b/fira_icse_amd/csrc/engine.h
--- a/fira_icse_amd/csrc/engine.h
+++ b/fira_icse_amd/csrc/engine.h
@@ -119,12 +119,14 @@
                      float* C, int ldc, const float* bias, int flags, int* rc, const int32_t* c_rows,
                      const float* relu_mask, const int32_t* a_rows, const EpiRes* er);
 bool gemm_tile32_ln_try(hipStream_t s, int M, int N, const float* S, int lds, const float* W, const float* bias, float* Y,
-                        int ldy, int flags, const float* gamma, const float* beta, float* x_out, float* stats_out, int* rc);
+                        int ldy, int flags, const float* gamma, const float* beta, float* x_out, float* stats_out, int* rc,
+                        int tn = 0);
 int gemm_tile32_lnb_blocks(int M);
 bool gemm_tile32_lnb_try(hipStream_t s, int M, int N, const float* dy, const float* W, int ldw, float* dX, int lddx,
                          const float* relu_mask, const float* sum, const float* stats, const float* gamma, float* ds,
                          float* dx_drop, float* part, float dropout, uint64_t seed, uint32_t site, int* rc,
-                         uint32_t idx0 = 0);
+                         uint32_t idx0 = 0,
+                         int tn = 0);
 bool gemm_small_try(hipStream_t s, int tA, int tB, int M, int N, int K, const float* A, int lda, const float* B, int ldb,
                     float* C, int ldc, const float* bias, int flags, int* rc, const int32_t* c_rows = nullptr,
                     const float* relu_mask = nullptr);
diff --git a/fira_icse_amd/csrc/gemm_small.hip b/fira_icse_amd/csrc/gemm_small.hip
--- a/fira_icse_amd/csrc/gemm_small.hip
+++ b/fira_icse_amd/csrc/gemm_small.hip
@@ -163,7 +163,17 @@
     uint32_t idx0 = 0;
 };
 
-template <bool B_KCONTIG, int NCH, bool LN_A = false, bool LN_B = false, int NW = 4>
+template <bool B_KCONTIG>
+__device__ __forceinline__ void tile32_fetch_b(ChunkRegs& R, const float* pb0, const float* pb1, const float* pb2, const float* pb3,
+                                               int kc, int ldb) {
+    const size_t ob = B_KCONTIG ? (size_t)kc : (size_t)kc * ldb;
+    R.b0 = *reinterpret_cast<const f32x4*>(pb0 + ob);
+    R.b1 = *reinterpret_cast<const f32x4*>(pb1 + ob);
+    R.b2 = *reinterpret_cast<const f32x4*>(pb2 + ob);
+    R.b3 = *reinterpret_cast<const f32x4*>(pb3 + ob);
+}
+
+template <bool B_KCONTIG, int NCH, bool LN_A = false, bool LN_B = false, int NW = 4, int TN = 1>
 __global__ __launch_bounds__(NW * 64) void gemm_tile32_kernel(int M, int N, const float* __restrict__ A, int lda,
                                                           const float* __restrict__ B, int ldb, float* __restrict__ C,
                                                           int ldc, const float* __restrict__ bias, int flags,
@@ -172,6 +182,7 @@
                                                           const int32_t* __restrict__ a_rows, int tiles_n, const EpiRes er,
                                                           const LnA ln, const LnB lb) {
     static_assert(NW == 4 || (!LN_A && !LN_B), "the LayerNorm prologues are written for four waves");
+    static_assert(TN == 1 || ((LN_A || LN_B) && NCH == 2), "several column tiles per workgroup: the LayerNorm-prologue variants only");
     extern __shared__ __attribute__((aligned(16))) char tile32_dyn[];
     __shared__ __attribute__((aligned(16))) char smem4[NW == 4 ? 4 * 8192 : 16];
     char* const smem = NW == 4 ? smem4 : tile32_dyn;
@@ -183,7 +194,10 @@
         const int b = blockIdx.x, nwg = gridDim.x, q = nwg >> 3, r = nwg & 7, x = b & 7;
         t = (x < r ? x * (q + 1) : r * (q + 1) + (x - r) * q) + (b >> 3);
     }
-    const int m0 = (t / tiles_n) * 32, n0 = (t % tiles_n) * 32;
+    const int groups_n = tiles_n / TN;
+    const int m0 = (t / groups_n) * 32;
+    int n0 = (t % groups_n) * (32 * TN);
+    const bool col0 = n0 == 0;
     char* slot = smem + wave * 8192;
     const int lr = lane >> 3, ls = lane & 7;
     const int sw_even = lr >> 1, sw_odd = 4 + (lr >> 1);
@@ -194,17 +208,20 @@
     const float* pa2 = A + (size_t)ra2 * lda + ((ls ^ sw_even) << 2);
     const float* pa3 = A + (size_t)ra3 * lda + ((ls ^ sw_odd) << 2);
     const float *pb0, *pb1, *pb2, *pb3;
-    if (B_KCONTIG) {
-        pb0 = B + (size_t)min(n0 + lr, N - 1) * ldb + ((ls ^ sw_even) << 2);
-        pb1 = B + (size_t)min(n0 + 8 + lr, N - 1) * ldb + ((ls ^ sw_odd) << 2);
-        pb2 = B + (size_t)min(n0 + 16 + lr, N - 1) * ldb + ((ls ^ sw_even) << 2);
-        pb3 = B + (size_t)min(n0 + 24 + lr, N - 1) * ldb + ((ls ^ sw_odd) << 2);
-    } else {
-        pb0 = B + (size_t)lr * ldb + n0 + (ls << 2);
-        pb1 = pb0 + (size_t)8 * ldb;
-        pb2 = pb0 + (size_t)16 * ldb;
-        pb3 = pb0 + (size_t)24 * ldb;
-    }
+    auto point_b = [&](int nb) {
+        if (B_KCONTIG) {
+            pb0 = B + (size_t)min(nb + lr, N - 1) * ldb + ((ls ^ sw_even) << 2);
+            pb1 = B + (size_t)min(nb + 8 + lr, N - 1) * ldb + ((ls ^ sw_odd) << 2);
+            pb2 = B + (size_t)min(nb + 16 + lr, N - 1) * ldb + ((ls ^ sw_even) << 2);
+            pb3 = B + (size_t)min(nb + 24 + lr, N - 1) * ldb + ((ls ^ sw_odd) << 2);
+        } else {
+            pb0 = B + (size_t)lr * ldb + nb + (ls << 2);
+            pb1 = pb0 + (size_t)8 * ldb;
+            pb2 = pb0 + (size_t)16 * ldb;
+            pb3 = pb0 + (size_t)24 * ldb;
+        }
+    };
+    point_b(n0);
     const int i31 = lane & 31, kh = lane >> 5;
     const int wr_off = lr * 128 + ls * 16;
     const int sw_i = swz8(i31);
@@ -255,7 +272,7 @@
         R0.a1 = (R0.a1 - mean[1]) * rstd[1] * g0o + b0o; R1.a1 = (R1.a1 - mean[1]) * rstd[1] * g1o + b1o;
         R0.a2 = (R0.a2 - mean[2]) * rstd[2] * g0e + b0e; R1.a2 = (R1.a2 - mean[2]) * rstd[2] * g1e + b1e;
         R0.a3 = (R0.a3 - mean[3]) * rstd[3] * g0o + b0o; R1.a3 = (R1.a3 - mean[3]) * rstd[3] * g1o + b1o;
-        if (n0 == 0) {
+        if (col0) {
             const int r0 = m0 + lr, r1 = m0 + 8 + lr, r2 = m0 + 16 + lr, r3 = m0 + 24 + lr;
             float* xo = ln.x_out;
             if (r0 < M) { *reinterpret_cast<f32x4*>(xo + (size_t)r0 * FIRA_D + k0 + ce) = R0.a0; *reinterpret_cast<f32x4*>(xo + (size_t)r0 * FIRA_D + k1 + ce) = R1.a0; }
@@ -299,7 +316,7 @@
                 ln_red[1][wave][lr] = q0; ln_red[1][wave][8 + lr] = q1; ln_red[1][wave][16 + lr] = q2; ln_red[1][wave][24 + lr] = q3;
             }
         }
-        if (lb.part && n0 == 0) {
+        if (lb.part && col0) {
             const bool v0 = m0 + lr < M, v1 = m0 + 8 + lr < M, v2 = m0 + 16 + lr < M, v3 = m0 + 24 + lr < M;
             const f32x4 z = {0.f, 0.f, 0.f, 0.f};
             const f32x4 d00 = v0 ? R0.a0 : z, d10 = v0 ? R1.a0 : z, d01 = v1 ? R0.a1 : z, d11 = v1 ? R1.a1 : z;
@@ -350,7 +367,7 @@
         const int r0 = m0 + lr, r1 = m0 + 8 + lr, r2 = m0 + 16 + lr, r3 = m0 + 24 + lr;
         R0.a0 = drop(e00, r0, k0 + ce); R1.a0 = drop(e10, r0, k1 + ce); R0.a1 = drop(e01, r1, k0 + co); R1.a1 = drop(e11, r1, k1 + co);
         R0.a2 = drop(e02, r2, k0 + ce); R1.a2 = drop(e12, r2, k1 + ce); R0.a3 = drop(e03, r3, k0 + co); R1.a3 = drop(e13, r3, k1 + co);
-        if (n0 == 0) {
+        if (col0) {
             float* o1 = lb.ds;
             float* o2 = lb.dx;
             if (r0 < M) { *reinterpret_cast<f32x4*>(o1 + (size_t)r0 * FIRA_D + k0 + ce) = e00; *reinterpret_cast<f32x4*>(o1 + (size_t)r0 * FIRA_D + k1 + ce) = e10;
@@ -363,46 +380,63 @@
                           *reinterpret_cast<f32x4*>(o2 + (size_t)r3 * FIRA_D + k0 + co) = R0.a3; *reinterpret_cast<f32x4*>(o2 + (size_t)r3 * FIRA_D + k1 + co) = R1.a3; }
         }
     }
-#pragma unroll
-    for (int ci = 0; ci < NCH; ++ci) {
-        if ((ci & 1) == 0) {
-            tile32_stage(R0, slot, wr_off);
-            if (ci + 2 < NCH) tile32_fetch<B_KCONTIG>(R0, pa0, pa1, pa2, pa3, pb0, pb1, pb2, pb3, (wave + NW * (ci + 2)) << 5, ldb);
-        } else {
-            tile32_stage(R1, slot, wr_off);
-            if (ci + 2 < NCH) tile32_fetch<B_KCONTIG>(R1, pa0, pa1, pa2, pa3, pb0, pb1, pb2, pb3, (wave + NW * (ci + 2)) << 5, ldb);
-        }
-        acc = tile32_compute<B_KCONTIG>(slot, fa0, fa1, fa2, fa3, fb, acc);
-    }
-    __builtin_amdgcn_wave_barrier();
-    float* red = reinterpret_cast<float*>(slot);
-#pragma unroll
-    for (int r = 0; r < 16; ++r) red[r * 64 + lane] = acc[r];
-    __syncthreads();
-    {
-        constexpr int NV = (16 + NW - 1) / NW;
-        const int lnn = threadIdx.x & 63;
-        float vals[NV];
-        int rows[NV];
-        const float* p0 = reinterpret_cast<const float*>(smem);
-#pragma unroll
-        for (int i = 0; i < NV; ++i) {
-            const int idx = threadIdx.x + NW * 64 * i, r = idx >> 6;
-            const bool in = (16 % NW == 0) || idx < 1024;
-            const int ix = in ? idx : threadIdx.x;
-            if constexpr (NW == 4) {
-                vals[i] = (p0[ix] + p0[2048 + ix]) + (p0[4096 + ix] + p0[6144 + ix]);
+#pragma unroll 1
+    for (int jt = 0; jt < TN; ++jt) {
+        const int n_next = n0 + (jt + 1 < TN ? 32 : 0);
+        if constexpr (TN > 1) {
+            point_b(n_next);
+#pragma unroll
+            for (int r = 0; r < 16; ++r) acc[r] = 0.f;
+        }
+#pragma unroll
+        for (int ci = 0; ci < NCH; ++ci) {
+            if ((ci & 1) == 0) {
+                tile32_stage(R0, slot, wr_off);
+                if (ci + 2 < NCH) tile32_fetch<B_KCONTIG>(R0, pa0, pa1, pa2, pa3, pb0, pb1, pb2, pb3, (wave + NW * (ci + 2)) << 5, ldb);
+                else if constexpr (TN > 1) tile32_fetch_b<B_KCONTIG>(R0, pb0, pb1, pb2, pb3, wave << 5, ldb);
             } else {
-                float v = 0.f;
-#pragma unroll
-                for (int w = 0; w < NW; w += 4)
-                    v += (p0[w * 2048 + ix] + p0[(w + 1) * 2048 + ix]) + (p0[(w + 2) * 2048 + ix] + p0[(w + 3) * 2048 + ix]);
-                vals[i] = v;
-            }
-            rows[i] = in ? m0 + (r & 3) + 8 * (r >> 2) + 4 * (lnn >> 5) : M;
-        }
-        epilogue_col<NV>(vals, rows, n0 + (lnn & 31), M, N, C, ldc, bias, flags & FIRA_GEMM_RELU, flags & FIRA_GEMM_ACCUM, false,
-                         c_rows, relu_mask, er);
+                tile32_stage(R1, slot, wr_off);
+                if (ci + 2 < NCH) tile32_fetch<B_KCONTIG>(R1, pa0, pa1, pa2, pa3, pb0, pb1, pb2, pb3, (wave + NW * (ci + 2)) << 5, ldb);
+                else if constexpr (TN > 1) tile32_fetch_b<B_KCONTIG>(R1, pb0, pb1, pb2, pb3, (wave + NW) << 5, ldb);
+            }
+            acc = tile32_compute<B_KCONTIG>(slot, fa0, fa1, fa2, fa3, fb, acc);
+        }
+        __builtin_amdgcn_wave_barrier();
+        float* red = reinterpret_cast<float*>(slot);
+#pragma unroll
+        for (int r = 0; r < 16; ++r) red[r * 64 + lane] = acc[r];
+        if constexpr (TN > 1) lds_barrier();
+        else __syncthreads();
+        {
+            constexpr int NV = (16 + NW - 1) / NW;
+            const int lnn = threadIdx.x & 63;
+            float vals[NV];
+            int rows[NV];
+            const float* p0 = reinterpret_cast<const float*>(smem);
+#pragma unroll
+            for (int i = 0; i < NV; ++i) {
+                const int idx = threadIdx.x + NW * 64 * i, r = idx >> 6;
+                const bool in = (16 % NW == 0) || idx < 1024;
+                const int ix = in ? idx : threadIdx.x;
+                if constexpr (NW == 4) {
+                    vals[i] = (p0[ix] + p0[2048 + ix]) + (p0[4096 + ix] + p0[6144 + ix]);
+                } else {
+                    float v = 0.f;
+#pragma unroll
+                    for (int w = 0; w < NW; w += 4)
+                        v += (p0[w * 2048 + ix] + p0[(w + 1) * 2048 + ix]) + (p0[(w + 2) * 2048 + ix] + p0[(w + 3) * 2048 + ix]);
+                    vals[i] = v;
+                }
+                rows[i] = in ? m0 + (r & 3) + 8 * (r >> 2) + 4 * (lnn >> 5) : M;
+            }
+            epilogue_col<NV>(vals, rows, n0 + (lnn & 31), M, N, C, ldc, bias, flags & FIRA_GEMM_RELU, flags & FIRA_GEMM_ACCUM, false,
+                             c_rows, relu_mask, er);
+        }
+        if constexpr (TN > 1) {
+            if (jt + 1 == TN) break;
+            lds_barrier();
+            n0 = n_next;
+        }
     }
 }
 
@@ -483,17 +517,32 @@
     return true;
 }
 
+static int tile32_ln_tn(int tiles_n, int row_blocks, int want, int slots) {
+    if (want > 0) return tiles_n % want == 0 ? want : 1;
+    return tiles_n % 2 == 0 && (long)row_blocks * tiles_n * 4 >= (long)slots * 5 ? 2 : 1;
+}
+constexpr int tile32_lna_slots = 3 * 256, tile32_lnb_slots = 2 * 256;
+
 bool gemm_tile32_ln_try(hipStream_t s, int M, int N, const float* S, int lds, const float* W, const float* bias, float* Y,
-                        int ldy, int flags, const float* gamma, const float* beta, float* x_out, float* stats_out, int* rc) {
+                        int ldy, int flags, const float* gamma, const float* beta, float* x_out, float* stats_out, int* rc, int tn) {
     if (!gemm_tile32_takes(1, M, N, FIRA_D, S, lds, W, FIRA_D)) return false;
     if (((uintptr_t)gamma % 16) || ((uintptr_t)beta % 16) || ((uintptr_t)x_out % 16)) return false;
     ProfScope prof(s, PROF_GEMM, 2.0 * M * N * (double)FIRA_D, 4.0 * ((double)M * FIRA_D + (double)N * FIRA_D + (double)M * N));
     const int tiles_n = cdiv(N, 32);
+    tn = tile32_ln_tn(tiles_n, cdiv(M, 32), tn, tile32_lna_slots);
     LnA ln;
     ln.gamma = gamma; ln.beta = beta; ln.x_out = x_out; ln.stats_out = stats_out;
-    hipLaunchKernelGGL((gemm_tile32_kernel<true, 2, true, false>), dim3(cdiv(M, 32) * tiles_n), dim3(256), 0, s, M, N, S, lds, W, FIRA_D,
-                       Y, ldy, bias, flags & 3, (const int32_t*)nullptr, (const float*)nullptr, (const int32_t*)nullptr, tiles_n,
-                       EpiRes(), ln, LnB());
+    const dim3 grid(cdiv(M, 32) * (tiles_n / tn));
+#define FIRA_T32LN(TN)                                                                                                 \
+    hipLaunchKernelGGL((gemm_tile32_kernel<true, 2, true, false, 4, TN>), grid, dim3(256), 0, s, M, N, S, lds, W, FIRA_D, Y, ldy, bias, \
+                       flags & 3, (const int32_t*)nullptr, (const float*)nullptr, (const int32_t*)nullptr, tiles_n, EpiRes(), ln, LnB())
+    switch (tn) {
+        case 8: FIRA_T32LN(8); break;
+        case 4: FIRA_T32LN(4); break;
+        case 2: FIRA_T32LN(2); break;
+        default: FIRA_T32LN(1); break;
+    }
+#undef FIRA_T32LN
     hipError_t e = hipGetLastError();
     *rc = e != hipSuccess ? set_err("gemm_tile32_ln: %s", hipGetErrorString(e)) : 0;
     return true;
@@ -502,17 +551,26 @@
 int gemm_tile32_lnb_blocks(int M) { return cdiv(M, 32); }
 bool gemm_tile32_lnb_try(hipStream_t s, int M, int N, const float* dy, const float* W, int ldw, float* dX, int lddx,
                          const float* relu_mask, const float* sum, const float* stats, const float* gamma, float* ds,
-                         float* dx_drop, float* part, float dropout, uint64_t seed, uint32_t site, int* rc, uint32_t idx0) {
+                         float* dx_drop, float* part, float dropout, uint64_t seed, uint32_t site, int* rc, uint32_t idx0, int tn) {
     if (!gemm_tile32_takes(0, M, N, FIRA_D, dy, FIRA_D, W, ldw)) return false;
     if (((uintptr_t)sum % 16) || ((uintptr_t)gamma % 16) || ((uintptr_t)ds % 16) || ((uintptr_t)dx_drop % 16) || ds == dy) return false;
     ProfScope prof(s, PROF_GEMM, 2.0 * M * N * (double)FIRA_D, 4.0 * ((double)M * FIRA_D + (double)N * FIRA_D + (double)M * N));
     const int tiles_n = cdiv(N, 32);
+    tn = tile32_ln_tn(tiles_n, cdiv(M, 32), tn, tile32_lnb_slots);
     LnB lb;
     lb.sum = sum; lb.stats = stats; lb.gamma = gamma; lb.ds = ds; lb.dx = dx_drop; lb.part = part;
     lb.p = dropout; lb.inv_keep = dropout > 0.f ? 1.0f / (1.0f - dropout) : 1.0f; lb.seed = seed; lb.site = site; lb.idx0 = idx0;
-    hipLaunchKernelGGL((gemm_tile32_kernel<false, 2, false, true>), dim3(cdiv(M, 32) * tiles_n), dim3(256), 0, s, M, N, dy, FIRA_D, W, ldw,
-                       dX, lddx, (const float*)nullptr, 0, (const int32_t*)nullptr, relu_mask, (const int32_t*)nullptr, tiles_n,
-                       EpiRes(), LnA(), lb);
+    const dim3 grid(cdiv(M, 32) * (tiles_n / tn));
+#define FIRA_T32LNB(TN)                                                                                                \
+    hipLaunchKernelGGL((gemm_tile32_kernel<false, 2, false, true, 4, TN>), grid, dim3(256), 0, s, M, N, dy, FIRA_D, W, ldw, dX, lddx,   \
+                       (const float*)nullptr, 0, (const int32_t*)nullptr, relu_mask, (const int32_t*)nullptr, tiles_n, EpiRes(), LnA(), lb)
+    switch (tn) {
+        case 8: FIRA_T32LNB(8); break;
+        case 4: FIRA_T32LNB(4); break;
+        case 2: FIRA_T32LNB(2); break;
+        default: FIRA_T32LNB(1); break;
+    }
+#undef FIRA_T32LNB
     hipError_t e = hipGetLastError();
     *rc = e != hipSuccess ? set_err("gemm_tile32_lnb: %s", hipGetErrorString(e)) : 0;
     return true;
@@ -655,16 +713,24 @@
         return fira::set_err("fira_linear_presum_f32: shape %d x 256 x %d / alignment not taken by the tile kernel", M, K);
     return rc;
 }
+static bool tile32_tn_arg(int tn) { return tn == 0 || tn == 1 || tn == 2 || tn == 4 || tn == 8; }
 int fira_ln_bwd_linear_f32(void* stream, int M, int N, const float* dy, const float* Wt, float* dX, const float* relu_mask,
                            const float* sum, const float* stats, const float* gamma, float* ds, float* dx_drop, float* dgamma,
                            float* dbeta, float* part, float dropout, uint64_t seed, uint32_t site) {
+    return fira_ln_bwd_linear_tn_f32(stream, M, N, dy, Wt, dX, relu_mask, sum, stats, gamma, ds, dx_drop, dgamma, dbeta, part, dropout,
+                                     seed, site, 0, 0);
+}
+int fira_ln_bwd_linear_tn_f32(void* stream, int M, int N, const float* dy, const float* Wt, float* dX, const float* relu_mask,
+                              const float* sum, const float* stats, const float* gamma, float* ds, float* dx_drop, float* dgamma,
+                              float* dbeta, float* part, float dropout, uint64_t seed, uint32_t site, uint32_t idx0, int tn) {
     FIRA_REQUIRE(dy && Wt && dX && sum && stats && gamma && ds && dx_drop && dgamma && dbeta && part && M > 0 && N > 0,
                  "fira_ln_bwd_linear_f32: bad argument");
     FIRA_REQUIRE(ds != dy, "fira_ln_bwd_linear_f32: ds must not alias dy");
     FIRA_REQUIRE(dropout >= 0.f && dropout < 1.f, "fira_ln_bwd_linear_f32: dropout must be in [0,1)");
+    FIRA_REQUIRE(tile32_tn_arg(tn), "fira_ln_bwd_linear_tn_f32: tn must be 0 (the engine's choice), 1, 2, 4 or 8");
     int rc = 0;
     if (!fira::gemm_tile32_lnb_try((hipStream_t)stream, M, N, dy, Wt, N, dX, N, relu_mask, sum, stats, gamma, ds, dx_drop, part,
-                                   dropout, seed, site, &rc))
+                                   dropout, seed, site, &rc, idx0, tn))
         return fira::set_err("fira_ln_bwd_linear_f32: shape %d x %d / alignment not taken by the tile kernel", M, N);
     if (rc) return rc;
     fira::RedTable tab;
@@ -676,10 +742,15 @@
 }
 int fira_ln_linear_f32(void* stream, int M, int N, const float* S, int lds, const float* W, const float* bias, float* Y,
                        int ldy, int relu, const float* gamma, const float* beta, float* x_out, float* stats_out) {
+    return fira_ln_linear_tn_f32(stream, M, N, S, lds, W, bias, Y, ldy, relu, gamma, beta, x_out, stats_out, 0);
+}
+int fira_ln_linear_tn_f32(void* stream, int M, int N, const float* S, int lds, const float* W, const float* bias, float* Y,
+                          int ldy, int relu, const float* gamma, const float* beta, float* x_out, float* stats_out, int tn) {
     FIRA_REQUIRE(S && W && Y && gamma && beta && x_out && M > 0 && N > 0, "fira_ln_linear_f32: bad argument");
+    FIRA_REQUIRE(tile32_tn_arg(tn), "fira_ln_linear_tn_f32: tn must be 0 (the engine's choice), 1, 2, 4 or 8");
     int rc = 0;
     if (!fira::gemm_tile32_ln_try((hipStream_t)stream, M, N, S, lds, W, bias, Y, ldy, relu ? FIRA_GEMM_RELU : 0, gamma, beta, x_out,
-                                  stats_out, &rc))
+                                  stats_out, &rc, tn))
         return fira::set_err("fira_ln_linear_f32: shape %d x %d / alignment not taken by the tile kernel", M, N);
     return rc;
 }
diff --git a/fira_icse_amd/ops.py b/fira_icse_amd/ops.py
--- a/fira_icse_amd/ops.py
+++ b/fira_icse_amd/ops.py
@@ -124,15 +124,19 @@
     return s
 
 
-def ln_linear(s, w, bias, gamma, beta, relu=False):
+def ln_linear(s, w, bias, gamma, beta, relu=False, tn=None):
     M = s.shape[0]
     N = w.shape[0]
     assert w.shape[1] == 256 and s.shape[1] == 256 and s.stride(1) == 1
     y = torch.empty((M, N), dtype=torch.float32, device=s.device)
     x = torch.empty((M, 256), dtype=torch.float32, device=s.device)
     stats = torch.empty((M, 2), dtype=torch.float32, device=s.device)
-    check(_lib.lib().fira_ln_linear_f32(cur_stream(), M, N, ptr(s), s.stride(0), ptr(_f32(w)), ptr(bias), ptr(y), N, int(relu),
-                                        ptr(_f32(gamma)), ptr(_f32(beta)), ptr(x), ptr(stats)), "fira_ln_linear_f32")
+    args = (cur_stream(), M, N, ptr(s), s.stride(0), ptr(_f32(w)), ptr(bias), ptr(y), N, int(relu), ptr(_f32(gamma)),
+            ptr(_f32(beta)), ptr(x), ptr(stats))
+    if tn is None:
+        check(_lib.lib().fira_ln_linear_f32(*args), "fira_ln_linear_f32")
+    else:
+        check(_lib.lib().fira_ln_linear_tn_f32(*args, tn), "fira_ln_linear_tn_f32")
     return y, x, stats
 
 
@@ -160,17 +164,19 @@
     return ds, dxd, dg, db
 
 
-def ln_bwd_linear(dy, Wt, summ, stats, gamma, relu_mask=None, dropout=0.0, seed=0, site=0):
+def ln_bwd_linear(dy, Wt, summ, stats, gamma, relu_mask=None, dropout=0.0, seed=0, site=0, idx0=0, tn=None):
     M, N = dy.shape[0], Wt.shape[1]
     dX = torch.empty((M, N), dtype=torch.float32, device=dy.device)
     ds, dxd = torch.empty_like(dy), torch.empty_like(dy)
     dg = torch.zeros(256, dtype=torch.float32, device=dy.device)
     db = torch.zeros(256, dtype=torch.float32, device=dy.device)
     part = torch.empty(((M + 31) // 32) * 512, dtype=torch.float32, device=dy.device)
-    check(_lib.lib().fira_ln_bwd_linear_f32(cur_stream(), M, N, ptr(_f32(dy)), ptr(_f32(Wt)), ptr(dX),
-                                            ptr(None if relu_mask is None else _f32(relu_mask)), ptr(_f32(summ)),
-                                            ptr(_f32(stats)), ptr(_f32(gamma)), ptr(ds), ptr(dxd), ptr(dg), ptr(db), ptr(part),
-                                            dropout, seed, site), "fira_ln_bwd_linear_f32")
+    args = (cur_stream(), M, N, ptr(_f32(dy)), ptr(_f32(Wt)), ptr(dX), ptr(None if relu_mask is None else _f32(relu_mask)),
+            ptr(_f32(summ)), ptr(_f32(stats)), ptr(_f32(gamma)), ptr(ds), ptr(dxd), ptr(dg), ptr(db), ptr(part), dropout, seed, site)
+    if tn is None and idx0 == 0:
+        check(_lib.lib().fira_ln_bwd_linear_f32(*args), "fira_ln_bwd_linear_f32")
+    else:
+        check(_lib.lib().fira_ln_bwd_linear_tn_f32(*args, idx0, tn or 0), "fira_ln_bwd_linear_tn_f32")
     return dX, ds, dxd, dg, db
 
 
diff --git a/include/fira_hip.h b/include/fira_hip.h
--- a/include/fira_hip.h
+++ b/include/fira_hip.h
@@ -157,6 +157,12 @@
 int fira_ln_bwd_linear_f32(void* stream, int M, int N, const float* dy, const float* Wt, float* dX, const float* relu_mask,
                            const float* sum, const float* stats, const float* gamma, float* ds, float* dx_drop,
                            float* dgamma, float* dbeta, float* part, float dropout, uint64_t seed, uint32_t site);
+int fira_ln_linear_tn_f32(void* stream, int M, int N, const float* S, int lds, const float* W, const float* bias, float* Y,
+                          int ldy, int relu, const float* gamma, const float* beta, float* x_out, float* stats_out, int tn);
+int fira_ln_bwd_linear_tn_f32(void* stream, int M, int N, const float* dy, const float* Wt, float* dX,
+                              const float* relu_mask, const float* sum, const float* stats, const float* gamma, float* ds,
+                              float* dx_drop, float* dgamma, float* dbeta, float* part, float dropout, uint64_t seed,
+                              uint32_t site, uint32_t idx0, int tn);
 int fira_linear_layernorm_bf16_fwd(void* stream, int M, const float* X, int ldx, const uint16_t* Wb, int ldb,
                                    const float* bias, const float* res, const float* gamma, const float* beta,
                                    float* sum, float* y, float* stats, float dropout, uint64_t seed,
```

New measurement: 13780 commits/s, median of 2. Within noise of the previous version (-0.5%).
